# arogozhnikov/demuxalot

Hardware: AMD Instinct MI355X
Metric: EM iterations/sec + barcodes demuxed/sec, 200k bc x 100k SNP x 64 gt (higher is better)
Workload: dtype f32 terms, f64 sums (guarded mode: coarse pass reads the table as f16 and sums in f32; exact redo where the contract is not proven)

## Files before the change

### demuxalot_amd/_lib.py

```python
import ctypes
import os
from ctypes import POINTER, c_char_p, c_double, c_float, c_int, c_int32, c_int64, c_void_p

import numpy as np

_HERE = os.path.dirname(os.path.abspath(__file__))
LIB_PATH = os.environ.get('DEMUXALOT_AMD_LIB') or os.path.join(_HERE, 'libdemux_hip.so')

DMX_F32, DMX_F64 = 0, 1
T_PSTEP, T_ESTEP, T_MSTEP, T_MCOMBINE, T_ALLREDUCE, T_COUNT = 0, 1, 2, 3, 4, 5
TIMER_NAMES = ('pstep', 'estep', 'mstep', 'mcombine', 'allreduce')
HOST_COLLECTIVE = ctypes.CFUNCTYPE(ctypes.c_int, ctypes.c_void_p, ctypes.c_int, ctypes.c_void_p, ctypes.c_int64, ctypes.c_int)
COLL_ALL_REDUCE, COLL_REDUCE_SCATTER, COLL_ALL_GATHER = 0, 1, 2
UNIQUE_ID_BYTES = 128

_P = c_void_p
SIGNATURES = {
    'dmx_last_error': (c_char_p, []),
    'dmx_version': (c_char_p, []),
    'dmx_device_count': (c_int, [POINTER(c_int)]),
    'dmx_create': (c_int, [c_int, POINTER(_P)]),
    'dmx_destroy': (c_int, [_P]),
    'dmx_synchronize': (c_int, [_P]),
    'dmx_pack_calls_host': (c_int, [c_int64, _P, _P, _P, c_int64, _P, _P, _P, _P, _P, _P,
                                    POINTER(c_int64), POINTER(c_int64), _P, _P, _P, _P, _P]),
    'dmx_hash_host': (c_int, [_P, c_int64, c_int32, POINTER(ctypes.c_uint64)]),
    'dmx_set_problem': (c_int, [_P, c_int64, c_int64, c_int32, c_int64, _P, _P, _P, _P]),
    'dmx_pack_and_set_problem': (c_int, [_P, c_int64, c_int64, c_int32, _P, _P, _P, _P, c_int64, _P, _P, _P, _P, _P,
                                         POINTER(c_int64), POINTER(c_int64), _P]),
    'dmx_pack_containers_and_set_problem': (c_int, [_P, c_int64, c_int64, c_int32, _P, _P, _P, _P, _P, c_int32,
                                                    POINTER(c_int64), POINTER(c_int64), _P]),
    'dmx_stage_containers': (c_int, [_P, _P, c_int32]),
    'dmx_pack_staged_and_set_problem': (c_int, [_P, c_int64, c_int64, c_int32, _P, _P, _P, _P, _P, c_int32,
                                                POINTER(c_int64), POINTER(c_int64), _P]),
    'dmx_get_packed_calls': (c_int, [_P, _P, _P, _P, _P]),
    'dmx_set_betas': (c_int, [_P, _P]),
    'dmx_set_prior_betas': (c_int, [_P, _P, c_double, c_int, _P, _P]),
    'dmx_set_addition': (c_int, [_P, _P]),
    'dmx_probs_from_betas': (c_int, [_P, c_float, c_float, _P]),
    'dmx_probs_from_betas_f64': (c_int, [_P, _P, c_float, c_float, _P]),
    'dmx_set_probs': (c_int, [_P, _P]),
    'dmx_estep': (c_int, [_P, c_int, _P, _P, c_int, _P, _P]),
    'dmx_mstep': (c_int, [_P, c_float, _P]),
    'dmx_em': (c_int, [_P, c_int, c_float, c_float, c_int, _P, _P, c_int, c_float, _P, _P, _P]),
    'dmx_run_iterations': (c_int, [_P, c_int, c_float, c_float, c_float]),
    'dmx_get_logits': (c_int, [_P, _P]),
    'dmx_get_probs': (c_int, [_P, _P]),
    'dmx_get_addition': (c_int, [_P, _P]),
    'dmx_get_block': (c_int, [_P, c_int, c_int64, c_int64, c_int64, c_int64, _P]),
    'dmx_get_assignments': (c_int, [_P, _P, _P]),
    'dmx_get_assignments_above': (c_int, [_P, c_float, _P, _P, POINTER(c_int64)]),
    'dmx_get_top_options': (c_int, [_P, c_int32, _P, _P]),
    'dmx_get_option_sums': (c_int, [_P, _P]),
    'dmx_set_keep_molecule_calls': (c_int, [_P, c_int]),
    'dmx_set_molecule_calls': (c_int, [_P, c_int64, _P, _P, _P]),
    'dmx_get_max_pair_count': (c_int, [_P, POINTER(c_int64)]),
    'dmx_estep_snp': (c_int, [_P, c_int, _P, c_int64, _P, c_int, _P, _P]),
    'dmx_mstep_f64': (c_int, [_P, c_double, _P]),
    'dmx_mstep_f64_sums': (c_int, [_P, c_double, _P]),
    'dmx_get_prior_betas': (c_int, [_P, _P]),
    'dmx_get_learnt_betas': (c_int, [_P, _P]),
    'dmx_exchange_slices': (c_int, [c_int64, _P, c_int32, _P, POINTER(c_int64), POINTER(c_int32)]),
    'dmx_comm_unique_id': (c_int, [_P]),
    'dmx_comm_init': (c_int, [_P, c_int, c_int, _P, c_int]),
    'dmx_comm_init_host': (c_int, [_P, c_int, c_int, _P, _P, c_int]),
    'dmx_get_timings': (c_int, [_P, POINTER(c_double), POINTER(c_int64)]),
    'dmx_reset_timings': (c_int, [_P]),
    'dmx_set_phase_timers': (c_int, [_P, c_int]),
    'dmx_set_logits_needed': (c_int, [_P, c_int]),
    'dmx_set_lean_memory': (c_int, [_P, c_int]),
    'dmx_device_bytes': (c_int, [_P, POINTER(c_int64)]),
    'dmx_trim_cache': (c_int, [_P, POINTER(c_int64)]),
    'dmx_release_problem': (c_int, [_P]),
    'dmx_trim_device_caches': (c_int, [c_int, POINTER(c_int64)]),
    'dmx_set_exact_additions': (c_int, [_P, c_int]),
    'dmx_set_estep_mode': (c_int, [_P, c_int]),
    'dmx_set_msteps_expected': (c_int, [_P, c_int64]),
    'dmx_snp_count': (c_int, [_P, _P, c_int32, _P, c_int64, c_int32, c_float, c_int32, POINTER(c_int64)]),
    'dmx_snp_score': (c_int, [_P, c_double, _P, _P, _P, _P, _P, _P]),
    'dmx_snp_select': (c_int, [_P, c_int64, c_int64, _P, POINTER(c_int64)]),
    'dmx_count_reads': (c_int, [_P, _P, _P, c_int64, _P, POINTER(c_int64), POINTER(c_int64)]),
    'dmx_count_reads_fetch': (c_int, [_P, _P, _P]),
    'dmx_coverage_count': (c_int, [_P, _P, c_int32, c_int32, c_int32, _P]),
    'dmx_coverage_candidates': (c_int, [_P, c_double, c_double, c_double, c_double, c_int64, POINTER(c_int64)]),
    'dmx_coverage_fetch_candidates': (c_int, [_P, _P, _P]),
}
DEBUG_SIGNATURES = {
    'dmx_comm_init_emulated': (c_int, [_P, c_int, c_int, c_double, c_double, c_int]),
    'dmx_get_exchange_compact': (c_int, [_P, POINTER(c_int64), POINTER(c_int64), POINTER(c_int64)]),
    'dmx_get_exchange_compact_table': (c_int, [_P, POINTER(c_int64), POINTER(c_int64), POINTER(c_int64)]),
    'dmx_get_guard_probes': (c_int, [_P, POINTER(c_int64), POINTER(c_int64)]),
    'dmx_debug_set_pass_ms': (c_int, [_P, c_double, c_double, c_double]),
    'dmx_get_redo_count': (c_int, [_P, POINTER(c_int64)]),
    'dmx_set_guard_adaptive': (c_int, [_P, c_int]),
    'dmx_set_coarse_pass': (c_int, [_P, c_int]),
    'dmx_set_mstep_incremental': (c_int, [_P, c_int]),
    'dmx_get_mstep_incremental': (c_int, [_P, POINTER(c_int64), POINTER(c_int64), POINTER(c_int64)]),
    'dmx_get_guard_levels': (c_int, [_P, POINTER(c_int32), POINTER(c_int64), POINTER(c_int64), POINTER(c_int64), POINTER(c_double), POINTER(c_double), POINTER(c_double)]),
    'dmx_get_guard_direct': (c_int, [_P, POINTER(c_int32), POINTER(c_int64), POINTER(c_int64), POINTER(c_double), POINTER(c_double)]),
    'dmx_set_estep_schedule': (c_int, [_P, c_int]),
    'dmx_set_estep_dictionary': (c_int, [_P, c_int]),
    'dmx_get_estep_form': (c_int, [_P, POINTER(c_int32), POINTER(c_int32)]),
    'dmx_set_estep_packing': (c_int, [_P, c_int]),
    'dmx_set_mstep_wide_addresses': (c_int, [_P, c_int]),
    'dmx_set_mstep_tiles': (c_int, [_P, c_int]),
    'dmx_get_mstep_form': (c_int, [_P, POINTER(c_int32)]),
    'dmx_get_mstep_tiles_info': (c_int, [_P, POINTER(c_int32), POINTER(c_double)]),
    'dmx_test_logf': (c_int, [_P, _P, _P, c_int64]),
    'dmx_test_logf_hot': (c_int, [_P, _P, _P, c_int64]),
    'dmx_test_expf': (c_int, [_P, _P, _P, c_int64]),
    'dmx_test_log2_hw': (c_int, [_P, _P, _P, c_int64]),
    'dmx_test_softmax': (c_int, [_P, _P, _P, c_int64, c_int64]),
    'dmx_runtime_info': (c_int, [c_char_p, c_int64]),
    'dmx_get_exchange_mode': (c_int, [_P, POINTER(c_int32)]),
    'dmx_get_guard_stats': (c_int, [_P, POINTER(c_int64), POINTER(c_int64), POINTER(c_int64)]),
    'dmx_get_count_reads_timings': (c_int, [_P, POINTER(c_double)]),
    'dmx_count_reads_begin': (c_int, [_P, _P, c_int64, _P]),
    'dmx_count_reads_push': (c_int, [_P, _P, c_int, POINTER(c_int64), POINTER(c_int64)]),
    'dmx_count_reads_end': (c_int, [_P]),
    'dmx_get_count_reads_carry': (c_int, [_P, POINTER(c_int64)]),
    'dmx_get_count_reads_peak_bytes': (c_int, [_P, POINTER(c_int64)]),
    'dmx_set_coverage_form': (c_int, [_P, c_int]),
    'dmx_get_coverage_timings': (c_int, [_P, POINTER(c_double)]),
    'dmx_reads_upload': (c_int, [_P, _P, POINTER(c_int64)]),
    'dmx_reads_release': (c_int, [_P, c_int64]),
    'dmx_reads_info': (c_int, [_P, c_int64, POINTER(c_int64)]),
    'dmx_count_reads_resident': (c_int, [_P, c_int64, _P, c_int64, _P, POINTER(c_int64), POINTER(c_int64)]),
    'dmx_coverage_count_resident': (c_int, [_P, c_int64, c_int32, c_int32, c_int32, _P]),
    'dmx_count_reads_push_resident': (c_int, [_P, c_int64, c_int64, c_int64, c_int, POINTER(c_int64), POINTER(c_int64)]),
    'dmx_get_reads_upload_bytes': (c_int, [_P, POINTER(c_int64)]),
}

COVERAGE_STAGES = ('upload', 'walk', 'window', 'accumulate', 'filter', 'top_n')
COVERAGE_ATOMIC, COVERAGE_TILED = 0, 1
READS_INFO = ('n_reads', 'n_cigar_ops', 'n_bases', 'nbytes', 'reference_length')
COUNT_READS_STAGES = ('upload', 'walk', 'molecules', 'duplicates', 'observations', 'fold', 'order')


class DecodedReadsStruct(ctypes.Structure):
    _fields_ = [('n_reads', c_int64), ('reference_start', _P), ('compressed_cb', _P), ('compressed_ub', _P), ('p_misaligned', _P),
                ('alignment_score', _P), ('cigar_begin', _P), ('n_cigar', _P), ('seq_begin', _P), ('l_seq', _P),
                ('n_cigar_ops', c_int64), ('cigar', _P), ('n_bases', c_int64), ('seq', _P), ('qual', _P)]


_lib = None


class DemuxHipError(RuntimeError):
    pass


def load():
    global _lib
    if _lib is None:
        if not os.path.exists(LIB_PATH):
            raise DemuxHipError(
                f'{LIB_PATH} is missing: build it with `python -c "import __graft_entry__ as g; g.build()"` '
                f'or `make -C demuxalot_amd/csrc`. demuxalot_amd has no CPU fallback.')
        os.environ.setdefault('HSA_ENABLE_IPC_MODE_LEGACY', '0')
        lib = ctypes.CDLL(LIB_PATH)
        for name, (res, args) in {**SIGNATURES, **DEBUG_SIGNATURES}.items():
            fn = getattr(lib, name)
            fn.restype = res
            fn.argtypes = args
        _lib = lib
    return _lib


def check(status):
    if status != 0:
# ... 32 lines not shown
```

### demuxalot_amd/csrc/dmx_api.cpp

```cpp
#include <dlfcn.h>
#include <hip/hip_runtime.h>
#include <rccl/rccl.h>

#include <array>
#include <chrono>
#include <functional>

#include <algorithm>
#include <mutex>
#include <cmath>
#include <cstdio>
#include <cstdlib>
#include <cstring>
#include <string>
#include <vector>

#include "dmx_ctx.h"
#include "dmx_host.h"

using namespace dmx::host;

extern "C" {

static int begin_problem(dmx_ctx *c, int64_t B, int64_t V, int32_t G, const int32_t *v2snp, std::vector<int> &snp_ptr,
// ... 175 lines not shown
    HIP_TRY(hipStreamSynchronize(c->stream));
    return 0;
}

int dmx_set_exact_additions(dmx_ctx *c, int exact)
{
    if (!c) return fail(DMX_ERR_INVALID, "null context");
    c->exact_additions = exact != 0;
    return 0;
}

int dmx_set_estep_mode(dmx_ctx *c, int mode)
{
    if (!c) return fail(DMX_ERR_INVALID, "null context");
    if (mode != DMX_ESTEP_EXACT && mode != DMX_ESTEP_FAST && mode != DMX_ESTEP_GUARDED) return fail(DMX_ERR_INVALID, "unknown E-step mode %d", mode);
    c->estep_mode = mode;
    return 0;
}

static int read_guard_state(dmx_ctx *c, unsigned (&st)[dmx::GS_WORDS], long long *count, long long *count_fine = nullptr, long long *count_coarse = nullptr)
{
    std::vector<unsigned> all((size_t)dmx::GUARD_STATE_WORDS, 0u);
    if (c->d_guard_count.p) {
        HIP_TRY(hipMemcpyAsync(all.data(), c->d_guard_count.p, all.size() * sizeof(unsigned), hipMemcpyDeviceToHost, c->stream));
        HIP_TRY(hipStreamSynchronize(c->stream));
    }
    for (int i = 0; i < dmx::GS_WORDS; i++) st[i] = all[(size_t)i];
    long long hashed_fine = 0, hashed_coarse = 0;
    for (int i = 0; i < dmx::GUARD_SLOTS; i++) {
        hashed_fine += all[(size_t)dmx::GS_SLOTS_FINE + i];
        hashed_coarse += all[(size_t)dmx::GS_SLOTS_COARSE + i];
    }
    const unsigned level = st[dmx::GS_LEVEL];
    const long long fine = level == 1u ? (long long)st[dmx::GS_COUNT] : hashed_fine;
    const long long coarse = level == 0u ? (long long)st[dmx::GS_COUNT] : (st[dmx::GS_CAPABLE] ? hashed_coarse : -1);
    *count = level == 0u ? coarse : fine;
    if (count_fine) *count_fine = fine;
    if (count_coarse) *count_coarse = coarse;
    return 0;
}

int dmx_get_guard_stats(dmx_ctx *c, int64_t *redone_last, int64_t *redone_total, int64_t *rows_total)
{
    DMX_TRY(bind(c));
    unsigned st[dmx::GS_WORDS];
    long long count = 0;
    DMX_TRY(read_guard_state(c, st, &count));
    const long long last = st[dmx::GS_DIRECT] ? (long long)st[dmx::GS_ROWS] : count;
    const long long total = (long long)(((unsigned long long)st[dmx::GS_TOTAL + 1] << 32) | st[dmx::GS_TOTAL]) + (st[dmx::GS_PENDING] ? last : 0);
    if (redone_last) *redone_last = c->guard_ran ? (int64_t)last : 0;
    if (redone_total) *redone_total = (int64_t)total;
    if (rows_total) *rows_total = (int64_t)c->guard_rows_total;
    return 0;
}

int dmx_set_mstep_incremental(dmx_ctx *c, int incremental)
{
    if (!c) return fail(DMX_ERR_INVALID, "null context");
    if (incremental < 0 || incremental > 2) return fail(DMX_ERR_INVALID, "incremental M-step: 0 off, 1 on, 2 on with the first sums built by the delta pass");
    if (incremental != c->mstep_incremental) c->incr_valid = false;
    c->mstep_incremental = incremental;
    return 0;
}

int dmx_get_mstep_incremental(dmx_ctx *c, int64_t *full_passes, int64_t *delta_passes, int64_t *barcodes_last_delta)
{
    DMX_TRY(bind(c));
    unsigned st[3 * dmx::IS_WORDS] = {};
    if (c->d_incr_state.p) {
        HIP_TRY(hipMemcpyAsync(st, c->d_incr_state.p, sizeof(st), hipMemcpyDeviceToHost, c->stream));
        HIP_TRY(hipStreamSynchronize(c->stream));
    }
    if (full_passes) *full_passes = (int64_t)st[2 * dmx::IS_WORDS];
    if (delta_passes) *delta_passes = (int64_t)st[2 * dmx::IS_WORDS + 1];
    if (barcodes_last_delta) *barcodes_last_delta = st[2 * dmx::IS_WORDS + 2] == 0xFFFFFFFFu ? -1 : (int64_t)st[2 * dmx::IS_WORDS + 2];
    return 0;
}

int dmx_set_coarse_pass(dmx_ctx *c, int coarse)
{
    if (!c) return fail(DMX_ERR_INVALID, "null context");
    if (coarse < 0 || coarse > 2) return fail(DMX_ERR_INVALID, "coarse pass: 0 never, 1 where the logits are not read, 2 wherever the shape allows");
    c->coarse_pass = coarse;
    return 0;
}

int dmx_set_lean_memory(dmx_ctx *c, int lean)
{
    DMX_TRY(bind(c));
    c->lean_memory = lean != 0;
    if (c->lean_memory && c->coarse_ready) {
        dev_free(c, c->d_tile_stream);
        dev_free(c, c->d_call_rows);
    }
    return 0;
}

int dmx_set_guard_adaptive(dmx_ctx *c, int adaptive)
{
    if (!c) return fail(DMX_ERR_INVALID, "null context");
    c->guard_adaptive = adaptive != 0;
    return 0;
}

int dmx_get_guard_direct(dmx_ctx *c, int32_t *last_ran_direct, int64_t *direct_steps, int64_t *would_queue_last, double *fast_pass_ms,
                         double *exact_pass_ms)
{
    DMX_TRY(bind(c));
    unsigned st[dmx::GS_WORDS];
    long long count = 0;
    DMX_TRY(read_guard_state(c, st, &count));
    if (last_ran_direct) *last_ran_direct = c->guard_ran && st[dmx::GS_DIRECT] ? 1 : 0;
    if (direct_steps) *direct_steps = (int64_t)st[dmx::GS_DIRECT_STEPS];
    if (would_queue_last) *would_queue_last = c->guard_ran ? (int64_t)count : 0;
    int khz = 0;
    HIP_TRY(hipDeviceGetAttribute(&khz, hipDeviceAttributeWallClockRate, c->device));
    const double ms_per_tick = khz > 0 ? 1.0 / (double)khz : 0.0;
    if (fast_pass_ms) *fast_pass_ms = st[dmx::GS_F_TICKS] * ms_per_tick;
    if (exact_pass_ms) *exact_pass_ms = (st[dmx::GS_E_MEASURED] ? 1.0 : -1.0) * st[dmx::GS_E_TICKS] * ms_per_tick;
    return 0;
}

int dmx_get_guard_levels(dmx_ctx *c, int32_t *level_last, int64_t *coarse_steps, int64_t *flagged_fine_last, int64_t *flagged_coarse_last,
                         double *coarse_pass_ms, double *fine_pass_ms, double *exact_pass_ms)
{
    DMX_TRY(bind(c));
    unsigned st[dmx::GS_WORDS];
    long long count = 0, fine = 0, coarse = 0;
    DMX_TRY(read_guard_state(c, st, &count, &fine, &coarse));
    if (level_last) *level_last = c->guard_ran ? (int32_t)st[dmx::GS_LEVEL] : -1;
    if (coarse_steps) *coarse_steps = (int64_t)st[dmx::GS_COARSE_STEPS];
    if (flagged_fine_last) *flagged_fine_last = c->guard_ran ? (int64_t)fine : 0;
    if (flagged_coarse_last) *flagged_coarse_last = c->guard_ran ? (int64_t)coarse : -1;
    int khz = 0;
    HIP_TRY(hipDeviceGetAttribute(&khz, hipDeviceAttributeWallClockRate, c->device));
    const double ms_per_tick = khz > 0 ? 1.0 / (double)khz : 0.0;
    if (coarse_pass_ms) *coarse_pass_ms = st[dmx::GS_C_TICKS] * ms_per_tick;
    if (fine_pass_ms) *fine_pass_ms = st[dmx::GS_F_TICKS] * ms_per_tick;
    if (exact_pass_ms) *exact_pass_ms = (st[dmx::GS_E_MEASURED] ? 1.0 : -1.0) * st[dmx::GS_E_TICKS] * ms_per_tick;
    return 0;
}

int dmx_set_logits_needed(dmx_ctx *c, int needed)
{
    if (!c) return fail(DMX_ERR_INVALID, "null context");
    c->logits_needed = needed != 0;
    return 0;
}

int dmx_get_guard_probes(dmx_ctx *c, int64_t *probes, int64_t *streak)
{
    DMX_TRY(bind(c));
    unsigned st[dmx::GS_WORDS];
    long long count = 0, fine = 0, coarse = 0;
    DMX_TRY(read_guard_state(c, st, &count, &fine, &coarse));
    if (probes) *probes = (int64_t)st[dmx::GS_PROBES];
    if (streak) *streak = (int64_t)st[dmx::GS_STREAK];
    return 0;
}

int dmx_debug_set_pass_ms(dmx_ctx *c, double coarse_pass_ms, double fine_pass_ms, double exact_pass_ms)
{
    DMX_TRY(bind(c));
    if (!c->d_guard_count.p) return fail(DMX_ERR_INVALID, "call order: a guarded E-step before dmx_debug_set_pass_ms");
    int khz = 0;
    HIP_TRY(hipDeviceGetAttribute(&khz, hipDeviceAttributeWallClockRate, c->device));
// ... 293 lines not shown
```

### demuxalot_amd/csrc/dmx_ctx.h

```cpp
#pragma once
#include <hip/hip_runtime.h>
#include <rccl/rccl.h>

#include <map>
#include <mutex>
#include <string>
#include <unordered_map>
#include <utility>
#include <vector>

#include "dmx_internal.h"
#include "kernels.h"

using dmx::fail;

#define HIP_TRY(expr)                                                                                   \
    do {                                                                                                \
        hipError_t _e = (expr);                                                                         \
        if (_e != hipSuccess) return fail(DMX_ERR_HIP, "%s failed: %s", #expr, hipGetErrorString(_e)); \
    } while (0)

#define DMX_TRY(expr)         \
    do {                      \
        int _s = (expr);      \
// ... 19 lines not shown
    size_t n = 0;
};

struct ResidentReads {
    long long n = 0, n_ops = 0, n_bases = 0;
    long long reference_length = 0;
    bool countable = false;
    int64_t bytes = 0;
    DevBuf<int> start, cb, ub, score, n_cigar, l_seq;
    DevBuf<double> p;
    DevBuf<long long> cigar_begin, seq_begin;
    DevBuf<unsigned> cigar;
    DevBuf<unsigned char> seq, qual;
};

struct dmx_ctx {
    int device = 0;
    hipStream_t stream = nullptr;
    long long B = 0, V = 0, N = 0, S = 0;
    int G = 0, K = 0;
    bool have_problem = false, have_betas = false, have_probs = false, have_post = false;

    DevBuf<long long> d_pair_ptr;
    DevBuf<dmx::CallPair> d_call_pairs;
    DevBuf<unsigned> d_call_rows;
    long long n_pairs = 0;
    DevBuf<uint2> d_csc;
    long long n_csc = 0;
    DevBuf<long long> d_item_start;
    DevBuf<int> d_item_len;
    DevBuf<long long> d_item_ptr;
    DevBuf<int> d_item_variant;
    DevBuf<int> d_bc_order, d_item_order;
    long long n_items = 0;
    long long n_bins = 0;
    int n_tiles = 0, bin_rows_cap = 0;
    DevBuf<int> d_bin_rows, d_bin_order;
    DevBuf<long long> d_bin_ptr;
    DevBuf<dmx::CallPair> d_tile_stream;
    DevBuf<int> d_v2snp, d_snp_ptr, d_snp_vars;
    DevBuf<float> d_prior, d_add, d_prob;
    DevBuf<float> d_raw;
    bool have_raw = false;
    DevBuf<unsigned short> d_prob16;
    DevBuf<unsigned> d_coarse_stream;
    DevBuf<long long> d_coarse_bin_ptr;
    DevBuf<double> d_log2_keep;
    bool coarse_ready = false;
    bool prob16_valid = false;
    int coarse_pass = 1;
    int lean_memory = 0;
    bool logits_needed = true;
    bool logits_readable = true;
    float p_clip_lo = 0.0f;
    DevBuf<double> d_add64, d_partial;
    DevBuf<float> d_logits, d_post;
    DevBuf<unsigned long long> d_nz;
    DevBuf<unsigned long long> d_redo;
    DevBuf<unsigned> d_n_redo;
    bool mstep_wide = false;
    DevBuf<uint2> d_mt_stream;
    DevBuf<long long> d_mt_ptr;
    DevBuf<int> d_mt_first;
    DevBuf<int> d_mt_order;
    DevBuf<int> d_mt_shift;
    DevBuf<unsigned char> d_mt_shift_v;
    DevBuf<unsigned long long> d_acc64;
    DevBuf<float> d_prev_post;
    DevBuf<uint2> d_prev_first;
    DevBuf<int> d_incr_list;
    DevBuf<unsigned char> d_incr_touched;
    DevBuf<unsigned> d_incr_state;
    int incr_parity = 0;
    bool incr_valid = false;
    float incr_power = 0.0f;
    int mstep_incremental = 1;
    long long mstep_incr_launches = 0;
    long long n_mt = 0;
    std::vector<long long> h_col_ptr;
    int mt_tv = 0;
    bool mt_tried = false;
    bool mt_shift_tried = false;
    int mstep_tiles = 1;
    long long msteps_done = 0;
    long long incr_rows = 0;
    DevBuf<unsigned char> d_incr_map;
    DevBuf<uint2> d_slice_rec;
    DevBuf<long long> d_slice_ptr;
    bool slice_index_tried = false;
    bool incr_heavy = false;
    int msteps_ahead = 0;
    long long msteps_expected = 0;
    double mt_build_ms = 0.0;
    int mstep_form = 0;
    DevBuf<int> d_sum_plan;
    long long sum_plan_k = -1;
    int sum_plan_values = 0;
    int item_calls = 1024;
    bool exact_additions = true;
    int estep_mode = DMX_ESTEP_EXACT;
    DevBuf<unsigned> d_guard_count;
    int guard_adaptive = 1;
    DevBuf<int> d_guard_list;
    DevBuf<int> d_guard_sub;
    unsigned guard_sub_cap = 0;
    long long guard_rows_total = 0;
    bool guard_ran = false;
    int tiled_estep = 1;
    int dict_mode = 1;
    bool add_is_zero = true;
    bool dict_candidate = false;
    int estep_form = 0;
    int estep_packing = 1;
    long long max_row_calls = 0;
    int n_simd = 0;
    long long long_row_calls[3] = {0, 0, 0};
    long long n_long_rows[3] = {0, 0, 0};
    int dict_distinct = 0;
    DevBuf<float> d_dict;
    DevBuf<unsigned char> d_codes;
    DevBuf<unsigned char> d_dtab;
    DevBuf<unsigned> d_dict_stat;
    DevBuf<dmx::EstepSegment> d_segs;
    DevBuf<int> d_split_first;
    DevBuf<double> d_seg_sums;
    long long n_segs = 0, n_split = 0;
    float nz_floor = 0.0f;
    DevBuf<uint2> d_first;
    DevBuf<unsigned long long> d_dense_calls;
    bool dense_stat_valid = false;
    DevBuf<float> d_pen;
    DevBuf<unsigned> d_pairs;
    DevBuf<unsigned> d_pair_blocks;
    int n_pair_blocks = 0;
    DevBuf<unsigned char> d_prior_logits;
    DevBuf<int> d_best;
    DevBuf<float> d_bestp;
    DevBuf<int> d_u_variant, d_u_cb;
    DevBuf<float> d_u_p;
    DevBuf<long long> d_u_count;
    long long n_u = 0;
    DevBuf<unsigned long long> d_mol;
    bool keep_molecule_calls = false;
    DevBuf<int> d_mc_variant;
    DevBuf<float> d_mc_e;
    DevBuf<long long> d_mc_start;
    unsigned mc_max_count = 0;
    DevBuf<double> d_logits64, d_post64;
    bool have_post64 = false;
    DevBuf<unsigned char> d_scratch;
    DevBuf<unsigned long long> d_sd_pos;
    DevBuf<int> d_sd_counts;
    DevBuf<double> d_sd_imp;
    long long sd_P = -1;
    int sd_D = 0;
    bool sd_scored = false;
    DevBuf<unsigned char> d_cr_molecules;
    DevBuf<unsigned char> d_cr_calls;
    long long cr_molecules = -1, cr_calls = 0;
    double cr_stage_ms[dmx::COUNT_READS_STAGES] = {};
    int64_t cr_peak_bytes = 0;
    long long cr_carried = 0;
    DevBuf<int> d_crs_positions;
    DevBuf<double> d_crs_table;
    DevBuf<int> d_crs_start, d_crs_cb, d_crs_ub, d_crs_score, d_crs_n_cigar, d_crs_l_seq;
    DevBuf<double> d_crs_p;
// ... 155 lines not shown
```

### demuxalot_amd/csrc/dmx_steps.cpp

```cpp
#include <dlfcn.h>
#include <hip/hip_runtime.h>
#include <rccl/rccl.h>

#include <array>
#include <chrono>
#include <functional>

#include <algorithm>
#include <mutex>
#include <cmath>
#include <cstdio>
#include <cstdlib>
#include <cstring>
#include <string>
#include <vector>

#include "dmx_ctx.h"
#include "dmx_host.h"

using namespace dmx::host;

namespace dmx {
namespace host {

// ... 72 lines not shown
    DMX_TRY(dev_grow(c, c->d_seg_sums, (size_t)c->n_segs * (size_t)K));
    HIP_TRY(hipStreamSynchronize(c->stream));
    if ((int)K != c->K) c->have_post64 = false;
    c->K = (int)K;
    return 0;
}

int upload_prior_logits(dmx_ctx *c, const void *prior, int dtype)
{
    if (!prior) return 0;
    if (dtype != DMX_F32 && dtype != DMX_F64) return fail(DMX_ERR_INVALID, "prior_dtype must be DMX_F32 or DMX_F64");
    const size_t bytes = (size_t)c->B * c->K * (dtype == DMX_F64 ? 8 : 4);
    if (bytes > c->d_prior_logits.n) {
        raw_free(c, c->d_prior_logits);
        DMX_TRY(raw_alloc(c, c->d_prior_logits, bytes));
    }
    HIP_TRY(hipMemcpyAsync(c->d_prior_logits.p, prior, bytes, hipMemcpyHostToDevice, c->stream));
    return 0;
}

int copy_prob_out(dmx_ctx *c, float *dst)
{
    if (!dst) return 0;
    const int G = c->G;
    if (!c->sliced) return copy_out(c, dst, c->d_prob.p, (size_t)c->V * G);
    for (int r = 0; r < c->nranks; r++) {
        const long long rows = c->cut[r + 1] - c->cut[r];
        if (rows) HIP_TRY(hipMemcpyAsync(dst + c->cut[r] * G, c->d_prob.p + (size_t)r * c->slice_rows * G, sizeof(float) * rows * G, hipMemcpyDeviceToHost, c->stream));
    }
    return 0;
}

int copy_prob_in(dmx_ctx *c, const float *src)
{
    const int G = c->G;
    c->prob_prev_valid = false;
    if (!c->sliced) {
        HIP_TRY(hipMemcpyAsync(c->d_prob.p, src, sizeof(float) * c->V * G, hipMemcpyHostToDevice, c->stream));
        return 0;
    }
    for (int r = 0; r < c->nranks; r++) {
        const long long rows = c->cut[r + 1] - c->cut[r];
        if (rows) HIP_TRY(hipMemcpyAsync(c->d_prob.p + (size_t)r * c->slice_rows * G, src + c->cut[r] * G, sizeof(float) * rows * G, hipMemcpyHostToDevice, c->stream));
    }
    return 0;
}

int ensure_full_addition(dmx_ctx *c)
{
    if (!c->add_partial) return 0;
    const int G = c->G, n = c->nranks;
    float *stage = (float *)c->d_add_stage.p;
    const size_t block = (size_t)c->slice_rows * G;
    const long long mine = c->cut[c->rank + 1] - c->cut[c->rank];
    if (mine) HIP_TRY(hipMemcpyAsync(stage + c->rank * block, c->d_add.p + c->cut[c->rank] * G, sizeof(float) * mine * G, hipMemcpyDeviceToDevice, c->stream));
    DMX_TRY(coll_all_gather(c, stage, block, "addition"));
    for (int k = 0; k < n; k++) {
        const long long rows = c->cut[k + 1] - c->cut[k];
        if (rows && k != c->rank) HIP_TRY(hipMemcpyAsync(c->d_add.p + c->cut[k] * G, stage + k * block, sizeof(float) * rows * G, hipMemcpyDeviceToDevice, c->stream));
    }
    c->add_partial = false;
    return 0;
}

bool coarse_capable(const dmx_ctx *c, int with_doublets, float lo)
{
    return c->coarse_pass && c->estep_mode == DMX_ESTEP_GUARDED && !with_doublets && c->K > 16 && c->K <= 128 && c->tiled_estep && c->n_bins > 0 &&
           (c->coarse_ready || c->d_tile_stream.p != nullptr) && lo >= 6.2e-5f && ((unsigned long long)c->prob_rows + 1ull) * (unsigned long long)c->G * 4ull < (1ull << 32);
}

int ensure_prob16(dmx_ctx *c)
{
    const size_t need16 = ((size_t)c->prob_rows + 1) * c->G * 2;
    if (need16 > c->d_prob16.n) {
        DMX_TRY(dev_grow(c, c->d_prob16, need16));
        c->prob16_valid = false;
        HIP_TRY(hipMemsetAsync(c->d_prob16.p, 0, need16 * sizeof(unsigned short), c->stream));
    }
    return 0;
}

int run_pstep(dmx_ctx *c, float lo, float hi, bool with_addition, bool with_half)
{
    const bool half_rows = with_half && c->sliced && c->prob_list_words != 0 && c->prob_prev_valid && c->prob16_valid && c->d_prob16.p != nullptr;
    with_half = with_half && !c->sliced;
    if (with_half) DMX_TRY(ensure_prob16(c));
    c->prob16_valid = false;
    TimerSpan ev{nullptr, nullptr};
    SpanGuard ev_guard{c, &ev};
    timer_begin(c, DMX_T_PSTEP, &ev);
    const long long v0 = c->sliced ? c->cut[c->rank] : 0, v1 = c->sliced ? c->cut[c->rank + 1] : c->V;
    if (c->emulated && c->sliced && !c->emu_table_filled) {
        for (int r = 0; r < c->nranks; r++)
            if (r != c->rank)
                HIP_TRY(dmx::launch_probs_from_betas(c->stream, c->d_prior.p, nullptr, c->d_v2snp.p, c->d_snp_ptr.p, c->d_snp_vars.p, c->cut[r],
                                                     c->cut[r + 1] - c->cut[r], -1LL, c->G, c->d_prow.p, lo, hi, c->d_prob.p));
        c->emu_table_filled = true;
    }
    HIP_TRY(dmx::launch_probs_from_betas(c->stream, c->d_prior.p, with_addition ? c->d_add.p : nullptr, c->d_v2snp.p,
                                         c->d_snp_ptr.p, c->d_snp_vars.p, v0, v1 - v0, c->sliced ? -1LL : (long long)c->S, c->G, c->d_prow.p, lo, hi,
                                         c->d_prob.p, (with_half || half_rows) ? c->d_prob16.p : nullptr));
    c->prob16_valid = with_half;
    timer_end(c, DMX_T_PSTEP, ev);
    if (c->sliced) {
        timer_begin(c, DMX_T_ALLREDUCE, &ev);
        const size_t block = (size_t)c->slice_rows * c->G;
        float *mine = c->d_prob.p + (size_t)c->rank * block;
        int rc = 0;
        bool whole = true;
        if (c->prob_list_words != 0 && c->prob_prev_valid) {
            const unsigned cap_now = std::max(1u, std::min(c->prob_cap_now, c->prob_list_cap));
            const size_t words_now = 4 + (size_t)cap_now * (size_t)(1 + c->G);
            HIP_TRY(dmx::launch_prob_changes_build(c->stream, mine, c->d_prob_prev.p, c->slice_rows, c->G, cap_now,
                                                   c->d_prob_list.p + (size_t)c->rank * words_now,
                                                   c->emulated ? c->d_prob_list.p : nullptr, (unsigned long long)words_now, c->nranks, c->rank));
            rc = coll_all_gather(c, (float *)c->d_prob_list.p, words_now, "changed rows of genotype_prob");
            if (rc == 0) {
                const unsigned seq = ++c->list_seq;
                HIP_TRY(dmx::launch_post_counts(c->stream, c->d_prob_list.p, (unsigned long long)words_now, c->nranks, c->h_prob_counts, seq));
                HIP_TRY(dmx::launch_prob_changes_apply(c->stream, c->d_prob.p, c->d_prob_list.p, (unsigned long long)words_now, c->slice_rows, c->G,
                                                       c->nranks, c->rank, cap_now, half_rows ? (unsigned short *)c->d_prob16.p : nullptr));
                DMX_TRY(wait_counts(c, c->h_prob_counts, c->nranks, seq));
                unsigned longest = 0;
                for (int r = 0; r < c->nranks; r++) longest = std::max(longest, c->h_prob_counts[r]);
                whole = longest > cap_now;
                if (std::getenv("DEMUXALOT_AMD_EXCHANGE_TRACE")) std::fprintf(stderr, "[table lists] longest %u capacity %u of %u\n", longest, cap_now, c->prob_list_cap);
                c->prob_cap_now = whole ? c->prob_list_cap : (unsigned)std::min<unsigned long long>(c->prob_list_cap, 4ull * longest + 512ull);
                if (!whole) {
                    c->prob_compact_taken++;
                    c->prob16_valid = half_rows;
                } else {
                    c->prob_compact_overflows++;
                }
            }
        } else if (c->prob_list_words != 0) {
            HIP_TRY(hipMemcpyAsync(c->d_prob_prev.p, mine, sizeof(float) * block, hipMemcpyDeviceToDevice, c->stream));
            c->prob_prev_valid = true;
        }
        if (rc == 0 && whole) rc = coll_all_gather(c, c->d_prob.p, block, "genotype_prob");
        timer_end(c, DMX_T_ALLREDUCE, ev);
        if (rc) return rc;
    }
    c->have_probs = true;
    c->p_clip_lo = lo;
    c->dict_candidate = !with_addition || c->add_is_zero;
    return 0;
}

int prepare_dictionary(dmx_ctx *c, bool pairs, dmx::EstepArgs &a, int *form)
{
    *form = DMX_FORM_DIRECT;
    a.dict_n = 0;
    c->dict_distinct = 0;
    const bool wanted = c->dict_mode == 2 || (c->dict_mode == 1 && c->dict_candidate);
    if (!wanted || c->estep_mode == DMX_ESTEP_FAST || c->B == 0 || c->prob_rows == 0) return 0;
    const int G = c->G;
    const long long K = c->K, rows = c->prob_rows;
    const bool block_form = pairs && K > dmx::DICT_LANE_K;
    if (a.call_rows == nullptr) return 0;
    if (!block_form && (K > dmx::DICT_LANE_K || rows >= (1 << 24) || a.pairs_bytes == 0)) return 0;
    if (block_form && (size_t)G * 72 + 9 * 1024 > 160 * 1024) return 0;
    if (G > 1024) return 0;
    if (c->dict_mode == 1 && !block_form) {
        const long long lanes = K <= 16 ? 4 : K <= 32 ? 8 : K <= 64 ? 16 : K <= 128 ? 32 : 64;
        if (pairs || c->B * lanes / 64 < 8192) return 0;
    }
    const size_t code_pitch = (size_t)dmx::dict_code_pitch(G);
    DMX_TRY(dev_grow(c, c->d_dict, (size_t)rows * dmx::DICT_CAP));
    DMX_TRY(dev_grow(c, c->d_codes, (size_t)rows * code_pitch));
    if (!c->d_dict_stat.p) DMX_TRY(dev_alloc(c, c->d_dict_stat, (size_t)1));
    HIP_TRY(dmx::launch_build_dict(c->stream, c->d_prob.p, rows, G, c->d_dict.p, c->d_codes.p, c->d_dict_stat.p));
    unsigned distinct = 0;
    HIP_TRY(hipMemcpyAsync(&distinct, c->d_dict_stat.p, sizeof(unsigned), hipMemcpyDeviceToHost, c->stream));
    HIP_TRY(hipStreamSynchronize(c->stream));
// ... 138 lines not shown
                if (c->lean_memory) {
                    dev_free(c, c->d_tile_stream);
                    dev_free(c, c->d_call_rows);
                    a.call_rows = nullptr;
                }
            }
            if (allow_coarse) DMX_TRY(ensure_prob16(c));
            HIP_TRY(dmx::launch_guard_begin(c->stream, c->d_guard_count.p, c->B, c->K, c->guard_adaptive, capable, allow_coarse));
            a.guard = 1;
            if (fine8) a.guard_per_call = dmx::guard_per_call_fine8(dmx::coarse_calls_per_gather((int)c->K));
            a.order_direct = c->d_bc_order.p;
            a.guard_main_coarse = 0;
            a.guard_alt_per_call = capable ? dmx::GUARD_PER_CALL_COARSE : 0.0f;
            a.guard_alt_accum = capable ? dmx::GUARD_ACCUM_F32 : 0.0f;
            if (allow_coarse) {
                if (!c->prob16_valid) {
                    const bool kept = c->sliced && c->prob_list_words != 0;
                    HIP_TRY(dmx::launch_prob_to_half(c->stream, c->d_prob.p, c->prob_rows, c->G, c->d_prob16.p, kept ? nullptr : c->d_guard_count.p + dmx::GS_SKIP_COARSE));
                    c->prob16_valid = kept;
                }
                dmx::EstepArgs coarse = a;
                coarse.prob16 = c->d_prob16.p;
                coarse.coarse_stream = c->d_coarse_stream.p;
                coarse.coarse_bin_ptr = c->d_coarse_bin_ptr.p;
                coarse.log2_keep = c->d_log2_keep.p;
                coarse.guard_per_call = dmx::GUARD_PER_CALL_COARSE;
                coarse.guard_accum = dmx::GUARD_ACCUM_F32;
                coarse.guard_main_coarse = 1;
                coarse.guard_alt_per_call = a.guard_per_call;
                coarse.guard_alt_accum = 0.0f;
                coarse.direct = c->d_guard_count.p + dmx::GS_SKIP_COARSE;
                HIP_TRY(dmx::launch_estep(c->stream, coarse, false));
            }
            a.direct = c->d_guard_count.p + dmx::GS_SKIP_FINE;
            a.tile_stream = c->d_tile_stream.p;
            if (c->d_tile_stream.p == nullptr) {
                if (c->coarse_ready && !with_doublets && a.n_bins > 0 && c->K > 16 && c->K <= 128) {
                    a.coarse_stream = c->d_coarse_stream.p;
                    a.coarse_bin_ptr = c->d_coarse_bin_ptr.p;
                    a.log2_keep = c->d_log2_keep.p;
                    a.prob16 = nullptr;
                    a.guard_per_call = dmx::guard_per_call_fine8(dmx::coarse_calls_per_gather((int)c->K));
                } else {
                    a.n_bins = 0;
                }
            }
            HIP_TRY(dmx::launch_estep(c->stream, a, with_doublets != 0));
            a.coarse_stream = nullptr;
            HIP_TRY(dmx::launch_guard_compact(c->stream, c->d_guard_count.p, c->d_guard_sub.p, c->guard_sub_cap, c->d_guard_list.p, c->d_bc_order.p, c->B));
            dmx::EstepArgs redo = a;
            redo.direct = c->d_guard_count.p + dmx::GS_DIRECT;
            redo.fast = 0;
            redo.guard = 2;
            redo.n_bins = 0;
            redo.order = c->d_guard_list.p;
            redo.order_count = c->d_guard_count.p + dmx::GS_COUNT;
            HIP_TRY(dmx::launch_estep(c->stream, redo, with_doublets != 0));
            c->guard_rows_total += c->B;
            c->guard_ran = true;
        } else {
            if (c->d_tile_stream.p == nullptr) {
                if (fine8 && a.fast) {
                    a.coarse_stream = c->d_coarse_stream.p;
                    a.coarse_bin_ptr = c->d_coarse_bin_ptr.p;
                    a.log2_keep = c->d_log2_keep.p;
                } else {
                    a.n_bins = 0;
                }
            }
            HIP_TRY(dmx::launch_estep(c->stream, a, with_doublets != 0));
        }
    }
    c->estep_form = form;
    if (a.dense_calls) HIP_TRY(dmx::launch_sum_dense(c->stream, c->d_dense_calls.p, c->guard_ran ? c->d_guard_count.p : nullptr));
    else if (c->guard_ran) HIP_TRY(dmx::launch_guard_stamp(c->stream, c->d_guard_count.p, dmx::GS_T_END));
    timer_end(c, DMX_T_ESTEP, ev);
    c->have_post = true;
    c->logits_readable = logits_kept;
    return 0;
}

int run_mstep(dmx_ctx *c, float power)
{
    const bool mshard = c->mshard;
    const size_t row_base = mshard ? (size_t)c->rank * (size_t)c->rows_pad : 0;
    const int Wn = (c->G + 63) / 64;
    dmx::MstepArgs a;
    a.order = c->d_item_order.p;
    a.item_start = c->d_item_start.p;
    a.item_len = c->d_item_len.p;
    a.calls = c->d_csc.p;
    a.post = mshard ? c->d_post_g.p : c->d_post.p;
    a.nz = mshard ? c->d_nz_g.p : c->d_nz.p;
    a.first = mshard ? c->d_first_g.p : c->d_first.p;
    const unsigned long long rows = mshard ? (unsigned long long)c->rows_total : (unsigned long long)c->B;
    a.K = mshard ? c->G : c->K;
    a.first_bytes = 8ull * rows;
    a.wide = c->mstep_wide;
    a.post_bytes = rows * (unsigned long long)a.K * 4ull;
    a.partial = c->d_partial.p;
    a.n_items = c->n_items;
    a.G = c->G;
    a.square = (power == 2.0f);
    a.power = power;
    a.dense_calls = c->dense_stat_valid && a.post_bytes < (1ull << 32) ? c->d_dense_calls.p : nullptr;
    a.total_calls = 2ull * (unsigned long long)c->n_pairs;
    if (!a.square && c->nz_floor != 0.0f) {
        HIP_TRY(dmx::launch_rebuild_nz(c->stream, c->d_post.p, c->B, c->K, c->G, 0.0f, (mshard ? c->d_nz_g.p : c->d_nz.p) + row_base * Wn,
                                       c->G <= 64 ? (mshard ? c->d_first_g.p : c->d_first.p) + row_base : nullptr));
        c->nz_floor = 0.0f;
        c->post_gathered = false;
    }
    DMX_TRY(gather_posteriors(c));
    c->add_is_zero = false;
    TimerSpan ev{nullptr, nullptr};
    SpanGuard ev_guard{c, &ev};
    const bool dist = c->attached();
    unsigned long long *redo = c->exact_additions ? c->d_redo.p : nullptr;
    a.item_variant = nullptr;
    a.item_ptr = c->d_item_ptr.p;
    a.prow = nullptr;
    a.out32 = nullptr;
    a.out64 = nullptr;
    const bool f64 = c->reduce_dtype == DMX_F64;
    a.item_variant = c->d_item_variant.p;
    a.redo_cap = c->d_redo.n;
    a.fixed_shift_v = nullptr;
    a.fixed_acc64 = nullptr;
    a.fixed_state = nullptr;
    a.incr_total = 0ull;
    a.tiles_done = false;
    dmx::MTileArgs tiles{};
    constexpr int MSTEP_TILES_PAY = 8;
    const long long ahead = std::max<long long>(c->msteps_ahead, c->msteps_expected);
    const bool own_sums = !mshard && (!dist || c->sliced);
    const bool can_go_incremental = c->mstep_incremental && c->mstep_tiles == 1 && !c->exact_additions && c->G <= 64 && c->n_csc > 0 && power > 0.0f &&
                                    own_sums && c->d_call_pairs.p != nullptr && c->d_item_variant.p != nullptr;
    if (can_go_incremental && !c->incr_heavy && c->n_mt == 0 && c->d_incr_state.p != nullptr &&
        (c->msteps_done == 4 || c->msteps_done == 16 || c->msteps_done == 64)) {
        unsigned full_passes = 0;
        HIP_TRY(hipMemcpyAsync(&full_passes, c->d_incr_state.p + 2 * dmx::IS_WORDS + 3, sizeof(unsigned), hipMemcpyDeviceToHost, c->stream));
        HIP_TRY(hipStreamSynchronize(c->stream));
        c->incr_heavy = c->msteps_done == 4 ? full_passes >= 3u : 2ull * full_passes >= (unsigned long long)c->msteps_done;
    }
    const bool tiles_wanted = c->mstep_tiles == 2 || (c->mstep_tiles == 1 && (c->n_mt > 0 || ((ahead >= MSTEP_TILES_PAY || c->msteps_done >= MSTEP_TILES_PAY) &&
                                                                                            (!can_go_incremental || c->incr_heavy))));
    if (c->msteps_expected > 0) c->msteps_expected--;
    c->msteps_done++;
    if (!c->exact_additions && tiles_wanted && c->G <= 64 && c->n_csc > 0 && power > 0.0f) {
        if (!c->mt_tried) {
            HIP_TRY(hipStreamSynchronize(c->stream));
            const auto t0 = std::chrono::steady_clock::now();
            DMX_TRY(dmx::build_mstep_tiles(c, mshard ? c->cut[c->rank] : 0, mshard ? c->cut[c->rank + 1] : c->V));
            c->mt_build_ms = std::chrono::duration<double, std::milli>(std::chrono::steady_clock::now() - t0).count();
        }
        if (c->n_mt > 0) {
            tiles.stream = c->d_mt_stream.p;
            tiles.ptr = c->d_mt_ptr.p;
            tiles.first = c->d_mt_first.p;
            tiles.order = c->d_mt_order.p;
            tiles.shift = c->d_mt_shift.p;
            tiles.n_tiles = c->n_mt;
            tiles.tv = c->mt_tv;
            a.tiles_done = true;
        }
    }
// ... 7 lines not shown
        if (f64) a.out64 = c->d_add64.p;
        else a.out32 = c->d_add.p;
    }
    bool fixed_items = !a.tiles_done && c->mstep_tiles != 0 && c->mstep_incremental && !c->exact_additions && c->G <= 64 && c->n_csc > 0 &&
                       power > 0.0f && own_sums && c->d_call_pairs.p != nullptr && c->d_item_variant.p != nullptr;
    if (fixed_items) {
        DMX_TRY(dmx::plan_mstep_shifts(c));
        fixed_items = c->d_mt_shift_v.p != nullptr;
    }
    const bool sharded_incr = a.tiles_done && c->mstep_incremental == 1 && mshard && c->d_mt_shift_v.p != nullptr && a.out32 == c->d_add.p && c->G <= 64 &&
                              c->d_item_variant.p != nullptr && c->rows_total > 0;
    const bool incremental = sharded_incr || ((a.tiles_done || fixed_items) && c->mstep_incremental && own_sums && c->d_mt_shift_v.p != nullptr &&
                                              c->d_call_pairs.p != nullptr);
    const long long incr_rows = sharded_incr ? c->rows_total : c->B;
    dmx::MIncrArgs incr{};
    if (incremental) {
        if (!c->d_acc64.p) {
            c->incr_rows = incr_rows;
            DMX_TRY(dev_alloc(c, c->d_acc64, (size_t)c->V * c->G));
            DMX_TRY(dev_alloc(c, c->d_prev_post, (size_t)incr_rows * c->G));
            DMX_TRY(dev_alloc(c, c->d_prev_first, (size_t)incr_rows));
            DMX_TRY(dev_alloc(c, c->d_incr_list, (size_t)incr_rows));
            if (sharded_incr) {
                DMX_TRY(dmx::build_slice_row_index(c));
                if (c->d_slice_rec.p == nullptr) {
                    DMX_TRY(dev_alloc(c, c->d_incr_map, (size_t)incr_rows));
                    HIP_TRY(hipMemsetAsync(c->d_incr_map.p, 0, (size_t)incr_rows, c->stream));
                }
            }
            DMX_TRY(dev_alloc(c, c->d_incr_touched, (size_t)c->V));
            DMX_TRY(dev_alloc(c, c->d_incr_state, (size_t)(3 * dmx::IS_WORDS)));
            HIP_TRY(hipMemsetAsync(c->d_incr_state.p, 0, sizeof(unsigned) * 3 * dmx::IS_WORDS, c->stream));
            HIP_TRY(hipMemsetAsync(c->d_incr_touched.p, 0, (size_t)c->V, c->stream));
            c->incr_valid = false;
        }
        if (!c->incr_valid || c->incr_power != power) {
            HIP_TRY(hipMemsetAsync(c->d_incr_state.p, 0, sizeof(unsigned) * 2 * dmx::IS_WORDS, c->stream));
            if (c->mstep_incremental == 2 && !dist) {
                const unsigned on[2] = {1u, 1u};
                HIP_TRY(hipMemsetAsync(c->d_acc64.p, 0, sizeof(unsigned long long) * (size_t)c->V * c->G, c->stream));
                HIP_TRY(hipMemsetAsync(c->d_prev_post.p, 0, sizeof(float) * (size_t)incr_rows * c->G, c->stream));
                HIP_TRY(hipMemsetAsync(c->d_prev_first.p, 0xFF, sizeof(uint2) * (size_t)incr_rows, c->stream));
                HIP_TRY(hipMemsetAsync(c->d_add.p, 0, sizeof(float) * (size_t)c->V * c->G, c->stream));
                HIP_TRY(hipMemcpyAsync(c->d_incr_state.p + dmx::IS_VALID, &on[0], sizeof(unsigned), hipMemcpyHostToDevice, c->stream));
                HIP_TRY(hipMemcpyAsync(c->d_incr_state.p + dmx::IS_FORCE, &on[1], sizeof(unsigned), hipMemcpyHostToDevice, c->stream));
                HIP_TRY(hipStreamSynchronize(c->stream));
            }
            c->incr_parity = 0;
            c->incr_valid = true;
            c->incr_power = power;
        }
        incr.state = c->d_incr_state.p + c->incr_parity * dmx::IS_WORDS;
        incr.next = c->d_incr_state.p + (c->incr_parity ^ 1) * dmx::IS_WORDS;
        c->incr_parity ^= 1;
        incr.counters = c->d_incr_state.p + 2 * dmx::IS_WORDS;
        incr.acc64 = c->d_acc64.p;
        incr.prev = c->d_prev_post.p;
        incr.prev_first = c->d_prev_first.p;
        incr.list = c->d_incr_list.p;
        incr.touched = c->d_incr_touched.p;
        incr.shift_v = c->d_mt_shift_v.p;
        incr.pairs = sharded_incr ? nullptr : c->d_call_pairs.p;
        incr.call_rows = sharded_incr ? nullptr : c->d_call_rows.p;
        incr.pair_ptr = sharded_incr ? nullptr : c->d_pair_ptr.p;
        incr.changed_map = sharded_incr ? c->d_incr_map.p : nullptr;
        incr.rec = sharded_incr ? c->d_slice_rec.p : nullptr;
        incr.rec_ptr = sharded_incr && c->d_slice_rec.p != nullptr ? c->d_slice_ptr.p : nullptr;
        incr.row_variant = !sharded_incr && c->sliced ? c->d_row_variant.p : nullptr;
        incr.B = incr_rows;
        incr.V = c->V;
        incr.floor = dmx::mincr_floor(power);
        a.incr_total = !sharded_incr ? 0ull : incr.rec_ptr != nullptr ? (unsigned long long)c->n_csc : 2ull * (unsigned long long)incr_rows;
        tiles.acc64 = c->d_acc64.p;
        tiles.incr_state = incr.state;
        if (fixed_items) {
            a.fixed_shift_v = c->d_mt_shift_v.p;
            a.fixed_acc64 = c->d_acc64.p;
            a.fixed_state = incr.state;
        }
        c->mstep_incr_launches++;
    } else {
        c->incr_valid = false;
    }
    timer_begin(c, DMX_T_MSTEP, &ev);
    if (sharded_incr) HIP_TRY(dmx::launch_mstep_incremental_sharded(c->stream, a, tiles, incr));
    else if (incremental && fixed_items) HIP_TRY(dmx::launch_mstep_items_incremental(c->stream, a, incr));
    else if (incremental) HIP_TRY(dmx::launch_mstep_incremental(c->stream, a, tiles, incr));
    else if (a.tiles_done) HIP_TRY(dmx::launch_mstep_tiles(c->stream, a, tiles));
    else HIP_TRY(dmx::launch_mstep(c->stream, a));
    c->mstep_form = a.tiles_done ? 2 : (incremental && fixed_items ? 3 : 1);
    timer_end(c, DMX_T_MSTEP, ev);
    if (!dist) {
        timer_begin(c, DMX_T_MCOMBINE, &ev);
        HIP_TRY(dmx::launch_mcombine(c->stream, a, c->d_item_ptr.p, 0, c->V, nullptr, c->d_add.p, nullptr, redo, c->d_n_redo.p, nullptr, true));
        timer_end(c, DMX_T_MCOMBINE, ev);
        return 0;
    }
    if (mshard) {
        timer_begin(c, DMX_T_MCOMBINE, &ev);
        HIP_TRY(dmx::launch_mcombine(c->stream, a, c->d_item_ptr.p, c->cut[c->rank], c->cut[c->rank + 1], nullptr, c->d_add.p, nullptr, redo,
                                     c->d_n_redo.p, nullptr, true));
        timer_end(c, DMX_T_MCOMBINE, ev);
        c->add_partial = c->nranks > 1;
        return 0;
    }
    int rc = 0;
    if (c->sliced) {
        timer_begin(c, DMX_T_MCOMBINE, &ev);
        HIP_TRY(dmx::launch_mcombine(c->stream, a, c->d_item_ptr.p, 0, c->V, c->d_prow.p, f64 ? nullptr : (float *)c->d_exch.p,
                                     f64 ? (double *)c->d_exch.p : nullptr, redo, c->d_n_redo.p, nullptr, true));
        timer_end(c, DMX_T_MCOMBINE, ev);
        timer_begin(c, DMX_T_ALLREDUCE, &ev);
        const size_t block = (size_t)c->slice_rows * c->G;
        rc = coll_reduce_scatter(c, c->d_exch.p, c->d_recv.p, block, f64, c->stream);
        if (rc == 0)
            HIP_TRY(dmx::launch_store_slice(c->stream, c->d_recv.p, f64, c->cut[c->rank], c->cut[c->rank + 1] - c->cut[c->rank], c->G, c->d_add.p));
        timer_end(c, DMX_T_ALLREDUCE, ev);
        if (rc) return rc;
        c->add_partial = c->nranks > 1;
        return 0;
    }
    timer_begin(c, DMX_T_MCOMBINE, &ev);
    HIP_TRY(dmx::launch_mcombine(c->stream, a, c->d_item_ptr.p, 0, c->V, nullptr, f64 ? nullptr : c->d_add.p, f64 ? c->d_add64.p : nullptr, redo,
                                 c->d_n_redo.p, nullptr, true));
    timer_end(c, DMX_T_MCOMBINE, ev);
    timer_begin(c, DMX_T_ALLREDUCE, &ev);
    const size_t cnt = (size_t)c->V * c->G;
    if (f64) {
        rc = coll_all_reduce(c, c->d_add64.p, cnt, true);
        if (rc == 0) HIP_TRY(dmx::launch_f64_to_f32(c->stream, c->d_add64.p, c->d_add.p, (long long)cnt));
    } else {
        rc = coll_all_reduce(c, c->d_add.p, cnt, false);
    }
    timer_end(c, DMX_T_ALLREDUCE, ev);
    return rc;
}

}
}

extern "C" {

int dmx_set_addition(dmx_ctx *c, const float *addition)
{
    DMX_TRY(bind(c));
    DMX_TRY(need(c, c->have_problem, "dmx_set_problem before dmx_set_addition"));
    const size_t vg = (size_t)c->V * c->G;
    c->incr_valid = false;
    if (addition) {
        HIP_TRY(hipMemcpyAsync(c->d_add.p, addition, sizeof(float) * vg, hipMemcpyHostToDevice, c->stream));
        HIP_TRY(hipStreamSynchronize(c->stream));
    } else {
        HIP_TRY(hipMemsetAsync(c->d_add.p, 0, sizeof(float) * (vg ? vg : 1), c->stream));
    }
    c->add_is_zero = addition == nullptr;
    c->add_partial = false;
    return 0;
}

int dmx_probs_from_betas(dmx_ctx *c, float lo, float hi, float *prob_out)
{
    DMX_TRY(bind(c));
    DMX_TRY(need(c, c->have_problem && c->have_betas, "dmx_set_problem + dmx_set_betas before dmx_probs_from_betas"));
    DMX_TRY(run_pstep(c, lo, hi, true));
    DMX_TRY(copy_prob_out(c, prob_out));
    HIP_TRY(hipStreamSynchronize(c->stream));
    return 0;
}

int dmx_set_probs(dmx_ctx *c, const float *prob)
{
    DMX_TRY(bind(c));
    DMX_TRY(need(c, c->have_problem, "dmx_set_problem before dmx_set_probs"));
    if (!prob && c->V > 0) return fail(DMX_ERR_INVALID, "null prob table");
    if (c->V) DMX_TRY(copy_prob_in(c, prob));
    HIP_TRY(hipMemsetAsync(c->d_best.p, 0, sizeof(int), c->stream));
    HIP_TRY(dmx::launch_check_unit_range(c->stream, c->d_prob.p, c->prob_rows * c->G, c->d_best.p));
    int flag = 0;
    HIP_TRY(hipMemcpyAsync(&flag, c->d_best.p, sizeof(int), hipMemcpyDeviceToHost, c->stream));
    HIP_TRY(hipStreamSynchronize(c->stream));
    if (flag) return fail(DMX_ERR_INVALID, "genotype_prob has entries outside [0, 1] (or NaN)");
    c->have_probs = true;
    c->p_clip_lo = 0.0f;
    c->prob16_valid = false;
    c->dict_candidate = true;
    return 0;
}

int dmx_probs_from_betas_f64(dmx_ctx *c, const double *betas, float lo, float hi, float *prob_out)
{
    DMX_TRY(bind(c));
    DMX_TRY(need(c, c->have_problem, "dmx_set_problem before dmx_probs_from_betas_f64"));
    const size_t vg = (size_t)c->V * c->G;
    if (!betas && vg) return fail(DMX_ERR_INVALID, "null betas");
    double *d_b = nullptr;
    HIP_TRY(hipMalloc((void **)&d_b, (vg ? vg : 1) * sizeof(double)));
    hipError_t e = vg ? hipMemcpyAsync(d_b, betas, vg * sizeof(double), hipMemcpyHostToDevice, c->stream) : hipSuccess;
    if (e == hipSuccess)
        c->prob_prev_valid = false;
        e = dmx::launch_probs_from_betas_f64(c->stream, d_b, c->d_v2snp.p, c->d_snp_ptr.p, c->d_snp_vars.p, c->V, c->S, c->G, c->d_prow.p, lo, hi, c->d_prob.p);
    int rc_copy = 0;
    if (e == hipSuccess && vg) rc_copy = copy_prob_out(c, prob_out);
    if (e == hipSuccess) e = hipStreamSynchronize(c->stream);
    (void)hipStreamSynchronize(c->stream);
    (void)hipFree(d_b);
    if (e != hipSuccess) return fail(DMX_ERR_HIP, "P-step from float64 betas: %s", hipGetErrorString(e));
    if (rc_copy) return rc_copy;
    c->have_probs = true;
    c->p_clip_lo = lo;
    c->prob16_valid = false;
    c->dict_candidate = true;
    return 0;
}

int dmx_estep(dmx_ctx *c, int with_doublets, const float *penalties, const void *prior_logits, int prior_dtype,
              float *logits_out, float *probs_out)
{
    DMX_TRY(bind(c));
    DMX_TRY(need(c, c->have_problem && c->have_probs, "genotype probabilities (dmx_probs_from_betas / dmx_set_probs) before dmx_estep"));
    if (!penalties) return fail(DMX_ERR_INVALID, "null penalties");
    DMX_TRY(ensure_options(c, with_doublets, penalties));
    DMX_TRY(upload_prior_logits(c, prior_logits, prior_dtype));
    DMX_TRY(run_estep(c, with_doublets, prior_logits != nullptr, prior_dtype, 2.0f));
    const size_t bk = (size_t)c->B * c->K;
    DMX_TRY(copy_out(c, logits_out, c->d_logits.p, bk));
    DMX_TRY(copy_out(c, probs_out, c->d_post.p, bk));
    HIP_TRY(hipStreamSynchronize(c->stream));
    return 0;
}

int dmx_mstep(dmx_ctx *c, float power, float *addition_out)
{
    DMX_TRY(bind(c));
    DMX_TRY(need(c, c->have_problem && c->have_post, "dmx_estep before dmx_mstep"));
    DMX_TRY(run_mstep(c, power));
    if (addition_out) DMX_TRY(ensure_full_addition(c));
    DMX_TRY(copy_out(c, addition_out, c->d_add.p, (size_t)c->V * c->G));
    HIP_TRY(hipStreamSynchronize(c->stream));
    return 0;
}

int dmx_em(dmx_ctx *c, int n_iterations, float lo, float hi, int with_doublets, const float *penalties,
           const void *prior_logits, int prior_dtype, float power, float *logits_out, float *probs_out,
           float *addition_out)
{
    DMX_TRY(bind(c));
    DMX_TRY(need(c, c->have_problem && c->have_betas, "dmx_set_problem + dmx_set_betas before dmx_em"));
    if (n_iterations < 1) return fail(DMX_ERR_INVALID, "n_iterations must be >= 1");
    if (!penalties) return fail(DMX_ERR_INVALID, "null penalties");
    DMX_TRY(ensure_options(c, with_doublets, penalties));
    DMX_TRY(upload_prior_logits(c, prior_logits, prior_dtype));
    const size_t vg = (size_t)c->V * c->G;
    HIP_TRY(hipMemsetAsync(c->d_add.p, 0, sizeof(float) * (vg ? vg : 1), c->stream));
    c->incr_valid = false;
    c->add_is_zero = true;
    c->add_partial = false;
    const bool keep_last = c->logits_needed || logits_out != nullptr;
    for (int it = 0; it < n_iterations; it++) {
        const bool kept = it + 1 == n_iterations && keep_last;
        DMX_TRY(run_pstep(c, lo, hi, true, !kept && it > 0 && coarse_capable(c, with_doublets, lo)));
        DMX_TRY(run_estep(c, with_doublets, it == 0 && prior_logits != nullptr, prior_dtype, power, kept));
        if (it + 1 < n_iterations) {
            c->msteps_ahead = n_iterations - 1 - it;
            const int rc_m = run_mstep(c, power);
            c->msteps_ahead = 0;
            if (rc_m) return rc_m;
        }
    }
    const size_t bk = (size_t)c->B * c->K;
    DMX_TRY(copy_out(c, logits_out, c->d_logits.p, bk));
    DMX_TRY(copy_out(c, probs_out, c->d_post.p, bk));
    DMX_TRY(ensure_full_addition(c));
    DMX_TRY(copy_out(c, addition_out, c->d_add.p, vg));
    HIP_TRY(hipStreamSynchronize(c->stream));
    return 0;
}

int dmx_run_iterations(dmx_ctx *c, int n_iterations, float lo, float hi, float power)
{
    DMX_TRY(bind(c));
    DMX_TRY(need(c, c->have_problem && c->have_betas && c->have_post && c->K > 0,
                 "dmx_estep or dmx_em (to fix the options) before dmx_run_iterations"));
    if (n_iterations < 0) return fail(DMX_ERR_INVALID, "negative n_iterations");
    const int with_doublets = c->K != c->G;
    for (int it = 0; it < n_iterations; it++) {
        const bool kept = it + 1 == n_iterations && c->logits_needed;
        DMX_TRY(run_pstep(c, lo, hi, true, !kept && coarse_capable(c, with_doublets, lo)));
        DMX_TRY(run_estep(c, with_doublets, false, DMX_F32, power, kept));
        c->msteps_ahead = n_iterations - it;
        const int rc_m = run_mstep(c, power);
        c->msteps_ahead = 0;
        if (rc_m) return rc_m;
    }
    return 0;
}

}
```

### demuxalot_amd/csrc/host_stubs.cpp

```cpp
#include <hip/hip_runtime.h>

#include <algorithm>
#include <cstdlib>
#include <cstring>
#include <numeric>
#include <vector>

#include "dmx_ctx.h"

extern "C" {

hipError_t hipGetDeviceCount(int *count)
{
    *count = 1;
    return hipSuccess;
}
hipError_t hipSetDevice(int) { return hipSuccess; }
hipError_t hipDeviceGetAttribute(int *value, hipDeviceAttribute_t, int)
{
    *value = 100000;
    return hipSuccess;
}
hipError_t hipDeviceSynchronize(void) { return hipSuccess; }
hipError_t hipGetLastError(void) { return hipSuccess; }
const char *hipGetErrorString(hipError_t e) { return e == hipSuccess ? "hipSuccess" : "hip error (host stub)"; }

hipError_t hipMalloc(void **p, size_t bytes)
{
    if (bytes > (size_t(1) << 31)) {
        *p = nullptr;
        return hipErrorOutOfMemory;
    }
    *p = std::malloc(bytes ? bytes : 1);
    return *p ? hipSuccess : hipErrorOutOfMemory;
}
hipError_t hipFree(void *p)
{
    std::free(p);
    return hipSuccess;
}
hipError_t hipHostMalloc(void **p, size_t bytes, unsigned) { return hipMalloc(p, bytes); }
hipError_t hipHostFree(void *p) { return hipFree(p); }

hipError_t hipMemcpyAsync(void *dst, const void *src, size_t bytes, hipMemcpyKind, hipStream_t)
{
    if (bytes) std::memmove(dst, src, bytes);
    return hipSuccess;
}
hipError_t hipMemcpy(void *dst, const void *src, size_t bytes, hipMemcpyKind kind) { return hipMemcpyAsync(dst, src, bytes, kind, nullptr); }
hipError_t hipMemcpy2DAsync(void *dst, size_t dpitch, const void *src, size_t spitch, size_t width, size_t height, hipMemcpyKind, hipStream_t)
{
    for (size_t r = 0; r < height; r++) std::memmove((char *)dst + r * dpitch, (const char *)src + r * spitch, width);
    return hipSuccess;
}
hipError_t hipMemsetAsync(void *dst, int value, size_t bytes, hipStream_t)
{
    if (bytes) std::memset(dst, value, bytes);
    return hipSuccess;
}

static int g_stream_tag, g_event_tag;
hipError_t hipStreamCreateWithFlags(hipStream_t *s, unsigned)
{
    *s = (hipStream_t)&g_stream_tag;
    return hipSuccess;
}
hipError_t hipStreamCreateWithPriority(hipStream_t *s, unsigned, int)
{
    *s = (hipStream_t)&g_stream_tag;
    return hipSuccess;
}
hipError_t hipStreamDestroy(hipStream_t) { return hipSuccess; }
hipError_t hipStreamSynchronize(hipStream_t) { return hipSuccess; }
hipError_t hipStreamQuery(hipStream_t) { return hipSuccess; }
hipError_t hipStreamWaitEvent(hipStream_t, hipEvent_t, unsigned) { return hipSuccess; }
hipError_t hipDeviceGetStreamPriorityRange(int *least, int *greatest)
{
    *least = 0;
    *greatest = -2;
    return hipSuccess;
}
hipError_t hipEventCreate(hipEvent_t *e)
{
    *e = (hipEvent_t)&g_event_tag;
    return hipSuccess;
}
hipError_t hipEventCreateWithFlags(hipEvent_t *e, unsigned) { return hipEventCreate(e); }
hipError_t hipEventDestroy(hipEvent_t) { return hipSuccess; }
hipError_t hipEventRecord(hipEvent_t, hipStream_t) { return hipSuccess; }
hipError_t hipEventSynchronize(hipEvent_t) { return hipSuccess; }
hipError_t hipEventElapsedTime(float *ms, hipEvent_t, hipEvent_t)
{
    *ms = 0.0f;
    return hipSuccess;
}

}

namespace dmx {

hipError_t launch_sum_dense(hipStream_t, unsigned long long *, unsigned *) { return hipSuccess; }
hipError_t launch_probs_from_betas(hipStream_t, const float *, const float *, const int *, const int *, const int *, long long, long long,
                                   long long, int, const int *, float, float, float *, unsigned short *) { return hipSuccess; }
hipError_t launch_probs_from_betas_f64(hipStream_t, const double *, const int *, const int *, const int *, long long, long long, int,
                                       const int *, float, float, float *) { return hipSuccess; }
hipError_t launch_check_unit_range(hipStream_t, const float *, long long, int *) { return hipSuccess; }
hipError_t launch_estep(hipStream_t, const EstepArgs &, bool) { return hipSuccess; }
hipError_t launch_softmax_rows(hipStream_t, const EstepArgs &) { return hipSuccess; }
hipError_t launch_build_dict(hipStream_t, const float *, long long, int, float *, unsigned char *, unsigned *stat)
{
    *stat = DICT_CAP + 1;
    return hipSuccess;
}
int dict_table_pitch(int, int, bool) { return 32; }
hipError_t launch_pack_rows(hipStream_t, const float *, const unsigned char *, const unsigned *, long long, int, int, bool, int,
                            unsigned char *) { return hipSuccess; }
hipError_t launch_estep_dict(hipStream_t, const EstepArgs &, bool) { return hipSuccess; }
hipError_t launch_estep_dict_block(hipStream_t, const EstepArgs &) { return hipSuccess; }
hipError_t launch_mstep(hipStream_t, const MstepArgs &) { return hipSuccess; }
hipError_t launch_mstep_incremental(hipStream_t, const MstepArgs &, const MTileArgs &, const MIncrArgs &) { return hipSuccess; }
hipError_t launch_mstep_items_incremental(hipStream_t, const MstepArgs &, const MIncrArgs &) { return hipSuccess; }
hipError_t launch_mstep_incremental_sharded(hipStream_t, const MstepArgs &, const MTileArgs &, const MIncrArgs &) { return hipSuccess; }
hipError_t launch_mstep_tiles(hipStream_t, const MstepArgs &, const MTileArgs &) { return hipSuccess; }
hipError_t launch_guard_begin(hipStream_t, unsigned *, long long, int, int, int, int) { return hipSuccess; }
hipError_t launch_prob_to_half(hipStream_t, const float *, long long, int, unsigned short *, const unsigned *) { return hipSuccess; }
hipError_t launch_build_coarse_stream(hipStream_t, const CallPair *, const long long *, long long, unsigned, int, long long *, unsigned *, const int *, int, double *) { return hipSuccess; }
hipError_t launch_guard_stamp(hipStream_t, unsigned *, int) { return hipSuccess; }
hipError_t launch_guard_compact(hipStream_t, unsigned *, const int *, unsigned, int *, const int *, long long) { return hipSuccess; }
hipError_t launch_mcombine(hipStream_t, const MstepArgs &, const long long *, long long, long long, const int *, float *, double *,
                           unsigned long long *, unsigned *, const int *, bool) { return hipSuccess; }
hipError_t launch_store_slice(hipStream_t, const void *, bool, long long, long long, int, float *) { return hipSuccess; }
bool estep_packed_shape(int, int, int *, int *) { return false; }
hipError_t launch_estep_packed(hipStream_t, const EstepArgs &) { return hipSuccess; }
hipError_t launch_remap_row_offsets(hipStream_t, CallPair *pairs, long long n_pairs, unsigned row_bytes, const int *new_rows, unsigned *call_rows)
{
    for (long long i = 0; i < n_pairs; i++)
        for (int h = 0; h < 2; h++) {
            const unsigned row = (unsigned)new_rows[pairs[i].row_off[h] / row_bytes];
            pairs[i].row_off[h] = row * row_bytes;
            if (call_rows) call_rows[2 * i + h] = row;
        }
    return hipSuccess;
}
hipError_t launch_f64_to_f32(hipStream_t, const double *, float *, long long) { return hipSuccess; }
hipError_t launch_add_f32(hipStream_t, const float *, const float *, float *, long long) { return hipSuccess; }
hipError_t launch_f32_to_f64(hipStream_t, const float *, double *, long long) { return hipSuccess; }
hipError_t launch_delay(hipStream_t, long long) { return hipSuccess; }
hipError_t launch_post_compact_build(hipStream_t, const uint2 *, const float *, long long, int, unsigned cap, unsigned *block, float *, unsigned char *,
                                     unsigned *, unsigned long long, int, int)
{
    block[0] = cap + 1;
    return hipSuccess;
}
hipError_t launch_prob_changes_build(hipStream_t, const float *, float *, long long, int, unsigned cap, unsigned *block, unsigned *,
                                     unsigned long long, int, int)
{
    block[0] = cap + 1;
    return hipSuccess;
}
hipError_t launch_prob_changes_apply(hipStream_t, float *, const unsigned *, unsigned long long, long long, int, int, int, unsigned, unsigned short *) { return hipSuccess; }
hipError_t launch_post_counts(hipStream_t, const unsigned *blocks, unsigned long long block_words, int nranks, unsigned *out, unsigned seq)
{
    for (int r = 0; r < nranks; r++) out[r] = blocks[(size_t)r * block_words];
    out[nranks] = seq;
    return hipSuccess;
}
hipError_t launch_post_reconstruct(hipStream_t, const uint2 *, float *, const unsigned *, unsigned long long, long long, int, int, int, unsigned, uint2 *) { return hipSuccess; }
hipError_t launch_prior_betas(hipStream_t, const float *, float *, const unsigned long long *, const int *, const int *, const int *,
                              long long, int, double, float *) { return hipSuccess; }
hipError_t launch_rebuild_nz(hipStream_t, const float *, long long, int, int, float, unsigned long long *, uint2 *) { return hipSuccess; }
hipError_t launch_assign(hipStream_t, const float *, long long, int, int *, float *) { return hipSuccess; }
hipError_t launch_test_log(hipStream_t, const float *, float *, long long) { return hipSuccess; }
hipError_t launch_test_log_hot(hipStream_t, const float *, float *, long long) { return hipSuccess; }
hipError_t launch_test_log2_hw(hipStream_t, const float *, float *, long long) { return hipSuccess; }
hipError_t launch_test_exp(hipStream_t, const float *, float *, long long) { return hipSuccess; }
hipError_t launch_test_softmax(hipStream_t, const float *, float *, long long, int) { return hipSuccess; }

int repack_on_device(dmx_ctx *c, const int32_t *variant, const int32_t *cb, const float *p)
{
    const long long B = c->B, V = c->V, N = c->N;
    const int G = c->G;
    c->item_calls = item_calls_for(N);
    for (long long i = 0; i < N; i++) {
        if ((unsigned)cb[i] >= (unsigned long long)B) return fail(DMX_ERR_INVALID, "compressed_cb[%lld]=%d outside [0,%lld)", i, cb[i], B);
        if ((unsigned)variant[i] >= (unsigned long long)V) return fail(DMX_ERR_INVALID, "variant_id[%lld]=%d outside [0,%lld)", i, variant[i], V);
        if (!(p[i] >= 0.0f && p[i] <= 1.0f)) return fail(DMX_ERR_INVALID, "p_base_wrong[%lld]=%g outside [0,1]", i, (double)p[i]);
// ... 182 lines not shown
```

### demuxalot_amd/csrc/kernels.h

```cpp
#pragma once
#include <hip/hip_runtime.h>

#include "demux_hip.h"
#include "demux_hip_debug.h"

namespace dmx {

struct alignas(32) CallPair {
    unsigned row_off[2];
    float keep[2];
    float floor[2];
    unsigned reserved[2];
};
static_assert(sizeof(CallPair) == 32, "CallPair layout");

#ifndef DMX_PAIRBLOCK_R1
#define DMX_PAIRBLOCK_R1 2
#define DMX_PAIRBLOCK_R2 3
#endif
constexpr int PAIRBLOCK_R1 = DMX_PAIRBLOCK_R1, PAIRBLOCK_R2 = DMX_PAIRBLOCK_R2;

struct EstepSegment {
    int barcode;
    int first_pair;
// ... 89 lines not shown
       GS_COUNT_COARSE = 21,
       GS_CAPABLE = 22,
       GS_COARSE_STEPS = 23,
       GS_PROBES = 24,
       GS_STREAK = 25,
       GS_WORDS = 26 };
constexpr unsigned GUARD_PROBE_STREAK = 64;
constexpr unsigned GS_UNKNOWN = 0xFFFFFFFFu;
constexpr float GUARD_PER_CALL_COARSE = 5.1e-4f;
inline float guard_per_call_fine8(int cpg) { return 1.91e-6f / (float)(8 / cpg) + 4.0f * 6.0e-8f + 7.0e-8f; }
constexpr float GUARD_ACCUM_F32 = 6.0e-8f;
constexpr int GUARD_SLOTS = 256;
constexpr int GUARD_QUEUES = 256;
constexpr int GS_SLOTS_FINE = GS_WORDS, GS_SLOTS_COARSE = GS_WORDS + GUARD_SLOTS, GS_QUEUE_LEN = GS_WORDS + 2 * GUARD_SLOTS;
constexpr int GUARD_STATE_WORDS = GS_WORDS + 2 * GUARD_SLOTS + GUARD_QUEUES;
hipError_t launch_guard_compact(hipStream_t st, unsigned *state, const int *sub, unsigned sub_cap, int *list, const int *order_direct, long long B);
hipError_t launch_guard_begin(hipStream_t st, unsigned *state, long long B, int K, int adaptive, int capable, int allow_coarse);
hipError_t launch_guard_stamp(hipStream_t st, unsigned *state, int which);

constexpr int CALL_PAD_PAIRS = 64;
constexpr int DICT_CAP = 8;
constexpr int DICT_PAIR_CAP = 4;
constexpr int DICT_LANE_K = 256;
__host__ __device__ inline int dict_code_pitch(int n) { return (n + 3) & ~3; }

constexpr int DENSE_SLOTS = 1024;
hipError_t launch_sum_dense(hipStream_t st, unsigned long long *counters, unsigned *guard_state = nullptr);
constexpr int TILE_R_MAX = 9;
constexpr long long TILE_BYTES = 1 << 20;
#ifndef DMX_TILE_MIN_BARCODES
#define DMX_TILE_MIN_BARCODES 8192
#endif
constexpr long long TILE_MIN_BARCODES = DMX_TILE_MIN_BARCODES;
#ifndef DMX_TILE_MIN_TABLE_BYTES
#define DMX_TILE_MIN_TABLE_BYTES (1 << 20)
#endif
constexpr long long TILE_MIN_TABLE_BYTES = DMX_TILE_MIN_TABLE_BYTES;

struct MstepArgs {
    const int *order;
    const long long *item_start;
    const int *item_len;
    const uint2 *calls;
    const float *post;
    const unsigned long long *nz;
    bool wide;
    unsigned long long first_bytes;
    const uint2 *first;
    double *partial;
    const int *item_variant;
    unsigned long long redo_cap;
    bool tiles_done;
    const long long *item_ptr;
    const int *prow;
    float *out32;
    double *out64;
    long long n_items;
    long long K;
    unsigned long long post_bytes;
    int G;
    int square;
    float power;
    const unsigned long long *dense_calls;
    unsigned long long total_calls;
    const unsigned char *fixed_shift_v;
    unsigned long long *fixed_acc64;
    const unsigned *fixed_state;
    unsigned long long incr_total;
};

constexpr float NZ_FLOOR_SQUARE = 8.271806125530277e-25f;

constexpr int MIN_ITEM_CALLS = 1024, MAX_ITEM_CALLS = 16384;
inline int item_calls_for(long long n_calls)
{
    long long len = MIN_ITEM_CALLS;
    while (len < MAX_ITEM_CALLS && len * 6000 < n_calls) len *= 2;
    return (int)len;
}

hipError_t launch_probs_from_betas(hipStream_t st, const float *prior, const float *addition, const int *v2snp,
                                   const int *snp_ptr, const int *snp_vars, long long v_begin, long long n_rows, long long n_snps,
                                   int G, const int *prow, float lo, float hi, float *prob, unsigned short *prob16 = nullptr);
hipError_t launch_probs_from_betas_f64(hipStream_t st, const double *betas, const int *v2snp, const int *snp_ptr,
                                       const int *snp_vars, long long V, long long n_snps, int G, const int *prow, float lo,
                                       float hi, float *prob);
hipError_t launch_check_unit_range(hipStream_t st, const float *x, long long n, int *flags);
hipError_t launch_estep(hipStream_t st, const EstepArgs &a, bool pairs);
constexpr int coarse_calls_per_gather(int K) { return K > 64 ? 1 : K > 32 ? 2 : 4; }
constexpr int coarse_batches_per_record(int cpg) { return cpg; }
hipError_t launch_build_coarse_stream(hipStream_t st, const CallPair *stream, const long long *bin_ptr, long long n_bins, unsigned zero_off,
                                      int cpg, long long *coarse_bin_ptr, unsigned *out, const int *bin_rows, int R, double *log2_keep);
hipError_t launch_prob_to_half(hipStream_t st, const float *prob, long long rows, int G, unsigned short *out, const unsigned *skip);
hipError_t launch_softmax_rows(hipStream_t st, const EstepArgs &a);
hipError_t launch_build_dict(hipStream_t st, const float *prob, long long rows, int G, float *dict, unsigned char *codes, unsigned *stat);
int dict_table_pitch(int distinct, int K, bool pairs);
hipError_t launch_pack_rows(hipStream_t st, const float *dict, const unsigned char *codes, const unsigned *opt_pairs, long long rows, int G,
                            int K, bool pairs, int distinct, unsigned char *table);
hipError_t launch_estep_dict(hipStream_t st, const EstepArgs &a, bool pairs);
hipError_t launch_estep_dict_block(hipStream_t st, const EstepArgs &a);
hipError_t launch_mstep(hipStream_t st, const MstepArgs &a);
struct MTileArgs {
    const uint2 *stream;
    const long long *ptr;
    const int *first;
    const int *order;
    const int *shift;
    long long n_tiles;
    int tv;
    unsigned long long *acc64;
    const unsigned *incr_state;
};
struct MIncrArgs {
    unsigned *state;
    unsigned *next;
    unsigned *counters;
    unsigned long long *acc64;
    float *prev;
    uint2 *prev_first;
    int *list;
    unsigned char *touched;
    const unsigned char *shift_v;
    const CallPair *pairs;
    const unsigned *call_rows;
    const long long *pair_ptr;
    long long B, V;
    float floor;
    unsigned char *changed_map;
    const int *row_variant;
    const uint2 *rec;
    const long long *rec_ptr;
};
enum { IS_N = 0,
       IS_CALLS = 2,
       IS_VALID = 4,
       IS_STREAK = 5,
       IS_SITOUT = 6,
       IS_FORCE = 7,
       IS_WORDS = 8 };
inline float mincr_floor(float power) { return power * 126.0f > 52.0f ? exp2f(-52.0f / power) : 0.0f; }
hipError_t launch_mstep_incremental(hipStream_t st, const MstepArgs &a, const MTileArgs &t, const MIncrArgs &x);
hipError_t launch_mstep_items_incremental(hipStream_t st, const MstepArgs &a, const MIncrArgs &x);
hipError_t launch_mstep_incremental_sharded(hipStream_t st, const MstepArgs &a, const MTileArgs &t, const MIncrArgs &x);
constexpr int MTILE_LDS_BYTES = 64 * 1024;
constexpr int MTILE_MAX_VARIANTS = 128;
hipError_t launch_mstep_tiles(hipStream_t st, const MstepArgs &a, const MTileArgs &t);

hipError_t launch_mcombine(hipStream_t st, const MstepArgs &a, const long long *item_ptr, long long v0, long long v1,
                           const int *prow, float *add32, double *add64, unsigned long long *redo, unsigned *n_redo,
                           const int *vlist = nullptr, bool skip_single = false);
hipError_t launch_store_slice(hipStream_t st, const void *slice, bool f64, long long v_begin, long long n_rows, int G, float *add);
bool estep_packed_shape(int K, int G, int *lanes, int *slots);
hipError_t launch_estep_packed(hipStream_t st, const EstepArgs &a);
hipError_t launch_remap_row_offsets(hipStream_t st, CallPair *pairs, long long n_pairs, unsigned row_bytes, const int *new_rows,
                                    unsigned *call_rows);
hipError_t launch_f64_to_f32(hipStream_t st, const double *in, float *out, long long n);
hipError_t launch_add_f32(hipStream_t st, const float *a, const float *b, float *out, long long n);
hipError_t launch_delay(hipStream_t st, long long ticks);
hipError_t launch_post_compact_build(hipStream_t st, const uint2 *first, const float *post, long long B, int G, unsigned cap, unsigned *block,
                                     float *sent, unsigned char *sent_multi, unsigned *peers, unsigned long long block_words, int nranks, int own);
hipError_t launch_prob_changes_build(hipStream_t st, const float *slice, float *prev, long long rows, int G, unsigned cap, unsigned *block,
                                     unsigned *peers, unsigned long long block_words, int nranks, int own);
hipError_t launch_prob_changes_apply(hipStream_t st, float *table, const unsigned *blocks, unsigned long long block_words, long long slice_rows, int G,
                                     int nranks, int own, unsigned cap, unsigned short *table16);
hipError_t launch_post_counts(hipStream_t st, const unsigned *blocks, unsigned long long block_words, int nranks, unsigned *out_host_visible, unsigned seq);
hipError_t launch_post_reconstruct(hipStream_t st, const uint2 *first_g, float *post_g, const unsigned *blocks, unsigned long long block_words,
                                   long long rows_pad, int G, int nranks, int own, unsigned cap, uint2 *seen);
hipError_t launch_f32_to_f64(hipStream_t st, const float *in, double *out, long long n);
hipError_t launch_prior_betas(hipStream_t st, const float *betas, float *bsum, const unsigned long long *n_mol,
                              const int *v2snp, const int *snp_ptr, const int *snp_vars, long long V, int G,
                              double default_prior, float *out);
hipError_t launch_rebuild_nz(hipStream_t st, const float *post, long long B, int K, int G, float nz_floor,
                             unsigned long long *nz, uint2 *first);
hipError_t launch_assign(hipStream_t st, const float *post, long long B, int K, int *best, float *best_p);
hipError_t launch_test_log(hipStream_t st, const float *in, float *out, long long n);
hipError_t launch_test_log_hot(hipStream_t st, const float *in, float *out, long long n);
hipError_t launch_test_exp(hipStream_t st, const float *in, float *out, long long n);
hipError_t launch_test_log2_hw(hipStream_t st, const float *in, float *out, long long n);
hipError_t launch_test_softmax(hipStream_t st, const float *in, float *out, long long rows, int cols);

}
```

### demuxalot_amd/csrc/kernels.hip

```cpp
#include <hip/hip_runtime.h>

#include <cstdlib>
#include <cstring>

#include <type_traits>
#include <utility>
#include "kernels.h"
#include "np_math.h"
#include "estep_epilogue.h"

namespace dmx {

template <typename T, int L>
__global__ __launch_bounds__(256) void k_probs_from_betas(const T *__restrict__ prior,
                                                          const T *__restrict__ addition,
                                                          const int *__restrict__ v2snp,
                                                          const int *__restrict__ snp_ptr,
                                                          const int *__restrict__ snp_vars, long long v_begin,
                                                          long long n_rows, long long n_snps, int G,
                                                          const int *__restrict__ prow, float clip_lo, float clip_hi,
                                                          float *__restrict__ prob, unsigned short *__restrict__ prob16)
{
    const int lane = threadIdx.x & 63, li = lane & (L - 1);
    const long long r = ((long long)blockIdx.x * 4 + (threadIdx.x >> 6)) * (64 / L) + lane / L;
    if (r >= (n_snps >= 0 ? n_snps : n_rows)) return;
    const int snp = n_snps >= 0 ? (int)r : v2snp[v_begin + r];
    const int j0 = snp_ptr[snp], j1 = snp_ptr[snp + 1];
    if (n_snps < 0 && snp_vars[j0] != v_begin + r) return;
    constexpr int HELD = 4;
    const int cnt = j1 - j0;
    long long w[HELD];
#pragma unroll
    for (int q = 0; q < HELD; q++) w[q] = q < cnt ? (long long)snp_vars[j0 + q] : -1;
    for (int g = li; g < G; g += L) {
        T held[HELD];
#pragma unroll
        for (int q = 0; q < HELD; q++) {
            held[q] = (T)0;
            if (w[q] >= 0) {
                const long long o = w[q] * G + g;
                held[q] = addition ? prior[o] + addition[o] : prior[o];
            }
        }
        double den = 0.0;
#pragma unroll
        for (int q = 0; q < HELD; q++) den += (double)held[q];
        for (int j = j0 + HELD; j < j1; j++) {
            const long long o = (long long)snp_vars[j] * G + g;
            den += (double)(addition ? prior[o] + addition[o] : prior[o]);
        }
        den = fmax(den, 1e-7);
#pragma unroll
        for (int q = 0; q < HELD; q++) {
            if (w[q] < 0) continue;
            float p = (float)((double)held[q] / den);
            p = fminf(fmaxf(p, clip_lo), clip_hi);
            const long long row = prow ? (long long)prow[w[q]] : w[q];
            prob[row * G + g] = p;
            if (prob16) prob16[row * (2 * G) + g] = __builtin_bit_cast(unsigned short, (_Float16)p);
        }
        for (int j = j0 + HELD; j < j1; j++) {
            const long long v_j = snp_vars[j];
            const long long o = v_j * G + g;
            const T beta = addition ? prior[o] + addition[o] : prior[o];
            float p = (float)((double)beta / den);
            p = fminf(fmaxf(p, clip_lo), clip_hi);
            const long long row = prow ? (long long)prow[v_j] : v_j;
            prob[row * G + g] = p;
            if (prob16) prob16[row * (2 * G) + g] = __builtin_bit_cast(unsigned short, (_Float16)p);
        }
    }
}

__global__ __launch_bounds__(256) void k_beta_rowsum(const float *__restrict__ betas, long long V, int G,
                                                     float *__restrict__ bsum)
{
    const int lane = threadIdx.x & 63;
    const long long v = (long long)blockIdx.x * 4 + (threadIdx.x >> 6);
    if (v >= V) return;
    const float tot = npm::row_sum_wave(betas + (size_t)v * G, G, lane);
    if (lane == 0) bsum[v] = tot;
}

__global__ __launch_bounds__(256) void k_prior_betas(const float *__restrict__ betas, const float *__restrict__ bsum,
                                                     const unsigned long long *__restrict__ n_mol,
                                                     const int *__restrict__ v2snp, const int *__restrict__ snp_ptr,
                                                     const int *__restrict__ snp_vars, long long V, int G,
                                                     double default_prior, float *__restrict__ out)
{
    const long long i = (long long)blockIdx.x * blockDim.x + threadIdx.x;
    if (i >= V * G) return;
    const long long v = i / G;
    const int snp = v2snp[v];
    double mol_snp = 0.0, beta_snp = 0.0;
    for (int j = snp_ptr[snp]; j < snp_ptr[snp + 1]; j++) {
        const int u = snp_vars[j];
        if (n_mol) mol_snp += (double)n_mol[u];
        beta_snp += (double)bsum[u];
    }
    double scale = 1.0;
    if (n_mol) scale = scale + (double)n_mol[v] / (mol_snp + 100.0);
    scale = scale + (double)bsum[v] / (beta_snp + 100.0);
    out[i] = betas[i] + (float)(scale * default_prior);
}

template <int L, typename T>
static __device__ __forceinline__ T group_bcast(T v, int i, int gbase)
{
    static_assert(sizeof(T) == 4, "32-bit payloads");
    if (L == 64) {
        const int r = __builtin_amdgcn_readlane(__builtin_bit_cast(int, v), i);
        return __builtin_bit_cast(T, r);
    }
    return __shfl(v, gbase + i);
}

struct FastAcc {
    double mant;
    int expo;
};

template <int A, bool PAIRS, int H>
static __device__ __forceinline__ void estep_products(const npm::f32x2 (&p1)[H][A], const npm::f32x2 (&p2)[H][A],
                                                      const npm::f32x2 (&keep)[H], const npm::f32x2 (&flo)[H],
                                                      float (&prod)[A], int n_slots)
{
#pragma unroll
    for (int q = 0; q < H; q++) {
#pragma unroll
        for (int s = 0; s < A; s++) {
            if (A > 1 && s >= n_slots) continue;
            npm::f32x2 p = p1[q][s];
            if (PAIRS) p = (p + p2[q][s]) * 0.5f;
            npm::f32x2 t = p * keep[q];
            t = t + flo[q];
            prod[s] = (prod[s] * t.x) * t.y;
        }
    }
}

template <int A>
static __device__ __forceinline__ void estep_flush(float (&prod)[A], FastAcc (&acc)[A], int n_slots)
{
#pragma unroll
    for (int s = 0; s < A; s++) {
        if (A > 1 && s >= n_slots) continue;
        const float m = __builtin_amdgcn_frexp_mantf(prod[s]);
        acc[s].expo += __builtin_amdgcn_frexp_expf(prod[s]);
        acc[s].mant += (double)__builtin_amdgcn_logf(m);
        prod[s] = 1.0f;
    }
}

template <int A>
// ... 1796 lines not shown
                val[(r + 2) * 64 + lane] = 0.0f;
                val[(r + 3) * 64 + lane] = 0.0f;
                accumulate(v0);
                accumulate(v1);
                accumulate(v2);
                accumulate(v3);
            }
        };
        auto put_sparse = [&](int mine) {
#pragma unroll
            for (int t = 0; t < NZ_S; t++) {
                if (t > 0 && !__any(t < mine)) break;
                if (t < mine) {
                    const int g = genotype(code, t);
                    const int pos = __popcll(colmask[g] & below);
                    val[pos * 64 + g] = power_of(ps0[t] * keep);
                }
            }
        };
        auto put_dense_calls = [&](u64 todo, u64 &cm, bool prefetched) {
            if (prefetched) {
#pragma unroll
                for (int j = 0; j < DP; j++) {
                    if (todo) {
                        put_dense(__builtin_ctzll(todo), q0[j], cm);
                        todo &= todo - 1ull;
                    }
                }
            }
            while (todo) {
                float q[D];
                load_dense_rows(todo, d0, bm0, q);
#pragma unroll
                for (int j = 0; j < D; j++) {
                    if (todo) {
                        put_dense(__builtin_ctzll(todo), q[j], cm);
                        todo &= todo - 1ull;
                    }
                }
            }
        };

        u64 cm = transpose(mine_all);
        if (!__any(__popcll(cm) + __popcll(dense0) > R)) {
            put_dense_calls(dense0, cm, true);
            colmask[lane] = cm;
            put_sparse(mine_all);
            drain(cm);
        } else {
            int first_lane = 0, width = 32;
            while (first_lane < 64) {
                const u64 range = ((1ull << width) - 1ull) << first_lane;
                const int mine = (range & bit) ? mine_all : 0;
                cm = transpose(mine);
                if (width > R && __any(__popcll(cm) + __popcll(dense0 & range) > R)) {
                    width >>= 1;
                    continue;
                }
                put_dense_calls(dense0 & range, cm, false);
                colmask[lane] = cm;
                put_sparse(mine);
                drain(cm);
                first_lane += width;
            }
        }
        d0 = d1; d1 = d2; d2 = d3;
        fc0 = fc1; fc1 = fc2;
        dense0 = dense1;
        bm0 = bm1;
#pragma unroll
        for (int j = 0; j < DP; j++) q0[j] = q1[j];
#pragma unroll
        for (int t = 0; t < NZ_S; t++) ps0[t] = ps1[t];
    }
    if (lane < G) {
        if constexpr (FIXED) mstep_store_fixed(a, item, lane, acc_fixed, shift);
        else mstep_store(a, item, lane, acc);
    }
}

constexpr int MTILE_THREADS = 1024;
constexpr int MTILE_QUEUE = 96;

template <bool SQUARE>
__global__ __launch_bounds__(MTILE_THREADS) void k_mstep_tiles(MstepArgs a, MTileArgs t)
{
    if (dense_regime(a)) return;
    if (t.incr_state != nullptr && !incr_full(t.incr_state, a)) return;
    extern __shared__ __attribute__((aligned(16))) unsigned long long mt_acc[];
    __shared__ unsigned mt_queue[MTILE_THREADS / 64][2][MTILE_QUEUE];
    const int tile = t.order[blockIdx.x];
    const int v0 = t.first[tile], nv = t.first[tile + 1] - v0;
    const long long beg = t.ptr[tile], end = t.ptr[tile + 1];
    const int G = a.G;
    const long long K = a.K;
    for (int i = threadIdx.x; i < nv * G; i += MTILE_THREADS) mt_acc[i] = 0ull;
    __syncthreads();
    const int lane = threadIdx.x & 63;
    const int wave = __builtin_amdgcn_readfirstlane((int)(threadIdx.x >> 6));
    const int shift = __builtin_amdgcn_readfirstlane(t.shift[tile]);
    unsigned *q_rec = mt_queue[wave][0], *q_keep = mt_queue[wave][1];
    int queued = 0;
    auto power_of = [&](float c) { return SQUARE ? c * c : powf(c, a.power); };
    constexpr double MAGIC = 6755399441055744.0;
    auto add = [&](int index, float c) {
        const double d = __builtin_ldexp((double)c, shift) + MAGIC;
        const unsigned long long q = (unsigned long long)(__double_as_longlong(d) - __double_as_longlong(MAGIC));
        __hip_atomic_fetch_add(&mt_acc[index], q, __ATOMIC_RELAXED, __HIP_MEMORY_SCOPE_WORKGROUP);
    };
    auto flush = [&]() {
        __builtin_amdgcn_fence(__ATOMIC_RELEASE, "wavefront");
        __builtin_amdgcn_wave_barrier();
        __builtin_amdgcn_fence(__ATOMIC_ACQUIRE, "wavefront");
        constexpr int DB = 16;
        for (int q0 = 0; q0 < queued; q0 += DB) {
            float p[DB];
#pragma unroll
            for (int i = 0; i < DB; i++) {
                p[i] = 0.0f;
                if (q0 + i < queued && lane < G) p[i] = a.post[(size_t)(q_rec[q0 + i] & 0xFFFFFFu) * K + lane];
            }
#pragma unroll
            for (int i = 0; i < DB; i++)
                if (q0 + i < queued && lane < G) add((int)(q_rec[q0 + i] >> 24) * G + lane, power_of(p[i] * __uint_as_float(q_keep[q0 + i])));
        }
        __builtin_amdgcn_fence(__ATOMIC_RELEASE, "wavefront");
        __builtin_amdgcn_wave_barrier();
        queued = 0;
    };
    constexpr int UN = 4;
    for (long long c0 = beg + (long long)wave * (64 * UN); c0 < end; c0 += (long long)(MTILE_THREADS / 64) * 64 * UN) {
        uint2 rec[UN], code[UN];
#pragma unroll
        for (int u = 0; u < UN; u++) {
            const long long i = c0 + 64 * u + lane;
            rec[u] = make_uint2(0u, 0u);
            if (i < end) rec[u] = t.stream[i];
        }
#pragma unroll
        for (int u = 0; u < UN; u++) {
            const long long i = c0 + 64 * u + lane;
            code[u] = make_uint2(0u, 0u);
            if (i < end) code[u] = a.first[rec[u].x & 0xFFFFFFu];
        }
        float extra[UN][NZ_CODE - 1];
#pragma unroll
        for (int u = 0; u < UN; u++) {
            const int nnz = (int)(code[u].y & 127u);
            const float *__restrict__ post_row = a.post + (size_t)(rec[u].x & 0xFFFFFFu) * K;
#pragma unroll
            for (int j = 1; j < NZ_CODE; j++) {
                extra[u][j - 1] = 0.0f;
                if (nnz <= NZ_CODE && j < nnz) extra[u][j - 1] = post_row[(code[u].y >> (7 + 6 * j)) & 63u];
            }
        }
#pragma unroll
        for (int u = 0; u < UN; u++) {
            const unsigned row = rec[u].x & 0xFFFFFFu;
            const int base = (int)(rec[u].x >> 24) * G;
            const float keep = __uint_as_float(rec[u].y);
            const int nnz = (int)(code[u].y & 127u);
            if (nnz >= 1 && nnz <= NZ_CODE) {
                add(base + (int)((code[u].y >> 7) & 63u), power_of(__uint_as_float(code[u].x) * keep));
#pragma unroll
                for (int j = 1; j < NZ_CODE; j++)
                    if (j < nnz) add(base + (int)((code[u].y >> (7 + 6 * j)) & 63u), power_of(extra[u][j - 1] * keep));
            }
            const unsigned long long dense = __ballot(nnz > NZ_CODE);
            if (dense) {
                if (queued > MTILE_QUEUE - 64) flush();
                if (nnz > NZ_CODE) {
                    const int at = queued + __popcll(dense & ((1ull << lane) - 1ull));
                    q_rec[at] = rec[u].x;
                    q_keep[at] = rec[u].y;
                }
                queued += __popcll(dense);
            }
        }
    }
    if (queued) flush();
    __syncthreads();
    for (int i = threadIdx.x; i < nv * G; i += MTILE_THREADS) {
        const int r = (int)((unsigned)i / (unsigned)G), g = i - r * G;
        const long long v = v0 + r;
        const size_t o = (size_t)(a.prow ? (long long)a.prow[v] : v) * G + g;
        const double sum = __builtin_ldexp((double)(long long)mt_acc[i], -shift);
        if (a.out32) a.out32[o] = (float)sum;
        else a.out64[o] = sum;
        if (t.acc64) t.acc64[(size_t)v * G + g] = mt_acc[i];
    }
}

constexpr unsigned MINCR_COOLDOWN = 8;
static __device__ __forceinline__ bool mincr_differs(float now, float before, float floor)
{
    return __float_as_uint(now) != __float_as_uint(before) && !(fmaxf(now, before) < floor);
}

__global__ __launch_bounds__(256) void k_mincr_changes(MstepArgs a, MIncrArgs x)
{
    if (x.state[IS_VALID] == 0u || dense_regime(a)) return;
    const int lane = threadIdx.x & 63;
    const long long b = ((long long)blockIdx.x * 4 + (threadIdx.x >> 6)) * 16 + lane;
    bool look = false;
    if (lane < 16 && b < x.B) {
        const uint2 now = a.first[b], before = x.prev_first[b];
        look = !((now.y & 127u) == 1u && now.x == before.x && now.y == before.y);
    }
    for (unsigned long long m = __ballot(look); m != 0ull; m &= m - 1ull) {
        const long long bb = b - lane + __builtin_ctzll(m);
        bool differs = false;
        if (lane < a.G) differs = mincr_differs(a.post[(size_t)bb * a.K + lane], x.prev[(size_t)bb * a.G + lane], x.floor);
        const bool changed = __ballot(differs) != 0ull;
        if (lane == 0) {
            if (changed) {
                x.list[atomicAdd(x.state + IS_N, 1u)] = (int)bb;
                atomicAdd((unsigned long long *)(x.state + IS_CALLS), x.pair_ptr  ? 2ull * (unsigned long long)(x.pair_ptr[bb + 1] - x.pair_ptr[bb])
                                                                    : x.rec_ptr ? (unsigned long long)(x.rec_ptr[bb + 1] - x.rec_ptr[bb])
                                                                                : 2ull);
                if (x.changed_map) x.changed_map[bb] = 1;
            } else {
                x.prev_first[bb] = a.first[bb];
            }
        }
    }
}

template <bool SQUARE>
__global__ __launch_bounds__(256) void k_mincr_delta(MstepArgs a, MIncrArgs x)
{
    if (incr_full(x.state, a)) return;
    const int lane = threadIdx.x & 63;
    const unsigned n = x.state[IS_N];
    const int G = a.G;
    constexpr double MAGIC = 6755399441055744.0;
    auto quant = [&](float c, int shift) {
        const double d = __builtin_ldexp((double)(SQUARE ? c * c : powf(c, a.power)), shift) + MAGIC;
        return (unsigned long long)(__double_as_longlong(d) - __double_as_longlong(MAGIC));
    };
    const int wave = threadIdx.x >> 6;
    for (unsigned i = blockIdx.x; i < n; i += gridDim.x) {
        const long long b = x.list[i];
        float now = 0.0f, before = 0.0f;
        if (lane < G) {
            now = a.post[(size_t)b * a.K + lane];
            before = x.prev[(size_t)b * G + lane];
        }
        const unsigned long long mask = __ballot(lane < G && mincr_differs(now, before, x.floor));
        const bool indexed = x.rec_ptr != nullptr;
        const long long p0 = indexed ? x.rec_ptr[b] : x.pair_ptr[b];
        const int n_calls = indexed ? (int)(x.rec_ptr[b + 1] - p0) : 2 * (int)(x.pair_ptr[b + 1] - p0);
        for (int c0 = 64 * wave; c0 < n_calls; c0 += 256) {
            const int ci = c0 + lane;
            const bool mine = ci < n_calls;
            float keep = 0.0f;
            unsigned row = 0u;
            if (mine && indexed) {
                const uint2 d = x.rec[p0 + ci];
                row = d.x;
                keep = __uint_as_float(d.y);
            } else if (mine) {
                keep = x.pairs[p0 + (ci >> 1)].keep[ci & 1];
                row = x.call_rows != nullptr ? x.call_rows[2 * p0 + ci] : x.pairs[p0 + (ci >> 1)].row_off[ci & 1] / (4u * (unsigned)G);
                if (x.row_variant != nullptr) row = (unsigned)x.row_variant[row];
            }
            const int shift = mine ? (int)x.shift_v[row] : 0;
            for (unsigned long long m = mask; m != 0ull; m &= m - 1ull) {
                const int g = __builtin_ctzll(m);
                const float pn = __shfl(now, g), po = __shfl(before, g);
                const unsigned long long qn = quant(pn * keep, shift), qo = quant(po * keep, shift);
                if (mine && qn != qo) {
                    __hip_atomic_fetch_add(&x.acc64[(size_t)row * G + g], qn - qo, __ATOMIC_RELAXED, __HIP_MEMORY_SCOPE_AGENT);
                    x.touched[row] = 1;
// ... 366 lines not shown
            bv = ov;
            bi = oi;
        }
    }
    if (lane == 0) {
        best[b] = bi;
        best_p[b] = bv;
    }
}

__global__ __launch_bounds__(256) void k_test_log(const float *in, float *out, long long n)
{
    const long long i = (long long)blockIdx.x * blockDim.x + threadIdx.x;
    if (i < n) out[i] = npm::log_f32<true>(in[i]);
}

__global__ __launch_bounds__(256) void k_test_log_hot(const float *in, float *out, long long n)
{
    const long long i = ((long long)blockIdx.x * blockDim.x + threadIdx.x) * 2;
    if (i >= n) return;
    const bool has2 = i + 1 < n;
    const npm::f32x2 v = {in[i], has2 ? in[i + 1] : 1.0f};
    const npm::f32x2 r = npm::log_f32_hot2(v);
    out[i] = r.x;
    if (has2) out[i + 1] = r.y;
}

__global__ __launch_bounds__(256) void k_test_log2_hw(const float *in, float *out, long long n)
{
    const long long i = (long long)blockIdx.x * blockDim.x + threadIdx.x;
    if (i < n) out[i] = __builtin_amdgcn_logf(in[i]);
}

__global__ __launch_bounds__(256) void k_test_exp(const float *in, float *out, long long n)
{
    const long long i = (long long)blockIdx.x * blockDim.x + threadIdx.x;
    if (i < n) out[i] = npm::exp_f32(in[i]);
}

__global__ __launch_bounds__(64) void k_test_softmax(const float *in, float *out, long long rows, int cols)
{
    const long long r = blockIdx.x;
    const int lane = threadIdx.x;
    const float *x = in + (size_t)r * cols;
    float *y = out + (size_t)r * cols;
    float mx = -__builtin_inff();
    for (int c = lane; c < cols; c += 64) mx = fmaxf(mx, x[c]);
#pragma unroll
    for (int off = 1; off < 64; off <<= 1) mx = fmaxf(mx, __shfl_xor(mx, off));
    for (int c = lane; c < cols; c += 64) y[c] = npm::exp_f32(x[c] - mx);
    __threadfence_block();
    __syncthreads();
    const float tot = npm::row_sum_wave(y, cols, lane);
    __syncthreads();
    for (int c = lane; c < cols; c += 64) y[c] = y[c] / tot;
}

static inline unsigned blocks_for(long long n, int per_block) { return (unsigned)((n + per_block - 1) / per_block); }

template <typename T>
static hipError_t launch_pstep(hipStream_t st, const T *prior, const T *addition, const int *v2snp, const int *snp_ptr,
                               const int *snp_vars, long long v_begin, long long n_rows, long long n_snps, int G, const int *prow,
                               float lo, float hi, float *prob, unsigned short *prob16 = nullptr)
{
    if (n_rows * G == 0) return hipSuccess;
    const long long groups = n_snps >= 0 ? n_snps : n_rows;
#define PSTEP(L)                                                                                                          \
    hipLaunchKernelGGL((k_probs_from_betas<T, L>), dim3(blocks_for(groups, 4 * (64 / L))), dim3(256), 0, st, prior, addition, \
                       v2snp, snp_ptr, snp_vars, v_begin, n_rows, n_snps, G, prow, lo, hi, prob, prob16)
    if (G <= 4) PSTEP(4);
    else if (G <= 8) PSTEP(8);
    else if (G <= 16) PSTEP(16);
    else if (G <= 32) PSTEP(16);
    else PSTEP(32);
#undef PSTEP
    return hipGetLastError();
}

hipError_t launch_probs_from_betas(hipStream_t st, const float *prior, const float *addition, const int *v2snp,
                                   const int *snp_ptr, const int *snp_vars, long long v_begin, long long n_rows, long long n_snps,
                                   int G, const int *prow, float lo, float hi, float *prob, unsigned short *prob16)
{
    return launch_pstep<float>(st, prior, addition, v2snp, snp_ptr, snp_vars, v_begin, n_rows, n_snps, G, prow, lo, hi, prob, prob16);
}

hipError_t launch_probs_from_betas_f64(hipStream_t st, const double *betas, const int *v2snp, const int *snp_ptr,
                                       const int *snp_vars, long long V, long long n_snps, int G, const int *prow, float lo, float hi,
                                       float *prob)
{
    return launch_pstep<double>(st, betas, (const double *)nullptr, v2snp, snp_ptr, snp_vars, 0LL, V, n_snps, G, prow, lo, hi, prob);
}

__global__ __launch_bounds__(256) void k_check_unit_range(const float *__restrict__ x, long long n, int *__restrict__ flags)
{
    const long long i = (long long)blockIdx.x * blockDim.x + threadIdx.x;
    const bool bad = i < n && !(x[i < n ? i : 0] >= 0.0f && x[i < n ? i : 0] <= 1.0f);
    if (__ballot(bad) != 0ull && (threadIdx.x & 63) == 0) atomicOr(flags, 1);
}

hipError_t launch_build_coarse_stream(hipStream_t st, const CallPair *stream, const long long *bin_ptr, long long n_bins, unsigned zero_off,
                                      int cpg, long long *coarse_bin_ptr, unsigned *out, const int *bin_rows, int R, double *log2_keep)
{
    if (n_bins == 0) return hipSuccess;
    hipLaunchKernelGGL(k_coarse_bin_ptr, dim3(1), dim3(1024), 0, st, bin_ptr, n_bins, cpg, coarse_bin_ptr);
    static_assert(CoarseShape<1>::BPR == 1 && CoarseShape<2>::BPR == 2 && CoarseShape<4>::BPR == 4, "coarse_batches_per_record");
    if (cpg == 1)
        hipLaunchKernelGGL(k_build_coarse_stream<1>, dim3(blocks_for(n_bins, 4)), dim3(256), 0, st, stream, bin_ptr, coarse_bin_ptr, n_bins, zero_off, out, bin_rows, R, log2_keep);
    else if (cpg == 2)
        hipLaunchKernelGGL(k_build_coarse_stream<2>, dim3(blocks_for(n_bins, 4)), dim3(256), 0, st, stream, bin_ptr, coarse_bin_ptr, n_bins, zero_off, out, bin_rows, R, log2_keep);
    else
        hipLaunchKernelGGL(k_build_coarse_stream<4>, dim3(blocks_for(n_bins, 4)), dim3(256), 0, st, stream, bin_ptr, coarse_bin_ptr, n_bins, zero_off, out, bin_rows, R, log2_keep);
    return hipGetLastError();
}

hipError_t launch_prob_to_half(hipStream_t st, const float *prob, long long rows, int G, unsigned short *out, const unsigned *skip)
{
    const long long n = rows * G;
    if (n == 0) return hipSuccess;
    hipLaunchKernelGGL(k_prob_to_half, dim3(blocks_for(n, 256)), dim3(256), 0, st, prob, n, out, G, skip);
    return hipGetLastError();
}

hipError_t launch_check_unit_range(hipStream_t st, const float *x, long long n, int *flags)
{
    if (n == 0) return hipSuccess;
    hipLaunchKernelGGL(k_check_unit_range, dim3(blocks_for(n, 256)), dim3(256), 0, st, x, n, flags);
    return hipGetLastError();
}

template <int L, int A, int U>
static void launch_direct(hipStream_t st, const EstepArgs &a_in, bool pairs)
{
    EstepArgs a = a_in;
    const bool fast = a.fast && (!(pairs && L == 64 && A <= 8) || a.G <= PairRowShape<A>::GPAD);
    const bool split = L == 64 && fast && a.segs != nullptr && a.n_segs > 0 && a.order_count == nullptr;
    if (!split) a.segs = nullptr;
    const dim3 grid(blocks_for(split ? a.n_segs + (a.B - a.n_split) : a.B, 4 * (64 / L))), block(256);
    if (fast) {
        if (pairs)
            hipLaunchKernelGGL((k_estep_direct<L, A, true, U, true>), grid, block, 0, st, a);
        else
            hipLaunchKernelGGL((k_estep_direct<L, A, false, U, true>), grid, block, 0, st, a);
        if constexpr (L == 64) {
            if (split) hipLaunchKernelGGL((k_estep_join<A>), dim3(blocks_for(a.n_split, 4)), block, 0, st, a);
        }
    } else {
        if (pairs)
            hipLaunchKernelGGL((k_estep_direct<L, A, true, U, false>), grid, block, 0, st, a);
        else
            hipLaunchKernelGGL((k_estep_direct<L, A, false, U, false>), grid, block, 0, st, a);
    }
}

template <int A>
static hipError_t launch_block(hipStream_t st, const EstepArgs &a, int k_base)
{
    int C = (16384 / (4 * a.G)) & ~7;
    C = C < 8 ? 8 : (C > 128 ? 128 : C);
    size_t bytes = (size_t)(C + 2) * a.G * 4 + (size_t)C * 12;
    bytes = (bytes + 15) & ~size_t(15);
    const void *kernel = a.fast ? (const void *)k_estep_block<A, true> : (const void *)k_estep_block<A, false>;
    hipError_t e = hipFuncSetAttribute(kernel, hipFuncAttributeMaxDynamicSharedMemorySize, (int)bytes);
    if (e != hipSuccess) return e;
    if (a.fast)
        hipLaunchKernelGGL((k_estep_block<A, true>), dim3((unsigned)a.B), dim3(256), bytes, st, a, C, k_base);
    else
// ... 136 lines not shown
    do {                                                                                                           \
        if (a.fixed_shift_v != nullptr) {                                                                          \
            if (buf) hipLaunchKernelGGL((k_mstep_calls<SQ, 16, 4, true, true>), grid, dim3(256), 0, st, a);        \
            else hipLaunchKernelGGL((k_mstep_calls<SQ, 16, 4, false, true>), grid, dim3(256), 0, st, a);           \
        } else if (buf) hipLaunchKernelGGL((k_mstep_calls<SQ, 16, 4, true>), grid, dim3(256), 0, st, a);           \
        else hipLaunchKernelGGL((k_mstep_calls<SQ, 16, 4, false>), grid, dim3(256), 0, st, a);                     \
    } while (0)
        if (a.square)
            MSTEP_CALLS(true);
        else
            MSTEP_CALLS(false);
#undef MSTEP_CALLS
        if (a.dense_calls) {
            const dim3 dense_grid(std::min(blocks_for(a.n_items, 4), 2048u));
            if (a.square)
                hipLaunchKernelGGL((k_mstep_dense<true>), dense_grid, dim3(256), 0, st, a);
            else
                hipLaunchKernelGGL((k_mstep_dense<false>), dense_grid, dim3(256), 0, st, a);
        }
        return hipGetLastError();
    }
    if (G <= 128) launch_m<2, 4>(st, a);
    else if (G <= 256) launch_m<4, 2>(st, a);
    else if (G <= 512) launch_m<8, 2>(st, a);
    else if (G <= 1024) launch_m<16, 2>(st, a);
    else return hipErrorInvalidValue;
    return hipGetLastError();
}

hipError_t launch_mstep_incremental(hipStream_t st, const MstepArgs &a, const MTileArgs &t, const MIncrArgs &x)
{
    if (t.n_tiles == 0 || x.B == 0) return hipSuccess;
    hipLaunchKernelGGL(k_mincr_changes, dim3(blocks_for(x.B, 64)), dim3(256), 0, st, a, x);
    if (a.square)
        hipLaunchKernelGGL((k_mincr_delta<true>), dim3(4096), dim3(256), 0, st, a, x);
    else
        hipLaunchKernelGGL((k_mincr_delta<false>), dim3(4096), dim3(256), 0, st, a, x);
    const hipError_t e = launch_mstep_tiles(st, a, t);
    if (e != hipSuccess) return e;
    hipLaunchKernelGGL(k_mincr_finish, dim3(2048), dim3(256), 0, st, a, x);
    return hipGetLastError();
}

hipError_t launch_mstep_items_incremental(hipStream_t st, const MstepArgs &a, const MIncrArgs &x)
{
    if (a.n_items == 0 || x.B == 0 || a.fixed_shift_v == nullptr) return hipErrorInvalidValue;
    hipLaunchKernelGGL(k_mincr_changes, dim3(blocks_for(x.B, 64)), dim3(256), 0, st, a, x);
    if (a.square)
        hipLaunchKernelGGL((k_mincr_delta<true>), dim3(4096), dim3(256), 0, st, a, x);
    else
        hipLaunchKernelGGL((k_mincr_delta<false>), dim3(4096), dim3(256), 0, st, a, x);
    const hipError_t e = launch_mstep(st, a);
    if (e != hipSuccess) return e;
    hipLaunchKernelGGL(k_mincr_finish, dim3(2048), dim3(256), 0, st, a, x);
    return hipGetLastError();
}

hipError_t launch_mstep_incremental_sharded(hipStream_t st, const MstepArgs &a, const MTileArgs &t, const MIncrArgs &x)
{
    if (t.n_tiles == 0 || x.B == 0 || (x.changed_map == nullptr && x.rec_ptr == nullptr)) return hipErrorInvalidValue;
    hipLaunchKernelGGL(k_mincr_changes, dim3(blocks_for(x.B, 64)), dim3(256), 0, st, a, x);
    const dim3 grid(std::min(blocks_for(a.n_items, 4), 8192u));
    if (x.rec_ptr != nullptr) {
        if (a.square)
            hipLaunchKernelGGL((k_mincr_delta<true>), dim3(4096), dim3(256), 0, st, a, x);
        else
            hipLaunchKernelGGL((k_mincr_delta<false>), dim3(4096), dim3(256), 0, st, a, x);
    } else if (a.n_items) {
        if (a.square)
            hipLaunchKernelGGL((k_mincr_delta_masked<true>), grid, dim3(256), 0, st, a, x);
        else
            hipLaunchKernelGGL((k_mincr_delta_masked<false>), grid, dim3(256), 0, st, a, x);
    }
    const hipError_t e = launch_mstep_tiles(st, a, t);
    if (e != hipSuccess) return e;
    hipLaunchKernelGGL(k_mincr_finish, dim3(2048), dim3(256), 0, st, a, x);
    return hipGetLastError();
}

hipError_t launch_mstep_tiles(hipStream_t st, const MstepArgs &a, const MTileArgs &t)
{
    if (t.n_tiles == 0) return hipSuccess;
    const size_t lds = (size_t)t.tv * a.G * sizeof(unsigned long long);
    if (a.square)
        hipLaunchKernelGGL((k_mstep_tiles<true>), dim3((unsigned)t.n_tiles), dim3(MTILE_THREADS), lds, st, a, t);
    else
        hipLaunchKernelGGL((k_mstep_tiles<false>), dim3((unsigned)t.n_tiles), dim3(MTILE_THREADS), lds, st, a, t);
    if (a.dense_calls && a.n_items) {
        const dim3 grid(std::min(blocks_for(a.n_items, 4), 2048u));
        if (a.square)
            hipLaunchKernelGGL((k_mstep_dense<true>), grid, dim3(256), 0, st, a);
        else
            hipLaunchKernelGGL((k_mstep_dense<false>), grid, dim3(256), 0, st, a);
    }
    return hipGetLastError();
}

hipError_t launch_mcombine(hipStream_t st, const MstepArgs &a, const long long *item_ptr, long long v0, long long v1,
                           const int *prow, float *add32, double *add64, unsigned long long *redo, unsigned *n_redo, const int *vlist,
                           bool skip_single)
{
    if ((v1 - v0) * a.G <= 0) return hipSuccess;
    if (redo) {
        const hipError_t e = hipMemsetAsync(n_redo, 0, 2 * sizeof(unsigned), st);
        if (e != hipSuccess) return e;
    }
    const unsigned full_grid = blocks_for((v1 - v0) * a.G, 256);
    hipLaunchKernelGGL(k_mcombine, dim3(a.tiles_done ? std::min(full_grid, 1024u) : full_grid), dim3(256), 0, st, a.partial, item_ptr,
                       a.item_start, a.item_len, v0, v1, a.G, prow, add32, add64, redo, n_redo, a.redo_cap, vlist, skip_single,
                       a.dense_calls, a.total_calls, a.tiles_done, a.fixed_shift_v, a.fixed_acc64, a.fixed_state);
    if (!redo) return hipGetLastError();
    const dim3 grid(512), block(64 * EXACT_WAVES);
    if (a.square)
        hipLaunchKernelGGL((k_mstep_exact<true>), grid, block, 0, st, a, item_ptr, redo, n_redo, prow, add32, add64);
    else
        hipLaunchKernelGGL((k_mstep_exact<false>), grid, block, 0, st, a, item_ptr, redo, n_redo, prow, add32, add64);
    return hipGetLastError();
}

__device__ __forceinline__ void clear_peer_headers(unsigned *__restrict__ peers, unsigned long long block_words, int nranks, int own)
{
    if (peers == nullptr || blockIdx.x != 0 || threadIdx.x != 0) return;
    for (int r = 0; r < nranks; r++)
        if (r != own) peers[(size_t)r * block_words] = 0u;
}

__global__ __launch_bounds__(256) void k_post_compact_build(const uint2 *__restrict__ first, const float *__restrict__ post, long long B, int G,
                                                            unsigned cap, unsigned *__restrict__ block, float *__restrict__ sent,
                                                            unsigned char *__restrict__ sent_multi, unsigned *__restrict__ peers,
                                                            unsigned long long block_words, int nranks, int own)
{
    clear_peer_headers(peers, block_words, nranks, own);
    const int lane = threadIdx.x & 63;
    const long long b0 = ((long long)blockIdx.x * 4 + (threadIdx.x >> 6)) * 16;
    const long long b = b0 + lane;
    const bool in = lane < 16 && b < B;
    const bool multi = in && (first[in ? b : 0].y & 127u) > 1u;
    const bool was = in && sent_multi[in ? b : 0] != 0;
    if (in && !multi && was) sent_multi[b] = 0;
    const unsigned long long m = __ballot(multi), was_m = __ballot(multi && was);
    if (!m) return;
    unsigned long long dm = 0ull;
    for (unsigned long long mm = m; mm != 0ull; mm &= mm - 1ull) {
        const int src = __builtin_ctzll(mm);
        bool same = false;
        if ((was_m >> src) & 1ull) {
            const size_t o = (size_t)(b0 + src) * G + lane;
            const bool differs = lane < G && __float_as_uint(post[lane < G ? o : 0]) != __float_as_uint(sent[lane < G ? o : 0]);
            same = __ballot(differs) == 0ull;
        }
        if (!same) dm |= 1ull << src;
    }
    if (!dm) return;
    unsigned base = 0;
    if (lane == 0) base = atomicAdd(&block[0], (unsigned)__popcll(dm));
    base = (unsigned)__shfl((int)base, 0);
    for (unsigned i = 0; dm != 0ull; dm &= dm - 1ull, i++) {
        const long long row = b0 + __builtin_ctzll(dm);
        const unsigned at = base + i;
        if (at >= cap) break;
        unsigned *e = block + 4 + (size_t)at * (size_t)(1 + G);
        if (lane == 0) {
            e[0] = (unsigned)row;
            sent_multi[row] = 1;
        }
        if (lane < G) {
            const float v = post[(size_t)row * G + lane];
// ... 256 lines not shown
```

### demuxalot_amd/csrc/repack_device.hip

```cpp
#include <cstring>

#include <cstdlib>
#include <algorithm>
#include <hip/hip_runtime.h>
#include <rocprim/rocprim.hpp>

#include "dmx_ctx.h"

namespace dmx {
namespace {

__global__ __launch_bounds__(256) void k_validate(const int *__restrict__ variant, const int *__restrict__ cb,
                                                  const float *__restrict__ p_wrong, long long N, long long B, long long V,
                                                  unsigned long long *__restrict__ bad)
{
    const long long i = (long long)blockIdx.x * blockDim.x + threadIdx.x;
    const bool in = i < N;
    const bool bad_b = in && ((unsigned)cb[in ? i : 0] >= (unsigned long long)B);
    const bool bad_v = in && ((unsigned)variant[in ? i : 0] >= (unsigned long long)V);
    const float e = p_wrong[in ? i : 0];
    const bool bad_p = in && !(e >= 0.0f && e <= 1.0f);
    if (__ballot(bad_b || bad_v || bad_p) == 0ull) return;
    if (bad_b || bad_v || bad_p) {
        atomicMax(&bad[bad_b ? 0 : (bad_v ? 1 : 2)], 1ull);
// ... 581 lines not shown
__global__ __launch_bounds__(256) void k_mtile_keys(const uint2 *__restrict__ csc, const long long *__restrict__ item_start,
                                                    const int *__restrict__ item_len, const int *__restrict__ item_variant,
                                                    const unsigned *__restrict__ tile_of, const unsigned *__restrict__ vin_of,
                                                    unsigned row_bits, unsigned *__restrict__ keys, uint2 *__restrict__ rec)
{
    const long long item = blockIdx.x;
    const long long s0 = item_start[item];
    const int n = item_len[item];
    const int v = item_variant[item];
    const unsigned tile = tile_of[v], vin = vin_of[v];
    for (int i = threadIdx.x; i < n; i += 256) {
        const uint2 d = csc[s0 + i];
        keys[s0 + i] = (tile << row_bits) | d.x;
        rec[s0 + i] = make_uint2(d.x | (vin << 24), d.y);
    }
}
}

namespace {
__global__ __launch_bounds__(256) void k_mtile_from_rows(const CallPair *__restrict__ pairs, const long long *__restrict__ pair_ptr,
                                                         long long B, unsigned row_bytes, const unsigned *__restrict__ tile_vin,
                                                         unsigned sentinel, unsigned *__restrict__ keys, unsigned long long *__restrict__ rec)
{
    const int lane = threadIdx.x & 63;
    const long long b = (long long)blockIdx.x * 4 + (threadIdx.x >> 6);
    if (b >= B) return;
    const long long p0 = pair_ptr[b];
    const long long n_pairs = pair_ptr[b + 1] - p0;
    for (long long j = lane; j < n_pairs; j += 64) {
        const uint4 lo = ((const uint4 *)(pairs + p0 + j))[0];
        const uint4 hi = ((const uint4 *)(pairs + p0 + j))[1];
        const unsigned row_off[2] = {lo.x, lo.y}, keep[2] = {lo.z, lo.w}, floor_bits[2] = {hi.x, hi.y};
        unsigned key[2];
        unsigned long long r[2];
#pragma unroll
        for (int h = 0; h < 2; h++) {
            const bool padding = keep[h] == 0u && floor_bits[h] == 0x3F800000u && row_off[h] == 0u;
            const unsigned tv = tile_vin[row_off[h] / row_bytes];
            key[h] = padding ? sentinel : tv >> 7;
            r[h] = (unsigned long long)((unsigned)b | ((tv & 127u) << 24)) | ((unsigned long long)keep[h] << 32);
        }
        *(uint2 *)(keys + 2 * (p0 + j)) = make_uint2(key[0], key[1]);
        *(ulonglong2 *)(rec + 2 * (p0 + j)) = make_ulonglong2(r[0], r[1]);
    }
}

__global__ __launch_bounds__(256) void k_tile_ptr(const unsigned *__restrict__ sorted_keys, long long n, long long n_tiles,
                                                  long long *__restrict__ ptr)
{
    const long long k = (long long)blockIdx.x * blockDim.x + threadIdx.x;
    if (k > n_tiles) return;
    long long lo = 0, hi = n;
    while (lo < hi) {
        const long long mid = (lo + hi) >> 1;
        if ((long long)sorted_keys[mid] < k) lo = mid + 1; else hi = mid;
    }
    ptr[k] = lo;
}

int sort_pairs64(Scratch &sc, const unsigned *keys_in, unsigned *keys_out, const unsigned long long *vals_in,
                 unsigned long long *vals_out, size_t n, unsigned end_bit, hipStream_t st)
{
    if (n == 0) return 0;
    size_t bytes = 0;
    HIP_TRY(rocprim::radix_sort_pairs(nullptr, bytes, keys_in, keys_out, vals_in, vals_out, n, 0u, end_bit, st));
    char *tmp = nullptr;
    DMX_TRY(sc.get(&tmp, bytes));
    HIP_TRY(rocprim::radix_sort_pairs(tmp, bytes, keys_in, keys_out, vals_in, vals_out, n, 0u, end_bit, st));
    return 0;
}
}

void release_mstep_tiles(dmx_ctx *c)
{
    dev_free(c, c->d_mt_stream);
    dev_free(c, c->d_mt_ptr);
    dev_free(c, c->d_mt_first);
    dev_free(c, c->d_mt_order);
    dev_free(c, c->d_mt_shift);
    dev_free(c, c->d_mt_shift_v);
    c->incr_valid = false;
    c->n_mt = 0;
    c->mt_tv = 0;
    c->mt_tried = false;
    c->mt_shift_tried = false;
}

namespace {
struct TileCut {
    std::vector<int> tile_first;
    std::vector<long long> tile_ptr;
    std::vector<unsigned> tile_of, vin_of;
    std::vector<int> tile_shift;
    int tv = 0;
    unsigned row_bits = 0;
    long long n_mt = 0;
};

bool cut_mstep_tiles(dmx_ctx *c, long long v_lo, long long v_hi, TileCut &t)
{
    const int G = c->G;
    const long long rows = c->mshard ? c->rows_total : c->B, m = c->n_csc;
    if (G < 1 || G > 64 || rows >= (1LL << 24) || m == 0 || m >= (1LL << 32) || v_hi <= v_lo) return false;
    const long long V = c->V;
    if ((long long)c->h_col_ptr.size() != V + 1 || c->h_col_ptr[(size_t)V] != m) return false;
    const std::vector<long long> &first_call = c->h_col_ptr;
    if (first_call[(size_t)v_lo] != 0 || first_call[(size_t)v_hi] != m) return false;
    if (!c->n_simd) {
        int cus = 0;
        if (hipDeviceGetAttribute(&cus, hipDeviceAttributeMultiprocessorCount, c->device) != hipSuccess) return false;
        c->n_simd = 4 * cus;
    }
    t.tv = std::max(1, std::min<int>(dmx::MTILE_MAX_VARIANTS, dmx::MTILE_LDS_BYTES / (G * 8)));
    t.row_bits = bits_for(rows ? (unsigned long long)rows - 1 : 0);
    t.tile_of.assign((size_t)V, 0u);
    t.vin_of.assign((size_t)V, 0u);
    long long cap = std::max<long long>(4096, m / std::max(1, c->n_simd));
    for (int attempt = 0;; attempt++) {
        t.tile_first.clear();
        t.tile_ptr.clear();
        long long v = v_lo;
        while (v < v_hi) {
            t.tile_first.push_back((int)v);
            t.tile_ptr.push_back(first_call[(size_t)v]);
            long long w = v + 1;
            while (w < v_hi && w - v < t.tv && first_call[(size_t)w + 1] - first_call[(size_t)v] <= cap) w++;
            for (long long x = v; x < w; x++) {
                t.tile_of[(size_t)x] = (unsigned)(t.tile_first.size() - 1);
                t.vin_of[(size_t)x] = (unsigned)(x - v);
            }
            v = w;
        }
        const unsigned tile_bits = bits_for(t.tile_first.empty() ? 0 : (unsigned long long)t.tile_first.size() - 1);
        if (tile_bits + t.row_bits <= 32) break;
        if (cap >= m || attempt > 40) return false;
        cap *= 2;
    }
    t.n_mt = (long long)t.tile_first.size();
    t.tile_first.push_back((int)v_hi);
    t.tile_ptr.push_back(m);
    t.tile_shift.resize((size_t)t.n_mt);
    for (long long i = 0; i < t.n_mt; i++) {
        long long longest = 1;
        for (long long v = t.tile_first[(size_t)i]; v < t.tile_first[(size_t)i + 1]; v++)
            longest = std::max(longest, first_call[(size_t)v + 1] - first_call[(size_t)v]);
        t.tile_shift[(size_t)i] = std::min(50, 62 - (int)bits_for((unsigned long long)longest));
    }
    return true;
}

int upload_variant_shifts(dmx_ctx *c, const TileCut &t)
{
    const long long V = c->V;
    std::vector<unsigned char> shift_v((size_t)V);
    for (long long v = 0; v < V; v++) shift_v[(size_t)v] = (unsigned char)t.tile_shift[(size_t)t.tile_of[(size_t)v]];
    if (!c->d_mt_shift_v.p) DMX_TRY(dev_alloc(c, c->d_mt_shift_v, (size_t)V));
    HIP_TRY(hipMemcpyAsync(c->d_mt_shift_v.p, shift_v.data(), (size_t)V, hipMemcpyHostToDevice, c->stream));
    HIP_TRY(hipStreamSynchronize(c->stream));
    return 0;
}
}

namespace {
__global__ __launch_bounds__(256) void k_slice_rows(const uint2 *__restrict__ csc, const long long *__restrict__ item_start, const int *__restrict__ item_len,
                                                    const int *__restrict__ item_variant, long long n_items, unsigned *__restrict__ keys,
                                                    unsigned long long *__restrict__ vals)
{
    const long long item = (long long)blockIdx.x * 4 + (threadIdx.x >> 6);
    if (item >= n_items) return;
    const long long s0 = item_start[item];
    const unsigned long long v = (unsigned long long)(unsigned)item_variant[item];
    for (int i = threadIdx.x & 63; i < item_len[item]; i += 64) {
        const uint2 d = csc[s0 + i];
        keys[s0 + i] = d.x;
        vals[s0 + i] = v | ((unsigned long long)d.y << 32);
    }
}
}

int build_slice_row_index(dmx_ctx *c)
{
    if (c->d_slice_rec.p != nullptr || c->slice_index_tried) return 0;
    c->slice_index_tried = true;
    const char *env = std::getenv("DEMUXALOT_AMD_SLICE_INDEX");
    if (env && atoi(env) == 0) return 0;
    const long long m = c->n_csc, rows = c->rows_total;
    if (!c->mshard || m == 0 || rows == 0 || m >= (1LL << 32) || c->d_item_variant.p == nullptr) return 0;
    hipStream_t st = c->stream;
    Scratch sc(c);
    unsigned *keys = nullptr, *keys_out = nullptr;
    unsigned long long *vals = nullptr;
    DMX_TRY(sc.get(&keys, (size_t)m));
    DMX_TRY(sc.get(&keys_out, (size_t)m));
    DMX_TRY(sc.get(&vals, (size_t)m));
    hipLaunchKernelGGL(k_slice_rows, dim3((unsigned)((c->n_items + 3) / 4)), dim3(256), 0, st, c->d_csc.p, c->d_item_start.p, c->d_item_len.p,
                       c->d_item_variant.p, c->n_items, keys, vals);
    DMX_TRY(dev_alloc(c, c->d_slice_rec, (size_t)m));
    DMX_TRY(sort_pairs64(sc, keys, keys_out, vals, (unsigned long long *)c->d_slice_rec.p, (size_t)m, bits_for((unsigned long long)(rows - 1)), st));
    DMX_TRY(dev_alloc(c, c->d_slice_ptr, (size_t)rows + 1));
    hipLaunchKernelGGL(k_tile_ptr, dim3(grid_for(rows + 1)), dim3(256), 0, st, keys_out, m, rows, c->d_slice_ptr.p);
    HIP_TRY(hipGetLastError());
    HIP_TRY(hipStreamSynchronize(st));
    return 0;
}

int plan_mstep_shifts(dmx_ctx *c)
{
    if (c->d_mt_shift_v.p != nullptr || c->mt_shift_tried) return 0;
    c->mt_shift_tried = true;
    if (c->mshard) return 0;
    TileCut t;
    if (!cut_mstep_tiles(c, 0, c->V, t)) return 0;
    return upload_variant_shifts(c, t);
}

int build_mstep_tiles(dmx_ctx *c, long long v_lo, long long v_hi)
{
    release_mstep_tiles(c);
    c->mt_tried = true;
    TileCut cut;
    if (!cut_mstep_tiles(c, v_lo, v_hi, cut)) return 0;
    const int G = c->G;
    const long long m = c->n_csc;
    hipStream_t st = c->stream;
    const long long V = c->V;
    const int tv = cut.tv;
    const unsigned row_bits = cut.row_bits;
    std::vector<int> &tile_first = cut.tile_first;
    std::vector<long long> &tile_ptr = cut.tile_ptr;
    std::vector<unsigned> &tile_of = cut.tile_of, &vin_of = cut.vin_of;
    std::vector<int> &tile_shift = cut.tile_shift;
    const long long n_mt = cut.n_mt;
    std::vector<int> order((size_t)n_mt);
    for (long long i = 0; i < n_mt; i++) order[(size_t)i] = (int)i;
    std::stable_sort(order.begin(), order.end(), [&](int x, int y) {
        return tile_ptr[(size_t)x + 1] - tile_ptr[(size_t)x] > tile_ptr[(size_t)y + 1] - tile_ptr[(size_t)y];
    });
    Scratch sc(c);
    unsigned *d_tile_of = nullptr, *d_vin_of = nullptr, *keys = nullptr, *keys_out = nullptr, *iota = nullptr, *perm = nullptr;
    uint2 *rec = nullptr;
    DMX_TRY(sc.get(&d_tile_of, (size_t)V));
    DMX_TRY(sc.get(&d_vin_of, (size_t)V));
    if (!c->mshard && !c->sliced && c->d_call_pairs.p != nullptr && v_lo == 0 && v_hi == V && c->n_pairs > 0 && 2 * c->n_pairs < (1LL << 32)) {
        const size_t n = (size_t)(2 * c->n_pairs);
        unsigned long long *vals = nullptr;
        DMX_TRY(sc.get(&keys, n));
        DMX_TRY(sc.get(&keys_out, n));
        DMX_TRY(sc.get(&vals, n));
        DMX_TRY(upload_variant_shifts(c, cut));
        for (long long v = 0; v < V; v++) tile_of[(size_t)v] = (tile_of[(size_t)v] << 7) | vin_of[(size_t)v];
        HIP_TRY(hipMemcpyAsync(d_tile_of, tile_of.data(), sizeof(unsigned) * V, hipMemcpyHostToDevice, st));
        DMX_TRY(dev_alloc(c, c->d_mt_stream, n));
        hipLaunchKernelGGL(k_mtile_from_rows, dim3((unsigned)((c->B + 3) / 4)), dim3(256), 0, st, c->d_call_pairs.p, c->d_pair_ptr.p, c->B,
                           (unsigned)G * 4u, d_tile_of, (unsigned)n_mt, keys, vals);
        DMX_TRY(sort_pairs64(sc, keys, keys_out, vals, (unsigned long long *)c->d_mt_stream.p, n, bits_for((unsigned long long)n_mt), st));
        DMX_TRY(dev_alloc(c, c->d_mt_ptr, (size_t)n_mt + 1));
        hipLaunchKernelGGL(k_tile_ptr, dim3(grid_for(n_mt + 1)), dim3(256), 0, st, keys_out, (long long)n, n_mt, c->d_mt_ptr.p);
        DMX_TRY(dev_alloc(c, c->d_mt_first, (size_t)n_mt + 1));
        DMX_TRY(dev_alloc(c, c->d_mt_order, (size_t)n_mt));
        DMX_TRY(dev_alloc(c, c->d_mt_shift, (size_t)n_mt));
        HIP_TRY(hipMemcpyAsync(c->d_mt_shift.p, tile_shift.data(), sizeof(int) * n_mt, hipMemcpyHostToDevice, st));
        HIP_TRY(hipMemcpyAsync(c->d_mt_first.p, tile_first.data(), sizeof(int) * (n_mt + 1), hipMemcpyHostToDevice, st));
        HIP_TRY(hipMemcpyAsync(c->d_mt_order.p, order.data(), sizeof(int) * n_mt, hipMemcpyHostToDevice, st));
        HIP_TRY(hipGetLastError());
        HIP_TRY(hipStreamSynchronize(st));
        c->n_mt = n_mt;
        c->mt_tv = tv;
        return 0;
    }
    DMX_TRY(upload_variant_shifts(c, cut));
    DMX_TRY(sc.get(&keys, (size_t)m));
    DMX_TRY(sc.get(&keys_out, (size_t)m));
    DMX_TRY(sc.get(&iota, (size_t)m));
    DMX_TRY(sc.get(&perm, (size_t)m));
    DMX_TRY(sc.get(&rec, (size_t)m));
    HIP_TRY(hipMemcpyAsync(d_tile_of, tile_of.data(), sizeof(unsigned) * V, hipMemcpyHostToDevice, st));
    HIP_TRY(hipMemcpyAsync(d_vin_of, vin_of.data(), sizeof(unsigned) * V, hipMemcpyHostToDevice, st));
    hipLaunchKernelGGL(k_mtile_keys, dim3((unsigned)c->n_items), dim3(256), 0, st, c->d_csc.p, c->d_item_start.p, c->d_item_len.p, c->d_item_variant.p,
                       d_tile_of, d_vin_of, row_bits, keys, rec);
    hipLaunchKernelGGL(k_iota, dim3(grid_for(m)), dim3(256), 0, st, iota, m);
    const unsigned tile_bits = bits_for(n_mt > 1 ? (unsigned long long)n_mt - 1 : 0);
    DMX_TRY(sort_pairs(sc, keys, keys_out, iota, perm, (size_t)m, std::max(1u, tile_bits + row_bits), st));
    DMX_TRY(dev_alloc(c, c->d_mt_stream, (size_t)m));
    hipLaunchKernelGGL(k_permute_records, dim3(grid_for(m)), dim3(256), 0, st, perm, rec, m, c->d_mt_stream.p);
    DMX_TRY(dev_alloc(c, c->d_mt_ptr, (size_t)n_mt + 1));
    DMX_TRY(dev_alloc(c, c->d_mt_first, (size_t)n_mt + 1));
    DMX_TRY(dev_alloc(c, c->d_mt_order, (size_t)n_mt));
    DMX_TRY(dev_alloc(c, c->d_mt_shift, (size_t)n_mt));
    HIP_TRY(hipMemcpyAsync(c->d_mt_shift.p, tile_shift.data(), sizeof(int) * n_mt, hipMemcpyHostToDevice, st));
    HIP_TRY(hipMemcpyAsync(c->d_mt_ptr.p, tile_ptr.data(), sizeof(long long) * (n_mt + 1), hipMemcpyHostToDevice, st));
    HIP_TRY(hipMemcpyAsync(c->d_mt_first.p, tile_first.data(), sizeof(int) * (n_mt + 1), hipMemcpyHostToDevice, st));
    HIP_TRY(hipMemcpyAsync(c->d_mt_order.p, order.data(), sizeof(int) * n_mt, hipMemcpyHostToDevice, st));
    HIP_TRY(hipGetLastError());
    HIP_TRY(hipStreamSynchronize(st));
    c->n_mt = n_mt;
    c->mt_tv = tv;
    return 0;
}

int repack_on_device(dmx_ctx *c, const int32_t *h_variant, const int32_t *h_cb, const float *h_p)
{
    const long long N = c->N;
    hipStream_t st = c->stream;
    Scratch sc(c);
    int *d_variant = nullptr, *d_cb = nullptr;
    float *d_p = nullptr;
    DMX_TRY(sc.get(&d_variant, (size_t)N));
    DMX_TRY(sc.get(&d_cb, (size_t)N));
    DMX_TRY(sc.get(&d_p, (size_t)N));
    if (N) {
        HIP_TRY(hipMemcpyAsync(d_variant, h_variant, sizeof(int) * N, hipMemcpyHostToDevice, st));
        HIP_TRY(hipMemcpyAsync(d_cb, h_cb, sizeof(int) * N, hipMemcpyHostToDevice, st));
        HIP_TRY(hipMemcpyAsync(d_p, h_p, sizeof(float) * N, hipMemcpyHostToDevice, st));
    }
    return repack_core(c, sc, d_variant, d_cb, d_p);
}

namespace {

__host__ __device__ inline unsigned long long variant_key(int chrom, int pos, unsigned char base)
{
    return ((unsigned long long)(unsigned)chrom << 35) | ((unsigned long long)(unsigned)pos << 3) | (unsigned long long)(base & 7);
}

constexpr unsigned long long EMPTY_SLOT = ~0ull;

__device__ __forceinline__ unsigned long long slot_of(unsigned long long key, unsigned bits)
{
    return (key * 0x9E3779B97F4A7C15ull) >> (64u - bits);
}

__global__ __launch_bounds__(256) void k_table_insert(const int *chrom, const int *pos, const unsigned char *base, long long V,
                                                      unsigned bits, unsigned long long *tkeys, unsigned *trows)
{
    const long long v = (long long)blockIdx.x * blockDim.x + threadIdx.x;
    if (v >= V) return;
    const unsigned long long key = variant_key(chrom[v], pos[v], base[v]), mask = (1ull << bits) - 1ull;
    for (unsigned long long h = slot_of(key, bits);; h = (h + 1ull) & mask) {
        const unsigned long long seen = atomicCAS(&tkeys[h], EMPTY_SLOT, key);
        if (seen == EMPTY_SLOT || seen == key) {
            atomicMin(&trows[h], (unsigned)v);
            return;
        }
    }
}

__global__ __launch_bounds__(256) void k_match(const int *chrom, const int *pos, const unsigned char *base, const int *cb,
                                               long long n, const unsigned long long *tkeys, const unsigned *trows,
                                               unsigned bits, int *call_variant, unsigned *flag, int *bad)
{
    const long long i = (long long)blockIdx.x * blockDim.x + threadIdx.x;
    if (i >= n) return;
    const unsigned long long q = variant_key(chrom[i], pos[i], base[i]), mask = (1ull << bits) - 1ull;
    int v = -1;
    for (unsigned long long h = slot_of(q, bits);; h = (h + 1ull) & mask) {
        const unsigned long long k = tkeys[h];
        if (k == q) v = (int)trows[h];
        if (k == q || k == EMPTY_SLOT) break;
    }
    call_variant[i] = v;
    flag[i] = v >= 0 ? 1u : 0u;
    if (v >= 0 && cb[i] < 0) atomicMax(bad, 1);
}

__global__ __launch_bounds__(256) void k_variant_counts(const unsigned long long *sorted_keys, long long m, long long V,
                                                        unsigned long long *counts)
{
    const long long v = (long long)blockIdx.x * blockDim.x + threadIdx.x;
    if (v >= V) return;
    auto lower = [&](unsigned long long key) {
        long long lo = 0, hi = m;
        while (lo < hi) {
            const long long mid = (lo + hi) >> 1;
            if (sorted_keys[mid] < key) lo = mid + 1; else hi = mid;
        }
        return lo;
    };
    counts[v] = (unsigned long long)(lower((unsigned long long)(v + 1) << 32) - lower((unsigned long long)v << 32));
}
// ... 303 lines not shown
```

### demuxalot_amd/device.py

```python
import ctypes
import os
import threading

import numpy as np

from . import _lib
from ._lib import DMX_F32, DMX_F64, as_c, check, ptr


DEFAULT_ESTEP_MODE = 'guarded'


class DeviceContext:
    def __init__(self, device=0):
        self._lib = _lib.load()
        handle = ctypes.c_void_p()
        check(self._lib.dmx_create(int(device), ctypes.byref(handle)))
        self._h = handle
        self.device = int(device)
        self.B = self.V = self.G = self.N = 0
        self.K = 0
        self._resident_key = None
        self._keep_molecule_calls = False
        self._snp_shape = (0, 0)
        self.apply_environment()

    def apply_environment(self):
        mode = os.environ.get('DEMUXALOT_AMD_ESTEP', '') or DEFAULT_ESTEP_MODE
        assert mode in ('exact', 'fast', 'guarded'), f'DEMUXALOT_AMD_ESTEP={mode!r}: exact, fast or guarded'
        self.set_estep_mode(mode)
        exact_additions = os.environ.get('DEMUXALOT_AMD_EXACT_ADDITIONS', '')
        self.set_exact_additions(mode == 'exact' if exact_additions == '' else exact_additions != '0')
        self.set_estep_schedule(os.environ.get('DEMUXALOT_AMD_ESTEP_SCHEDULE', 'auto'))
        self.set_estep_dictionary(os.environ.get('DEMUXALOT_AMD_ESTEP_DICT', 'auto'))
        self.set_estep_packing(os.environ.get('DEMUXALOT_AMD_ESTEP_PACKED', 'auto'))
        self.set_coarse_pass(os.environ.get('DEMUXALOT_AMD_COARSE_PASS', '1') != '0')
        self.set_mstep_incremental(os.environ.get('DEMUXALOT_AMD_MSTEP_INCREMENTAL', '1') != '0')
        self.set_lean_memory(os.environ.get('DEMUXALOT_AMD_LEAN', '0') not in ('', '0'))
        self.set_phase_timers(False)
        self.set_logits_needed(True)

    def __enter__(self):
        return self

    def __exit__(self, *_exc):
        self.close()

    def close(self):
        if getattr(self, '_h', None):
            self._lib.dmx_destroy(self._h)
            self._h = None

    def __del__(self):
        try:
            self.close()
        except Exception:
            pass

    def set_problem(self, n_barcodes, n_variants, n_genotypes, variant_id, compressed_cb, p_base_wrong, v2snp):
        self._resident_key = None
        variant_id = as_c(variant_id, np.int32)
        compressed_cb = as_c(compressed_cb, np.int32)
        p_base_wrong = as_c(p_base_wrong, np.float32)
        v2snp = as_c(v2snp, np.int32)
        assert len(variant_id) == len(compressed_cb) == len(p_base_wrong)
        assert len(v2snp) == n_variants
        check(self._lib.dmx_set_problem(self._h, n_barcodes, n_variants, n_genotypes, len(variant_id),
                                        ptr(variant_id), ptr(compressed_cb), ptr(p_base_wrong), ptr(v2snp)))
        self.B, self.V, self.G, self.N = int(n_barcodes), int(n_variants), int(n_genotypes), len(variant_id)

    def pack_and_set_problem(self, n_barcodes, n_genotypes, var_chrom, var_pos, var_base, v2snp,
                             call_chrom, call_pos, call_base, call_cb, call_p):
        self._resident_key = None
        var_chrom, var_pos, var_base = as_c(var_chrom, np.int32), as_c(var_pos, np.int32), as_c(var_base, np.uint8)
        v2snp = as_c(v2snp, np.int32)
        call_chrom, call_pos = as_c(call_chrom, np.int32), as_c(call_pos, np.int32)
        call_base, call_cb, call_p = as_c(call_base, np.uint8), as_c(call_cb, np.int32), as_c(call_p, np.float32)
        n_variants, n_calls = len(var_pos), len(call_pos)
        assert len(v2snp) == n_variants
        mol_per_variant = np.zeros(n_variants, dtype=np.int64)
        n_matched, n_unique = ctypes.c_int64(0), ctypes.c_int64(0)
        check(self._lib.dmx_pack_and_set_problem(
            self._h, n_barcodes, n_variants, n_genotypes, ptr(var_chrom), ptr(var_pos), ptr(var_base), ptr(v2snp),
            n_calls, ptr(call_chrom), ptr(call_pos), ptr(call_base), ptr(call_cb), ptr(call_p),
            ctypes.byref(n_matched), ctypes.byref(n_unique), ptr(mol_per_variant)))
        self.B, self.V, self.G, self.N = int(n_barcodes), int(n_variants), int(n_genotypes), n_unique.value
        return n_matched.value, n_unique.value, mol_per_variant

    def _container_list(self, containers):
        from .snp_counter import MOLECULE_DTYPE, SNP_CALL_DTYPE

        class Container(ctypes.Structure):
            _fields_ = [('snp_calls', ctypes.c_void_p), ('n_snp_calls', ctypes.c_int64),
                        ('molecules', ctypes.c_void_p), ('n_molecules', ctypes.c_int64), ('chrom', ctypes.c_int32)]

        keep_alive, parts = [], (Container * max(1, len(containers)))()
        for k, (chrom, snp_calls, molecules) in enumerate(containers):
            assert snp_calls.dtype == SNP_CALL_DTYPE and molecules.dtype == MOLECULE_DTYPE
            snp_calls, molecules = np.ascontiguousarray(snp_calls), np.ascontiguousarray(molecules)
            keep_alive += [snp_calls, molecules]
            parts[k] = Container(snp_calls.ctypes.data, len(snp_calls), molecules.ctypes.data, len(molecules), int(chrom))
        return parts, keep_alive

    def pack_containers_and_set_problem(self, n_barcodes, n_genotypes, var_chrom, var_pos, var_base, v2snp, containers):
        self._resident_key = None
        var_chrom, var_pos, var_base = as_c(var_chrom, np.int32), as_c(var_pos, np.int32), as_c(var_base, np.uint8)
        v2snp = as_c(v2snp, np.int32)
        n_variants = len(var_pos)
        assert len(v2snp) == n_variants
        parts, _keep_alive = self._container_list(containers)
        mol_per_variant = np.zeros(n_variants, dtype=np.int64)
        n_matched, n_unique = ctypes.c_int64(0), ctypes.c_int64(0)
        check(self._lib.dmx_pack_containers_and_set_problem(
            self._h, n_barcodes, n_variants, n_genotypes, ptr(var_chrom), ptr(var_pos), ptr(var_base), ptr(v2snp),
            ctypes.cast(parts, ctypes.c_void_p), len(containers), ctypes.byref(n_matched), ctypes.byref(n_unique),
            ptr(mol_per_variant)))
        self.B, self.V, self.G, self.N = int(n_barcodes), int(n_variants), int(n_genotypes), n_unique.value
        return n_matched.value, n_unique.value, mol_per_variant

    def stage_containers(self, containers):
        self._resident_key = None
# ... 356 lines not shown
        check(self._lib.dmx_get_coverage_timings(self._h, ms))
        return dict(zip(_lib.COVERAGE_STAGES, ms))

    def set_coverage_form(self, form):
        check(self._lib.dmx_set_coverage_form(self._h, int(form)))

    def get_top_options(self, k):
        options = np.empty((self.B, int(k)), dtype=np.int32)
        probs = np.empty((self.B, int(k)), dtype=np.float32)
        check(self._lib.dmx_get_top_options(self._h, int(k), ptr(options), ptr(probs)))
        return options, probs

    def get_option_sums(self):
        out = np.empty(self.K, dtype=np.float64)
        check(self._lib.dmx_get_option_sums(self._h, ptr(out)))
        return out

    def synchronize(self):
        check(self._lib.dmx_synchronize(self._h))

    @staticmethod
    def new_unique_id() -> bytes:
        buf = ctypes.create_string_buffer(_lib.UNIQUE_ID_BYTES)
        check(_lib.load().dmx_comm_unique_id(buf))
        return buf.raw

    def comm_init(self, rank, nranks, unique_id: bytes, reduce_dtype='f64'):
        assert len(unique_id) == _lib.UNIQUE_ID_BYTES
        buf = ctypes.create_string_buffer(unique_id, _lib.UNIQUE_ID_BYTES)
        check(self._lib.dmx_comm_init(self._h, int(rank), int(nranks), buf, DMX_F64 if reduce_dtype == 'f64' else DMX_F32))

    def comm_init_host(self, rank, nranks, collective, reduce_dtype='f64'):
        names = {_lib.COLL_ALL_REDUCE: 'all_reduce', _lib.COLL_REDUCE_SCATTER: 'reduce_scatter', _lib.COLL_ALL_GATHER: 'all_gather'}

        def trampoline(_user, op, buf, count, dtype):
            try:
                kind = np.float64 if dtype == DMX_F64 else np.float32
                n = count if op == _lib.COLL_ALL_REDUCE else count * nranks
                raw = (ctypes.c_char * (n * np.dtype(kind).itemsize)).from_address(buf)
                view = np.frombuffer(raw, dtype=kind)
                collective(names[op], view if op == _lib.COLL_ALL_REDUCE else view.reshape(nranks, count))
                return 0
            except Exception:
                import traceback
                traceback.print_exc()
                return 1
        self._host_collective = _lib.HOST_COLLECTIVE(trampoline)
        check(self._lib.dmx_comm_init_host(self._h, int(rank), int(nranks), self._host_collective, None,
                                           DMX_F64 if reduce_dtype == 'f64' else DMX_F32))

    def comm_init_emulated(self, rank, nranks, link_gbytes_per_s=50.0, latency_us=10.0, reduce_dtype='f64'):
        check(self._lib.dmx_comm_init_emulated(self._h, int(rank), int(nranks), float(link_gbytes_per_s), float(latency_us),
                                               DMX_F64 if reduce_dtype == 'f64' else DMX_F32))

    def exchange_compact(self):
        taken, overflows, cap = ctypes.c_int64(0), ctypes.c_int64(0), ctypes.c_int64(0)
        check(self._lib.dmx_get_exchange_compact(self._h, ctypes.byref(taken), ctypes.byref(overflows), ctypes.byref(cap)))
        return int(taken.value), int(overflows.value), int(cap.value)

    def exchange_compact_table(self):
        taken, overflows, cap = ctypes.c_int64(0), ctypes.c_int64(0), ctypes.c_int64(0)
        check(self._lib.dmx_get_exchange_compact_table(self._h, ctypes.byref(taken), ctypes.byref(overflows), ctypes.byref(cap)))
        return int(taken.value), int(overflows.value), int(cap.value)

    def exchange_mode(self):
        mode = ctypes.c_int32(0)
        check(self._lib.dmx_get_exchange_mode(self._h, ctypes.byref(mode)))
        return {0: None, 1: 'variant', 2: 'reduce_scatter', 3: 'allreduce'}[mode.value]

    def set_estep_mode(self, mode):
        check(self._lib.dmx_set_estep_mode(self._h, {'exact': 0, 'fast': 1, 'guarded': 2}[mode]))

    def guard_stats(self):
        last, total, rows = ctypes.c_int64(0), ctypes.c_int64(0), ctypes.c_int64(0)
        check(self._lib.dmx_get_guard_stats(self._h, ctypes.byref(last), ctypes.byref(total), ctypes.byref(rows)))
        return last.value, total.value, rows.value

    def set_guard_adaptive(self, adaptive):
        check(self._lib.dmx_set_guard_adaptive(self._h, int(bool(adaptive))))

    def set_coarse_pass(self, coarse):
        check(self._lib.dmx_set_coarse_pass(self._h, 2 if coarse == 'always' else int(bool(coarse))))

    def set_lean_memory(self, lean):
        check(self._lib.dmx_set_lean_memory(self._h, int(bool(lean))))

    def set_mstep_incremental(self, incremental):
        check(self._lib.dmx_set_mstep_incremental(self._h, 2 if incremental == 'bootstrap' else int(bool(incremental))))

    def mstep_incremental(self):
        full, delta, last = ctypes.c_int64(), ctypes.c_int64(), ctypes.c_int64()
        check(self._lib.dmx_get_mstep_incremental(self._h, ctypes.byref(full), ctypes.byref(delta), ctypes.byref(last)))
        return full.value, delta.value, last.value

    def guard_levels(self):
        level = ctypes.c_int32()
        steps, fine, coarse = ctypes.c_int64(), ctypes.c_int64(), ctypes.c_int64()
        c_ms, f_ms, e_ms = ctypes.c_double(), ctypes.c_double(), ctypes.c_double()
        check(self._lib.dmx_get_guard_levels(self._h, ctypes.byref(level), ctypes.byref(steps), ctypes.byref(fine), ctypes.byref(coarse),
                                             ctypes.byref(c_ms), ctypes.byref(f_ms), ctypes.byref(e_ms)))
        return {'level': level.value, 'coarse_steps': steps.value, 'flagged_fine': fine.value, 'flagged_coarse': coarse.value,
                'coarse_pass_ms': c_ms.value, 'fine_pass_ms': f_ms.value, 'exact_pass_ms': e_ms.value}

    def set_logits_needed(self, needed):
        check(self._lib.dmx_set_logits_needed(self._h, int(bool(needed))))

    def guard_probes(self):
        probes, streak = ctypes.c_int64(), ctypes.c_int64()
        check(self._lib.dmx_get_guard_probes(self._h, ctypes.byref(probes), ctypes.byref(streak)))
        return probes.value, streak.value

    def debug_set_pass_ms(self, coarse=-1.0, fine=-1.0, exact=-1.0):
        check(self._lib.dmx_debug_set_pass_ms(self._h, float(coarse), float(fine), float(exact)))

    def guard_direct(self):
        return self.guard_state()[:3]

    def guard_state(self):
        last, steps, would = ctypes.c_int32(0), ctypes.c_int64(0), ctypes.c_int64(0)
        fast_ms, exact_ms = ctypes.c_double(0), ctypes.c_double(0)
        check(self._lib.dmx_get_guard_direct(self._h, ctypes.byref(last), ctypes.byref(steps), ctypes.byref(would),
                                             ctypes.byref(fast_ms), ctypes.byref(exact_ms)))
        return bool(last.value), steps.value, would.value, fast_ms.value, exact_ms.value

    def set_estep_dictionary(self, mode):
        check(self._lib.dmx_set_estep_dictionary(self._h, {'never': 0, 'auto': 1, 'always': 2}[mode]))

    def estep_form(self):
        import ctypes
        form, distinct = ctypes.c_int32(0), ctypes.c_int32(0)
        check(self._lib.dmx_get_estep_form(self._h, ctypes.byref(form), ctypes.byref(distinct)))
        return {0: None, 1: 'direct', 2: 'dict', 3: 'dict_block', 4: 'packed'}[form.value], distinct.value

    def set_estep_packing(self, mode):
        check(self._lib.dmx_set_estep_packing(self._h, {'never': 0, 'auto': 1, 'always': 2, 'split': 3}[mode]))

    def set_estep_schedule(self, schedule):
        check(self._lib.dmx_set_estep_schedule(self._h, {'direct': 0, 'auto': 1, 'tiled': 2}[schedule]))

    def set_mstep_wide_addresses(self, wide):
        check(self._lib.dmx_set_mstep_wide_addresses(self._h, int(bool(wide))))

    def set_mstep_tiles(self, mode):
        if isinstance(mode, str):
            mode = {'never': 0, 'auto': 1, 'always': 2}[mode]
        check(self._lib.dmx_set_mstep_tiles(self._h, int(mode) if not isinstance(mode, bool) else (2 if mode else 0)))

    def set_msteps_expected(self, n):
        check(self._lib.dmx_set_msteps_expected(self._h, int(n)))

    def mstep_tiles_info(self):
        built, ms = ctypes.c_int32(0), ctypes.c_double(0)
        check(self._lib.dmx_get_mstep_tiles_info(self._h, ctypes.byref(built), ctypes.byref(ms)))
        return bool(built.value), ms.value

    def mstep_form(self):
        form = ctypes.c_int32(0)
        check(self._lib.dmx_get_mstep_form(self._h, ctypes.byref(form)))
        return {0: None, 1: 'items', 2: 'tiles', 3: 'items_fixed'}[form.value]

    def redo_count(self):
        n = ctypes.c_int64(0)
        check(self._lib.dmx_get_redo_count(self._h, ctypes.byref(n)))
        return n.value

    def set_exact_additions(self, exact):
# ... 136 lines not shown
```

### include/demux_hip_debug.h

```cpp
#ifndef DEMUX_HIP_DEBUG_H
#define DEMUX_HIP_DEBUG_H

#include "demux_hip.h"

#ifdef __cplusplus
extern "C" {
#endif

int dmx_get_redo_count(dmx_ctx *ctx, int64_t *count);

int dmx_set_mstep_tiles(dmx_ctx *ctx, int enable);
int dmx_get_mstep_tiles_info(dmx_ctx *ctx, int32_t *built, double *build_ms);
int dmx_get_mstep_form(dmx_ctx *ctx, int32_t *form);

int dmx_set_guard_adaptive(dmx_ctx *ctx, int adaptive);
int dmx_set_coarse_pass(dmx_ctx *ctx, int coarse);

int dmx_set_mstep_incremental(dmx_ctx *ctx, int incremental);
int dmx_get_mstep_incremental(dmx_ctx *ctx, int64_t *full_passes, int64_t *delta_passes, int64_t *barcodes_changed_last);
int dmx_get_guard_levels(dmx_ctx *ctx, int32_t *level_last, int64_t *coarse_steps, int64_t *flagged_fine_last, int64_t *flagged_coarse_last,
                         double *coarse_pass_ms, double *fine_pass_ms, double *exact_pass_ms);
int dmx_get_guard_probes(dmx_ctx *ctx, int64_t *probes, int64_t *streak);
int dmx_debug_set_pass_ms(dmx_ctx *ctx, double coarse_pass_ms, double fine_pass_ms, double exact_pass_ms);
int dmx_get_guard_direct(dmx_ctx *ctx, int32_t *last_ran_direct, int64_t *direct_steps, int64_t *would_queue_last, double *fast_pass_ms,
                         double *exact_pass_ms);

int dmx_set_estep_schedule(dmx_ctx *ctx, int tiled);

#define DMX_FORM_NONE 0
#define DMX_FORM_DIRECT 1
#define DMX_FORM_DICT 2
#define DMX_FORM_DICT_BLOCK 3
#define DMX_FORM_PACKED 4
int dmx_set_estep_dictionary(dmx_ctx *ctx, int mode);
int dmx_get_estep_form(dmx_ctx *ctx, int32_t *form, int32_t *distinct_values);

int dmx_set_estep_packing(dmx_ctx *ctx, int mode);

int dmx_set_mstep_wide_addresses(dmx_ctx *ctx, int wide);

int dmx_comm_init_emulated(dmx_ctx *ctx, int rank, int nranks, double link_gbytes_per_s, double latency_us, int reduce_dtype);

int dmx_get_exchange_compact(dmx_ctx *ctx, int64_t *taken, int64_t *overflows, int64_t *capacity_rows);
int dmx_get_exchange_compact_table(dmx_ctx *ctx, int64_t *taken, int64_t *overflows, int64_t *capacity_rows);

int dmx_test_logf(dmx_ctx *ctx, const float *in, float *out, int64_t n);
int dmx_test_logf_hot(dmx_ctx *ctx, const float *in, float *out, int64_t n);
int dmx_test_expf(dmx_ctx *ctx, const float *in, float *out, int64_t n);
int dmx_test_log2_hw(dmx_ctx *ctx, const float *in, float *out, int64_t n);
int dmx_test_softmax(dmx_ctx *ctx, const float *in, float *out, int64_t rows, int64_t cols);

int dmx_get_guard_stats(dmx_ctx *ctx, int64_t *redone_last, int64_t *redone_total, int64_t *rows_total);

#define DMX_EXCHANGE_NONE 0
#define DMX_EXCHANGE_VARIANT 1
#define DMX_EXCHANGE_REDUCE_SCATTER 2
#define DMX_EXCHANGE_ALLREDUCE 3
int dmx_get_exchange_mode(dmx_ctx *ctx, int32_t *mode);

int dmx_runtime_info(char *out, int64_t capacity);

int dmx_count_reads_begin(dmx_ctx *ctx, const int32_t *positions, int64_t n_positions, const double *qual_table41);
int dmx_count_reads_push(dmx_ctx *ctx, const dmx_decoded_reads *chunk, int final, int64_t *n_molecules, int64_t *n_calls);
int dmx_count_reads_end(dmx_ctx *ctx);

int dmx_get_count_reads_timings(dmx_ctx *ctx, double *stage_ms);
int dmx_get_count_reads_carry(dmx_ctx *ctx, int64_t *n_reads);
int dmx_get_count_reads_peak_bytes(dmx_ctx *ctx, int64_t *bytes);

#define DMX_COVERAGE_ATOMIC 0
#define DMX_COVERAGE_TILED 1
int dmx_set_coverage_form(dmx_ctx *ctx, int form);
int dmx_get_coverage_timings(dmx_ctx *ctx, double *stage_ms);

int dmx_reads_upload(dmx_ctx *ctx, const dmx_decoded_reads *reads, int64_t *handle);
int dmx_reads_release(dmx_ctx *ctx, int64_t handle);
int dmx_reads_info(dmx_ctx *ctx, int64_t handle, int64_t *info);
int dmx_count_reads_resident(dmx_ctx *ctx, int64_t handle, const int32_t *positions, int64_t n_positions, const double *qual_table41,
                             int64_t *n_molecules, int64_t *n_calls);
int dmx_coverage_count_resident(dmx_ctx *ctx, int64_t handle, int32_t start, int32_t stop, int32_t quality_threshold,
                                int32_t *coverage_out);
int dmx_count_reads_push_resident(dmx_ctx *ctx, int64_t handle, int64_t first_read, int64_t last_read, int final, int64_t *n_molecules,
                                  int64_t *n_calls);
int dmx_get_reads_upload_bytes(dmx_ctx *ctx, int64_t *bytes);

#ifdef __cplusplus
}
#endif
#endif
```

Before: 185.6 million.

## Fuse next P-step into tiled M-step tail with dense-fallback P-step kernel

When M-step tiles hold whole SNPs, the tiled M-step kernel now also computes the next iteration's genotype probability table (f32 and optional f16), so the separate P-step pass and the mcombine launch are skipped. Tile cutting is adjusted so SNP groups are not split across tiles. A conditional dense-path kernel recomputes probabilities when the M-step took the dense route. This removes a full-table read/write pass per EM iteration. In exchange it adds cross-step state, more complex tile boundaries, and a risk of stale tables if the arming logic misfires.

Result: no change. 185.9 million, median of 6 (+0.2%).

```diff
diff --git a/demuxalot_amd/_lib.py b/demuxalot_amd/_lib.py
--- a/demuxalot_amd/_lib.py
+++ b/demuxalot_amd/_lib.py
@@ -86,6 +86,9 @@
     'dmx_coverage_fetch_candidates': (c_int, [_P, _P, _P]),
 }
 DEBUG_SIGNATURES = {
+    'dmx_set_fused_tail': (c_int, [_P, c_int]),
+    'dmx_get_fused_tail': (c_int, [_P, POINTER(c_int32), POINTER(c_int64)]),
+    'dmx_debug_get_prob_tables': (c_int, [_P, _P, _P, POINTER(c_int32)]),
     'dmx_comm_init_emulated': (c_int, [_P, c_int, c_int, c_double, c_double, c_int]),
     'dmx_get_exchange_compact': (c_int, [_P, POINTER(c_int64), POINTER(c_int64), POINTER(c_int64)]),
     'dmx_get_exchange_compact_table': (c_int, [_P, POINTER(c_int64), POINTER(c_int64), POINTER(c_int64)]),
diff --git a/demuxalot_amd/csrc/dmx_api.cpp b/demuxalot_amd/csrc/dmx_api.cpp
--- a/demuxalot_amd/csrc/dmx_api.cpp
+++ b/demuxalot_amd/csrc/dmx_api.cpp
@@ -281,6 +281,23 @@
     if (!c) return fail(DMX_ERR_INVALID, "null context");
     if (coarse < 0 || coarse > 2) return fail(DMX_ERR_INVALID, "coarse pass: 0 never, 1 where the logits are not read, 2 wherever the shape allows");
     c->coarse_pass = coarse;
+    return 0;
+}
+
+int dmx_set_fused_tail(dmx_ctx *c, int fused)
+{
+    if (!c) return fail(DMX_ERR_INVALID, "null context");
+    if (fused < 0 || fused > 1) return fail(DMX_ERR_INVALID, "fused tail: 0 or 1");
+    c->fused_tail = fused;
+    c->next_pstep = dmx_ctx::NextPstep{};
+    return 0;
+}
+
+int dmx_get_fused_tail(dmx_ctx *c, int32_t *snps_whole_in_tiles, int64_t *fused_msteps)
+{
+    if (!c) return fail(DMX_ERR_INVALID, "null context");
+    if (snps_whole_in_tiles) *snps_whole_in_tiles = c->n_mt > 0 && c->mt_snp_whole ? 1 : 0;
+    if (fused_msteps) *fused_msteps = (int64_t)c->fused_msteps;
     return 0;
 }
 
diff --git a/demuxalot_amd/csrc/dmx_ctx.h b/demuxalot_amd/csrc/dmx_ctx.h
--- a/demuxalot_amd/csrc/dmx_ctx.h
+++ b/demuxalot_amd/csrc/dmx_ctx.h
@@ -125,6 +125,17 @@
     bool mt_tried = false;
     bool mt_shift_tried = false;
     int mstep_tiles = 1;
+    int fused_tail = 1;
+    bool mt_snp_whole = false;
+    long long fused_msteps = 0;
+    struct NextPstep {
+        bool armed = false;
+        bool done = false;
+        bool with_half = false;
+        float lo = 0.0f, hi = 0.0f;
+        const unsigned long long *dense_calls = nullptr;
+        unsigned long long total_calls = 0;
+    } next_pstep;
     long long msteps_done = 0;
     long long incr_rows = 0;
     DevBuf<unsigned char> d_incr_map;
diff --git a/demuxalot_amd/csrc/dmx_steps.cpp b/demuxalot_amd/csrc/dmx_steps.cpp
--- a/demuxalot_amd/csrc/dmx_steps.cpp
+++ b/demuxalot_amd/csrc/dmx_steps.cpp
@@ -178,6 +178,8 @@
 
 int run_pstep(dmx_ctx *c, float lo, float hi, bool with_addition, bool with_half)
 {
+    const dmx_ctx::NextPstep fused = c->next_pstep;
+    c->next_pstep = dmx_ctx::NextPstep{};
     const bool half_rows = with_half && c->sliced && c->prob_list_words != 0 && c->prob_prev_valid && c->prob16_valid && c->d_prob16.p != nullptr;
     with_half = with_half && !c->sliced;
     if (with_half) DMX_TRY(ensure_prob16(c));
@@ -186,6 +188,16 @@
     SpanGuard ev_guard{c, &ev};
     timer_begin(c, DMX_T_PSTEP, &ev);
     const long long v0 = c->sliced ? c->cut[c->rank] : 0, v1 = c->sliced ? c->cut[c->rank + 1] : c->V;
+    if (fused.done && with_addition && !c->sliced && fused.lo == lo && fused.hi == hi && fused.with_half == with_half) {
+        HIP_TRY(dmx::launch_probs_if_dense(c->stream, fused.dense_calls, fused.total_calls, c->d_prior.p, c->d_add.p, c->d_snp_ptr.p, c->d_snp_vars.p,
+                                           (long long)c->S, c->G, lo, hi, c->d_prob.p, with_half ? c->d_prob16.p : nullptr));
+        c->prob16_valid = with_half;
+        timer_end(c, DMX_T_PSTEP, ev);
+        c->have_probs = true;
+        c->p_clip_lo = lo;
+        c->dict_candidate = c->add_is_zero;
+        return 0;
+    }
     if (c->emulated && c->sliced && !c->emu_table_filled) {
         for (int r = 0; r < c->nranks; r++)
             if (r != c->rank)
@@ -490,6 +502,8 @@
 
 int run_mstep(dmx_ctx *c, float power)
 {
+    const dmx_ctx::NextPstep announced = c->next_pstep;
+    c->next_pstep = dmx_ctx::NextPstep{};
     const bool mshard = c->mshard;
     const size_t row_base = mshard ? (size_t)c->rank * (size_t)c->rows_pad : 0;
     const int Wn = (c->G + 63) / 64;
@@ -663,6 +677,20 @@
     } else {
         c->incr_valid = false;
     }
+    const bool fuse = c->fused_tail && announced.armed && !dist && !mshard && !c->sliced && a.tiles_done && !incremental && c->mt_snp_whole &&
+                      a.out32 == c->d_add.p && a.prow == nullptr && c->prob_rows == c->V && c->d_prior.p != nullptr;
+    if (fuse) {
+        if (announced.with_half) DMX_TRY(ensure_prob16(c));
+        tiles.p_prior = c->d_prior.p;
+        tiles.p_v2snp = c->d_v2snp.p;
+        tiles.p_snp_ptr = c->d_snp_ptr.p;
+        tiles.p_snp_vars = c->d_snp_vars.p;
+        tiles.p_prob = c->d_prob.p;
+        tiles.p_prob16 = announced.with_half ? c->d_prob16.p : nullptr;
+        tiles.p_lo = announced.lo;
+        tiles.p_hi = announced.hi;
+        c->prob16_valid = false;
+    }
     timer_begin(c, DMX_T_MSTEP, &ev);
     if (sharded_incr) HIP_TRY(dmx::launch_mstep_incremental_sharded(c->stream, a, tiles, incr));
     else if (incremental && fixed_items) HIP_TRY(dmx::launch_mstep_items_incremental(c->stream, a, incr));
@@ -671,7 +699,15 @@
     else HIP_TRY(dmx::launch_mstep(c->stream, a));
     c->mstep_form = a.tiles_done ? 2 : (incremental && fixed_items ? 3 : 1);
     timer_end(c, DMX_T_MSTEP, ev);
+    if (fuse) {
+        c->next_pstep = announced;
+        c->next_pstep.done = true;
+        c->next_pstep.dense_calls = a.dense_calls;
+        c->next_pstep.total_calls = a.total_calls;
+        c->fused_msteps++;
+    }
     if (!dist) {
+        if (c->fused_tail && a.tiles_done && redo == nullptr && a.dense_calls == nullptr) return 0;
         timer_begin(c, DMX_T_MCOMBINE, &ev);
         HIP_TRY(dmx::launch_mcombine(c->stream, a, c->d_item_ptr.p, 0, c->V, nullptr, c->d_add.p, nullptr, redo, c->d_n_redo.p, nullptr, true));
         timer_end(c, DMX_T_MCOMBINE, ev);
@@ -726,6 +762,7 @@
 {
     DMX_TRY(bind(c));
     DMX_TRY(need(c, c->have_problem, "dmx_set_problem before dmx_set_addition"));
+    c->next_pstep = dmx_ctx::NextPstep{};
     const size_t vg = (size_t)c->V * c->G;
     c->incr_valid = false;
     if (addition) {
@@ -743,8 +780,23 @@
 {
     DMX_TRY(bind(c));
     DMX_TRY(need(c, c->have_problem && c->have_betas, "dmx_set_problem + dmx_set_betas before dmx_probs_from_betas"));
+    c->next_pstep = dmx_ctx::NextPstep{};
     DMX_TRY(run_pstep(c, lo, hi, true));
     DMX_TRY(copy_prob_out(c, prob_out));
+    HIP_TRY(hipStreamSynchronize(c->stream));
+    return 0;
+}
+
+int dmx_debug_get_prob_tables(dmx_ctx *c, float *prob_out, uint16_t *prob16_out, int32_t *prob16_valid)
+{
+    DMX_TRY(bind(c));
+    DMX_TRY(need(c, c->have_problem && c->have_probs, "a genotype table before dmx_debug_get_prob_tables"));
+    if (c->sliced) return fail(DMX_ERR_INVALID, "dmx_debug_get_prob_tables: one context's own table only");
+    DMX_TRY(copy_prob_out(c, prob_out));
+    const bool half = c->prob16_valid && c->d_prob16.p != nullptr;
+    if (prob16_valid) *prob16_valid = half ? 1 : 0;
+    if (prob16_out && half)
+        HIP_TRY(hipMemcpyAsync(prob16_out, c->d_prob16.p, sizeof(unsigned short) * 2 * (size_t)c->V * c->G, hipMemcpyDeviceToHost, c->stream));
     HIP_TRY(hipStreamSynchronize(c->stream));
     return 0;
 }
@@ -814,6 +866,7 @@
 {
     DMX_TRY(bind(c));
     DMX_TRY(need(c, c->have_problem && c->have_post, "dmx_estep before dmx_mstep"));
+    c->next_pstep = dmx_ctx::NextPstep{};
     DMX_TRY(run_mstep(c, power));
     if (addition_out) DMX_TRY(ensure_full_addition(c));
     DMX_TRY(copy_out(c, addition_out, c->d_add.p, (size_t)c->V * c->G));
@@ -827,6 +880,7 @@
 {
     DMX_TRY(bind(c));
     DMX_TRY(need(c, c->have_problem && c->have_betas, "dmx_set_problem + dmx_set_betas before dmx_em"));
+    c->next_pstep = dmx_ctx::NextPstep{};
     if (n_iterations < 1) return fail(DMX_ERR_INVALID, "n_iterations must be >= 1");
     if (!penalties) return fail(DMX_ERR_INVALID, "null penalties");
     DMX_TRY(ensure_options(c, with_doublets, penalties));
@@ -843,6 +897,11 @@
         DMX_TRY(run_estep(c, with_doublets, it == 0 && prior_logits != nullptr, prior_dtype, power, kept));
         if (it + 1 < n_iterations) {
             c->msteps_ahead = n_iterations - 1 - it;
+            c->next_pstep = dmx_ctx::NextPstep{};
+            c->next_pstep.armed = true;
+            c->next_pstep.lo = lo;
+            c->next_pstep.hi = hi;
+            c->next_pstep.with_half = !(it + 2 == n_iterations && keep_last) && coarse_capable(c, with_doublets, lo);
             const int rc_m = run_mstep(c, power);
             c->msteps_ahead = 0;
             if (rc_m) return rc_m;
@@ -862,6 +921,7 @@
     DMX_TRY(bind(c));
     DMX_TRY(need(c, c->have_problem && c->have_betas && c->have_post && c->K > 0,
                  "dmx_estep or dmx_em (to fix the options) before dmx_run_iterations"));
+    c->next_pstep = dmx_ctx::NextPstep{};
     if (n_iterations < 0) return fail(DMX_ERR_INVALID, "negative n_iterations");
     const int with_doublets = c->K != c->G;
     for (int it = 0; it < n_iterations; it++) {
@@ -869,11 +929,22 @@
         DMX_TRY(run_pstep(c, lo, hi, true, !kept && coarse_capable(c, with_doublets, lo)));
         DMX_TRY(run_estep(c, with_doublets, false, DMX_F32, power, kept));
         c->msteps_ahead = n_iterations - it;
+        c->next_pstep = dmx_ctx::NextPstep{};
+        if (it + 1 < n_iterations) {
+            c->next_pstep.armed = true;
+            c->next_pstep.lo = lo;
+            c->next_pstep.hi = hi;
+            c->next_pstep.with_half = !(it + 2 == n_iterations && c->logits_needed) && coarse_capable(c, with_doublets, lo);
+        }
         const int rc_m = run_mstep(c, power);
         c->msteps_ahead = 0;
-        if (rc_m) return rc_m;
-    }
-    return 0;
-}
-
-}
+        if (rc_m) {
+            c->next_pstep = dmx_ctx::NextPstep{};
+            return rc_m;
+        }
+    }
+    c->next_pstep = dmx_ctx::NextPstep{};
+    return 0;
+}
+
+}
diff --git a/demuxalot_amd/csrc/host_stubs.cpp b/demuxalot_amd/csrc/host_stubs.cpp
--- a/demuxalot_amd/csrc/host_stubs.cpp
+++ b/demuxalot_amd/csrc/host_stubs.cpp
@@ -102,6 +102,8 @@
 hipError_t launch_sum_dense(hipStream_t, unsigned long long *, unsigned *) { return hipSuccess; }
 hipError_t launch_probs_from_betas(hipStream_t, const float *, const float *, const int *, const int *, const int *, long long, long long,
                                    long long, int, const int *, float, float, float *, unsigned short *) { return hipSuccess; }
+hipError_t launch_probs_if_dense(hipStream_t, const unsigned long long *, unsigned long long, const float *, const float *, const int *, const int *,
+                                 long long, int, float, float, float *, unsigned short *) { return hipSuccess; }
 hipError_t launch_probs_from_betas_f64(hipStream_t, const double *, const int *, const int *, const int *, long long, long long, int,
                                        const int *, float, float, float *) { return hipSuccess; }
 hipError_t launch_check_unit_range(hipStream_t, const float *, long long, int *) { return hipSuccess; }
diff --git a/demuxalot_amd/csrc/kernels.h b/demuxalot_amd/csrc/kernels.h
--- a/demuxalot_amd/csrc/kernels.h
+++ b/demuxalot_amd/csrc/kernels.h
@@ -195,6 +195,9 @@
 hipError_t launch_probs_from_betas(hipStream_t st, const float *prior, const float *addition, const int *v2snp,
                                    const int *snp_ptr, const int *snp_vars, long long v_begin, long long n_rows, long long n_snps,
                                    int G, const int *prow, float lo, float hi, float *prob, unsigned short *prob16 = nullptr);
+hipError_t launch_probs_if_dense(hipStream_t st, const unsigned long long *dense_calls, unsigned long long total_calls, const float *prior,
+                                 const float *addition, const int *snp_ptr, const int *snp_vars, long long n_snps, int G, float lo, float hi,
+                                 float *prob, unsigned short *prob16);
 hipError_t launch_probs_from_betas_f64(hipStream_t st, const double *betas, const int *v2snp, const int *snp_ptr,
                                        const int *snp_vars, long long V, long long n_snps, int G, const int *prow, float lo,
                                        float hi, float *prob);
@@ -223,6 +226,11 @@
     int tv;
     unsigned long long *acc64;
     const unsigned *incr_state;
+    const float *p_prior;
+    const int *p_v2snp, *p_snp_ptr, *p_snp_vars;
+    float *p_prob;
+    unsigned short *p_prob16;
+    float p_lo, p_hi;
 };
 struct MIncrArgs {
     unsigned *state;
diff --git a/demuxalot_amd/csrc/kernels.hip b/demuxalot_amd/csrc/kernels.hip
--- a/demuxalot_amd/csrc/kernels.hip
+++ b/demuxalot_amd/csrc/kernels.hip
@@ -10,6 +10,43 @@
 #include "estep_epilogue.h"
 
 namespace dmx {
+
+constexpr int PSTEP_HELD = 4;
+template <typename T, typename Beta>
+static __device__ __forceinline__ void pstep_column(const long long (&w)[PSTEP_HELD], int j0, int j1, const int *__restrict__ snp_vars, int g,
+                                                    int G, const int *__restrict__ prow, float clip_lo, float clip_hi,
+                                                    float *__restrict__ prob, unsigned short *__restrict__ prob16, Beta beta)
+{
+    constexpr int HELD = PSTEP_HELD;
+    T held[HELD];
+#pragma unroll
+    for (int q = 0; q < HELD; q++) {
+        held[q] = (T)0;
+        if (w[q] >= 0) held[q] = beta(w[q], g);
+    }
+    double den = 0.0;
+#pragma unroll
+    for (int q = 0; q < HELD; q++) den += (double)held[q];
+    for (int j = j0 + HELD; j < j1; j++) den += (double)beta((long long)snp_vars[j], g);
+    den = fmax(den, 1e-7);
+#pragma unroll
+    for (int q = 0; q < HELD; q++) {
+        if (w[q] < 0) continue;
+        float p = (float)((double)held[q] / den);
+        p = fminf(fmaxf(p, clip_lo), clip_hi);
+        const long long row = prow ? (long long)prow[w[q]] : w[q];
+        prob[row * G + g] = p;
+        if (prob16) prob16[row * (2 * G) + g] = __builtin_bit_cast(unsigned short, (_Float16)p);
+    }
+    for (int j = j0 + HELD; j < j1; j++) {
+        const long long v_j = snp_vars[j];
+        float p = (float)((double)beta(v_j, g) / den);
+        p = fminf(fmaxf(p, clip_lo), clip_hi);
+        const long long row = prow ? (long long)prow[v_j] : v_j;
+        prob[row * G + g] = p;
+        if (prob16) prob16[row * (2 * G) + g] = __builtin_bit_cast(unsigned short, (_Float16)p);
+    }
+}
 
 template <typename T, int L>
 __global__ __launch_bounds__(256) void k_probs_from_betas(const T *__restrict__ prior,
@@ -27,49 +64,15 @@
     const int snp = n_snps >= 0 ? (int)r : v2snp[v_begin + r];
     const int j0 = snp_ptr[snp], j1 = snp_ptr[snp + 1];
     if (n_snps < 0 && snp_vars[j0] != v_begin + r) return;
-    constexpr int HELD = 4;
     const int cnt = j1 - j0;
-    long long w[HELD];
-#pragma unroll
-    for (int q = 0; q < HELD; q++) w[q] = q < cnt ? (long long)snp_vars[j0 + q] : -1;
-    for (int g = li; g < G; g += L) {
-        T held[HELD];
-#pragma unroll
-        for (int q = 0; q < HELD; q++) {
-            held[q] = (T)0;
-            if (w[q] >= 0) {
-                const long long o = w[q] * G + g;
-                held[q] = addition ? prior[o] + addition[o] : prior[o];
-            }
-        }
-        double den = 0.0;
-#pragma unroll
-        for (int q = 0; q < HELD; q++) den += (double)held[q];
-        for (int j = j0 + HELD; j < j1; j++) {
-            const long long o = (long long)snp_vars[j] * G + g;
-            den += (double)(addition ? prior[o] + addition[o] : prior[o]);
-        }
-        den = fmax(den, 1e-7);
-#pragma unroll
-        for (int q = 0; q < HELD; q++) {
-            if (w[q] < 0) continue;
-            float p = (float)((double)held[q] / den);
-            p = fminf(fmaxf(p, clip_lo), clip_hi);
-            const long long row = prow ? (long long)prow[w[q]] : w[q];
-            prob[row * G + g] = p;
-            if (prob16) prob16[row * (2 * G) + g] = __builtin_bit_cast(unsigned short, (_Float16)p);
-        }
-        for (int j = j0 + HELD; j < j1; j++) {
-            const long long v_j = snp_vars[j];
-            const long long o = v_j * G + g;
-            const T beta = addition ? prior[o] + addition[o] : prior[o];
-            float p = (float)((double)beta / den);
-            p = fminf(fmaxf(p, clip_lo), clip_hi);
-            const long long row = prow ? (long long)prow[v_j] : v_j;
-            prob[row * G + g] = p;
-            if (prob16) prob16[row * (2 * G) + g] = __builtin_bit_cast(unsigned short, (_Float16)p);
-        }
-    }
+    long long w[PSTEP_HELD];
+#pragma unroll
+    for (int q = 0; q < PSTEP_HELD; q++) w[q] = q < cnt ? (long long)snp_vars[j0 + q] : -1;
+    auto beta = [&](long long v, int g) -> T {
+        const long long o = v * G + g;
+        return addition ? prior[o] + addition[o] : prior[o];
+    };
+    for (int g = li; g < G; g += L) pstep_column<T>(w, j0, j1, snp_vars, g, G, prow, clip_lo, clip_hi, prob, prob16, beta);
 }
 
 __global__ __launch_bounds__(256) void k_beta_rowsum(const float *__restrict__ betas, long long V, int G,
@@ -2032,7 +2035,7 @@
 constexpr int MTILE_THREADS = 1024;
 constexpr int MTILE_QUEUE = 96;
 
-template <bool SQUARE>
+template <bool SQUARE, bool PSTEP = false>
 __global__ __launch_bounds__(MTILE_THREADS) void k_mstep_tiles(MstepArgs a, MTileArgs t)
 {
     if (dense_regime(a)) return;
@@ -2139,6 +2142,47 @@
         else a.out64[o] = sum;
         if (t.acc64) t.acc64[(size_t)v * G + g] = mt_acc[i];
     }
+    if constexpr (PSTEP) {
+        auto beta = [&](long long v, int g) -> float {
+            const double sum = __builtin_ldexp((double)(long long)mt_acc[(int)(v - v0) * G + g], -shift);
+            return t.p_prior[v * G + g] + (float)sum;
+        };
+        for (int i = threadIdx.x; i < nv * G; i += MTILE_THREADS) {
+            const int r = (int)((unsigned)i / (unsigned)G), g = i - r * G;
+            const long long v = v0 + r;
+            const int snp = t.p_v2snp[v];
+            const int j0 = t.p_snp_ptr[snp], j1 = t.p_snp_ptr[snp + 1];
+            if (t.p_snp_vars[j0] != v) continue;
+            const int cnt = j1 - j0;
+            long long w[PSTEP_HELD];
+#pragma unroll
+            for (int q = 0; q < PSTEP_HELD; q++) w[q] = q < cnt ? (long long)t.p_snp_vars[j0 + q] : -1;
+            pstep_column<float>(w, j0, j1, t.p_snp_vars, g, G, nullptr, t.p_lo, t.p_hi, t.p_prob, t.p_prob16, beta);
+        }
+    }
+}
+
+template <int L>
+__global__ __launch_bounds__(256) void k_probs_if_dense(const unsigned long long *__restrict__ dense_calls, unsigned long long total_calls,
+                                                        const float *__restrict__ prior, const float *__restrict__ addition,
+                                                        const int *__restrict__ snp_ptr, const int *__restrict__ snp_vars, long long n_snps,
+                                                        int G, float clip_lo, float clip_hi, float *__restrict__ prob,
+                                                        unsigned short *__restrict__ prob16)
+{
+    if (!(dense_calls != nullptr && 4ull * *dense_calls > total_calls)) return;
+    const int lane = threadIdx.x & 63, li = lane & (L - 1);
+    auto beta = [&](long long v, int g) -> float {
+        const long long o = v * G + g;
+        return prior[o] + addition[o];
+    };
+    for (long long r = ((long long)blockIdx.x * 4 + (threadIdx.x >> 6)) * (64 / L) + lane / L; r < n_snps; r += (long long)gridDim.x * 4 * (64 / L)) {
+        const int j0 = snp_ptr[r], j1 = snp_ptr[r + 1];
+        const int cnt = j1 - j0;
+        long long w[PSTEP_HELD];
+#pragma unroll
+        for (int q = 0; q < PSTEP_HELD; q++) w[q] = q < cnt ? (long long)snp_vars[j0 + q] : -1;
+        for (int g = li; g < G; g += L) pstep_column<float>(w, j0, j1, snp_vars, g, G, nullptr, clip_lo, clip_hi, prob, prob16, beta);
+    }
 }
 
 constexpr unsigned MINCR_COOLDOWN = 8;
@@ -2671,6 +2715,20 @@
                                    int G, const int *prow, float lo, float hi, float *prob, unsigned short *prob16)
 {
     return launch_pstep<float>(st, prior, addition, v2snp, snp_ptr, snp_vars, v_begin, n_rows, n_snps, G, prow, lo, hi, prob, prob16);
+}
+
+hipError_t launch_probs_if_dense(hipStream_t st, const unsigned long long *dense_calls, unsigned long long total_calls, const float *prior,
+                                 const float *addition, const int *snp_ptr, const int *snp_vars, long long n_snps, int G, float lo, float hi,
+                                 float *prob, unsigned short *prob16)
+{
+    if (n_snps == 0 || G == 0 || dense_calls == nullptr) return hipSuccess;
+#define PSTEP_DENSE(L)                                                                                                                   \
+    hipLaunchKernelGGL((k_probs_if_dense<L>), dim3(std::min(blocks_for(n_snps, 4 * (64 / L)), 1024u)), dim3(256), 0, st, dense_calls, \
+                       total_calls, prior, addition, snp_ptr, snp_vars, n_snps, G, lo, hi, prob, prob16)
+    if (G <= 16) PSTEP_DENSE(16);
+    else PSTEP_DENSE(32);
+#undef PSTEP_DENSE
+    return hipGetLastError();
 }
 
 hipError_t launch_probs_from_betas_f64(hipStream_t st, const double *betas, const int *v2snp, const int *snp_ptr,
@@ -2973,7 +3031,13 @@
 {
     if (t.n_tiles == 0) return hipSuccess;
     const size_t lds = (size_t)t.tv * a.G * sizeof(unsigned long long);
-    if (a.square)
+    if (t.p_prob != nullptr) {
+        if (t.incr_state != nullptr || a.out32 == nullptr || a.prow != nullptr) return hipErrorInvalidValue;
+        if (a.square)
+            hipLaunchKernelGGL((k_mstep_tiles<true, true>), dim3((unsigned)t.n_tiles), dim3(MTILE_THREADS), lds, st, a, t);
+        else
+            hipLaunchKernelGGL((k_mstep_tiles<false, true>), dim3((unsigned)t.n_tiles), dim3(MTILE_THREADS), lds, st, a, t);
+    } else if (a.square)
         hipLaunchKernelGGL((k_mstep_tiles<true>), dim3((unsigned)t.n_tiles), dim3(MTILE_THREADS), lds, st, a, t);
     else
         hipLaunchKernelGGL((k_mstep_tiles<false>), dim3((unsigned)t.n_tiles), dim3(MTILE_THREADS), lds, st, a, t);
diff --git a/demuxalot_amd/csrc/repack_device.hip b/demuxalot_amd/csrc/repack_device.hip
--- a/demuxalot_amd/csrc/repack_device.hip
+++ b/demuxalot_amd/csrc/repack_device.hip
@@ -687,6 +687,7 @@
     c->incr_valid = false;
     c->n_mt = 0;
     c->mt_tv = 0;
+    c->mt_snp_whole = false;
     c->mt_tried = false;
     c->mt_shift_tried = false;
 }
@@ -700,6 +701,7 @@
     int tv = 0;
     unsigned row_bits = 0;
     long long n_mt = 0;
+    bool snp_whole = false;
 };
 
 bool cut_mstep_tiles(dmx_ctx *c, long long v_lo, long long v_hi, TileCut &t)
@@ -717,6 +719,7 @@
         c->n_simd = 4 * cus;
     }
     t.tv = std::max(1, std::min<int>(dmx::MTILE_MAX_VARIANTS, dmx::MTILE_LDS_BYTES / (G * 8)));
+    const int *snp_of = (long long)c->h_v2snp.size() == V && v_lo == 0 && v_hi == V ? c->h_v2snp.data() : nullptr;
     t.row_bits = bits_for(rows ? (unsigned long long)rows - 1 : 0);
     t.tile_of.assign((size_t)V, 0u);
     t.vin_of.assign((size_t)V, 0u);
@@ -730,6 +733,11 @@
             t.tile_ptr.push_back(first_call[(size_t)v]);
             long long w = v + 1;
             while (w < v_hi && w - v < t.tv && first_call[(size_t)w + 1] - first_call[(size_t)v] <= cap) w++;
+            if (snp_of != nullptr && w < v_hi && snp_of[w] == snp_of[w - 1]) {
+                long long s0 = w - 1;
+                while (s0 > v && snp_of[s0 - 1] == snp_of[w]) s0--;
+                if (s0 > v) w = s0;
+            }
             for (long long x = v; x < w; x++) {
                 t.tile_of[(size_t)x] = (unsigned)(t.tile_first.size() - 1);
                 t.vin_of[(size_t)x] = (unsigned)(x - v);
@@ -742,6 +750,15 @@
         cap *= 2;
     }
     t.n_mt = (long long)t.tile_first.size();
+    t.snp_whole = snp_of != nullptr;
+    if (t.snp_whole) {
+        std::vector<long long> tile_of_snp((size_t)c->S, -1);
+        for (long long v = 0; v < V && t.snp_whole; v++) {
+            long long &home = tile_of_snp[(size_t)snp_of[v]];
+            if (home < 0) home = (long long)t.tile_of[(size_t)v];
+            else if (home != (long long)t.tile_of[(size_t)v]) t.snp_whole = false;
+        }
+    }
     t.tile_first.push_back((int)v_hi);
     t.tile_ptr.push_back(m);
     t.tile_shift.resize((size_t)t.n_mt);
@@ -871,6 +888,7 @@
         HIP_TRY(hipStreamSynchronize(st));
         c->n_mt = n_mt;
         c->mt_tv = tv;
+        c->mt_snp_whole = cut.snp_whole;
         return 0;
     }
     DMX_TRY(upload_variant_shifts(c, cut));
@@ -900,6 +918,7 @@
     HIP_TRY(hipStreamSynchronize(st));
     c->n_mt = n_mt;
     c->mt_tv = tv;
+    c->mt_snp_whole = cut.snp_whole;
     return 0;
 }
 
diff --git a/demuxalot_amd/device.py b/demuxalot_amd/device.py
--- a/demuxalot_amd/device.py
+++ b/demuxalot_amd/device.py
@@ -37,6 +37,7 @@
         self.set_coarse_pass(os.environ.get('DEMUXALOT_AMD_COARSE_PASS', '1') != '0')
         self.set_mstep_incremental(os.environ.get('DEMUXALOT_AMD_MSTEP_INCREMENTAL', '1') != '0')
         self.set_lean_memory(os.environ.get('DEMUXALOT_AMD_LEAN', '0') not in ('', '0'))
+        self.set_fused_tail(os.environ.get('DEMUXALOT_AMD_FUSED_TAIL', '1') != '0')
         self.set_phase_timers(False)
         self.set_logits_needed(True)
 
@@ -559,6 +560,21 @@
     def set_coarse_pass(self, coarse):
         check(self._lib.dmx_set_coarse_pass(self._h, 2 if coarse == 'always' else int(bool(coarse))))
 
+    def set_fused_tail(self, fused):
+        check(self._lib.dmx_set_fused_tail(self._h, int(bool(fused))))
+
+    def fused_tail(self):
+        whole, n = ctypes.c_int32(0), ctypes.c_int64(0)
+        check(self._lib.dmx_get_fused_tail(self._h, ctypes.byref(whole), ctypes.byref(n)))
+        return {'snps_whole_in_tiles': bool(whole.value), 'fused_msteps': int(n.value)}
+
+    def prob_tables(self):
+        prob = np.empty((self.V, self.G), dtype=np.float32)
+        half = np.zeros((self.V, 2 * self.G), dtype=np.uint16)
+        valid = ctypes.c_int32(0)
+        check(self._lib.dmx_debug_get_prob_tables(self._h, ptr(prob), ptr(half), ctypes.byref(valid)))
+        return prob, (np.ascontiguousarray(half[:, :self.G]) if valid.value else None)
+
     def set_lean_memory(self, lean):
         check(self._lib.dmx_set_lean_memory(self._h, int(bool(lean))))
 
diff --git a/include/demux_hip_debug.h b/include/demux_hip_debug.h
--- a/include/demux_hip_debug.h
+++ b/include/demux_hip_debug.h
@@ -12,6 +12,9 @@
 int dmx_set_mstep_tiles(dmx_ctx *ctx, int enable);
 int dmx_get_mstep_tiles_info(dmx_ctx *ctx, int32_t *built, double *build_ms);
 int dmx_get_mstep_form(dmx_ctx *ctx, int32_t *form);
+int dmx_set_fused_tail(dmx_ctx *ctx, int fused);
+int dmx_get_fused_tail(dmx_ctx *ctx, int32_t *snps_whole_in_tiles, int64_t *fused_msteps);
+int dmx_debug_get_prob_tables(dmx_ctx *ctx, float *prob_out, uint16_t *prob16_out, int32_t *prob16_valid);
 
 int dmx_set_guard_adaptive(dmx_ctx *ctx, int adaptive);
 int dmx_set_coarse_pass(dmx_ctx *ctx, int coarse);
```
